# jcasal-homer/HomerHEVC

Hardware: AMD Instinct MI355X
Metric: encoded frames/sec, 1080p & 2160p YUV420 fixed-QP IPPP, 1/2/4/8 MI355X (higher is better)
Workload: dtype int16; 1 GPU; cfg2-1080p-encode; sequences_per_gpu=256, width=1920, height=1080, wfpp_num_threads=17, qp=32, gop=IPPP intra_period=100

## Files before the change

### homerhevc_amd/csrc/k_encode.hip

```cpp
#define HENC_TU_OPERANDS_IN_LDS 1
#include <stddef.h>
#include <stdlib.h>
#include <algorithm>
#include <chrono>
#include <mutex>
#include <condition_variable>
#include <new>
#include <string>
#include <thread>
#include <vector>

#include <type_traits>
#include "common.h"
#include "enc/enc_sched.h"
#include "enc/enc_host.h"
#include "enc/enc_post.h"
#include "picture_io.h"

using namespace henc;

int hmr_subpel_plane_on(hipStream_t stream, int comp, const int16_t *pic, int stride, int rows, uint8_t *out);
int hmr_subpel_planes_on(hipStream_t stream, const int16_t *pic_y, const int16_t *pic_u, const int16_t *pic_v, int stride_y, int rows_y, int stride_c, int rows_c, uint8_t *out_y,
			 uint8_t *out_u, uint8_t *out_v);

struct EncDev {
	const Seq *seq;
	const FrameCtx *frame;
	const DevTables *tables;
	const Geo *geo;
	CtuInfo *ctus, *ctus_start;
	WorkSlow *work_slow;
	int16_t *coeff;
	int *progress;
	uint32_t *prefix;
	unsigned long long *prof;
	uint8_t *guess, *truth, *outtok;
	uint8_t *chain_start, *chain_end;
	int *valid, *dirty;
	unsigned long long *hash;
	uint32_t *intra_before, *used_intra, *used_parts;
	uint8_t *rowstate;
	int *thread_seen;
	int *row0_checked;
	int *counters;
	int threads;
	int dep, dep_full;
	int after, raster;
	FrameCtx *next_frame;
	double *fin;
	RcFrame *rc_dyn;
	const int *rd_src;
	const uint8_t *rd_init, *rd_ring;
	PostPic post;
};

__device__ __forceinline__ void wave_copy_words(void *dst, const void *src, int bytes, int tid)
{
	uint32_t *d = (uint32_t *)dst;
	const uint32_t *s = (const uint32_t *)src;
	for (int i = tid; i < bytes / 4; i += 64) d[i] = s[i];
}
__device__ __forceinline__ void wave_copy_quads(void *dst, const void *src, int bytes, int tid)
{
	uint4 *d = (uint4 *)dst;
	const uint4 *s = (const uint4 *)src;
#pragma unroll 4
	for (int i = tid; i < bytes / 16; i += 64) d[i] = s[i];
}
constexpr int PRED_STATE_BYTES = (64 * 64 + 2 * 32 * 32) * (int)sizeof(pred_t), ROW_STATE_BYTES = MODE_STATE_BYTES + PRED_STATE_BYTES;
static_assert(offsetof(Work, pred_c) == offsetof(Work, pred_y) + 64 * 64 * sizeof(pred_t) && sizeof(((Work *)nullptr)->pred_c) == 2 * 32 * 32 * sizeof(pred_t), "the prediction windows are one block of Work");
static_assert(MODE_STATE_BYTES % 16 == 0 && offsetof(Work, pred_y) % 16 == 0, "wave_copy_quads alignment");

constexpr size_t LDS_WORK = (sizeof(Work) + 15) & ~(size_t)15, LDS_NODES = (sizeof(Node) * NODE_SLOTS + 15) & ~(size_t)15,
		 LDS_GEO = NHELP * HSCRATCH_ELEMS * 2;
namespace henc { __constant__ Geo henc_geo_table[NNODES]; }
constexpr bool LDS_KEEPS_CTU_RECORD = false, LDS_KEEPS_TU_TABLES = false;
static_assert(LDS_KEEPS_TU_TABLES == (HENC_TU_TABLES_IN_LDS != 0), "enc_platform.h: HENC_FT");
constexpr size_t LDS_SEQ = (sizeof(Seq) + sizeof(FrameCtx) + 31) & ~(size_t)15, LDS_CTU = LDS_KEEPS_CTU_RECORD ? (sizeof(CtuPublic) + 15) & ~(size_t)15 : 0,
		 LDS_FT = LDS_KEEPS_TU_TABLES ? (sizeof(FastTables) + 15) & ~(size_t)15 : 0;
#if defined(HENC_PROFILE)
constexpr size_t LDS_BOX = LDS_BOX_BYTES + (1 + NHELP) * LDS_ENC_BYTES, LDS_HSCRATCH = 0, LDS_RD = (sizeof(WorkRd) + 15) & ~(size_t)15;
constexpr size_t LDS_BYTES = HENC_LDS_PROF_OFFSET + 2 * PP_COUNT * 8;
constexpr size_t LDS_FT_OFFSET = LDS_WORK + LDS_NODES + LDS_GEO + LDS_SEQ + LDS_CTU + LDS_BOX + LDS_HSCRATCH;
static_assert(LDS_WORK + LDS_NODES + LDS_GEO + LDS_SEQ + LDS_CTU + LDS_BOX + LDS_HSCRATCH + LDS_FT + LDS_RD <= HENC_LDS_PROF_OFFSET, "profile table overlaps the worker state");
#else
constexpr size_t LDS_BOX = LDS_BOX_BYTES + (1 + NHELP) * LDS_ENC_BYTES, LDS_HSCRATCH = 0, LDS_RD = (sizeof(WorkRd) + 15) & ~(size_t)15;
constexpr size_t LDS_BYTES = LDS_WORK + LDS_NODES + LDS_GEO + LDS_SEQ + LDS_CTU + LDS_BOX + LDS_HSCRATCH + LDS_FT + LDS_RD;
constexpr size_t LDS_FT_OFFSET = LDS_WORK + LDS_NODES + LDS_GEO + LDS_SEQ + LDS_CTU + LDS_BOX + LDS_HSCRATCH;
#endif
static_assert(sizeof(SubpelScratch) <= LDS_WORK + LDS_NODES + LDS_GEO, "task S works where the post stage does");
static_assert(sizeof(PostScratch) <= LDS_WORK + LDS_NODES + LDS_GEO, "the post stage works in what is idle between two CTUs: the worker's Work area, the CTU's partition nodes, the helpers' scratch");
#if !defined(HENC_PROFILE)
static_assert(LDS_OFF_RD == (int)(LDS_BYTES - LDS_RD), "the RD_FULL arrays are the tail of a worker's LDS");
#endif
static_assert(LDS_OFF_ENC == (int)(LDS_WORK + LDS_NODES + LDS_GEO + LDS_SEQ + LDS_CTU + LDS_BOX_BYTES) || LDS_FT != 0 || LDS_CTU != 0, "the RD_FULL arrays are the tail of a worker's LDS: launches without RD_FULL pictures leave them out");
static_assert(LDS_OFF_NODES == (int)LDS_WORK && LDS_OFF_SEQ == (int)(LDS_WORK + LDS_NODES + LDS_GEO) && LDS_OFF_BOX == (int)(LDS_WORK + LDS_NODES + LDS_GEO + LDS_SEQ + LDS_CTU),
	      "enc_common.h: the fixed places of Enc's LDS members");
#if !defined(HENC_WAVES_PER_EU)
#define HENC_WAVES_PER_EU 2
#endif
constexpr int ENC_THREADS = 64 * (1 + NHELP);
static_assert(LDS_BYTES <= 160 * 1024, "a workgroup has 160 KiB of LDS on gfx950");
constexpr int workers_per_cu(size_t lds_bytes)
{
	const int by_lds = (int)((160 * 1024) / ((lds_bytes + 1279) / 1280 * 1280)), by_waves = 4 * HENC_WAVES_PER_EU / (1 + NHELP);
	return by_lds < by_waves ? by_lds : by_waves;
}
constexpr int WORKERS_PER_CU = workers_per_cu(LDS_BYTES - LDS_RD);
#if !defined(HENC_PROFILE) && HENC_WAVES_PER_EU == 2 && HENC_NHELP == 1
static_assert(WORKERS_PER_CU == 4, "a worker's LDS (without the RD_FULL arrays) has to stay within a quarter of the CU's: 32 granules of 1280 bytes");
#endif
#if defined(HENC_PRINT_LDS)
static_assert(LDS_BYTES - LDS_RD == 0 && LDS_WORK == 0 && LDS_NODES == 0 && LDS_BOX == 0 && sizeof(PostScratch) == 0 && WORKERS_PER_CU == 0, "sizes");
#endif

__device__ __forceinline__ bool helper_serve(HelperBox *box, int h, int16_t *scratch, const WaveGrp g, int seq)
{
	extern __shared__ __align__(16) uint8_t lds[];
	Enc &e = *(Enc *)(lds + LDS_OFF_ENC + (1 + h) * LDS_ENC_BYTES);
	HENC_ENC_IN_LDS(e);
	const Enc &worker = *(const Enc *)(lds + LDS_OFF_ENC);
	{
		const int job = box->job[h];
		if (job == HJOB_QUIT) return false;
		if (job == HJOB_NEW_CTU) {
			wave_copy_words(&e, &worker, (int)sizeof(Enc), g.tid);
			g.sync();
			e.box = nullptr;
			e.on_helper = 1 + h;
			e.scratch_a = scratch;
			e.scratch_b = scratch + 1024;
			e.adi_c = scratch + 2048;
			e.prof = nullptr;
		}
		const int *a = box->a[h];
		uint32_t r0 = 0, r1 = 0, r2 = 0, r3 = 0, r4 = 0, r5 = 0;
		switch (job) {
		case HJOB_INTER_TU: {
			int sum = 0;
			uint32_t raw = 0;
			if (NHELP == 1 && a[1] == COMP_UV && e.geo[a[0]].size_chroma <= 8) {
				const PairGrp pg{g.tid & 31, g.tid >> 5};
				const uint32_t d = encode_inter_tu(pg, e, a[0], COMP_U + pg.half, a[2], a[3], &sum, &raw, pg.half * 512);
				r0 = (uint32_t)__builtin_amdgcn_readlane((int)d, 0); r1 = (uint32_t)__builtin_amdgcn_readlane(sum, 0); r2 = (uint32_t)__builtin_amdgcn_readlane((int)raw, 0);
				r3 = (uint32_t)__builtin_amdgcn_readlane((int)d, 32); r4 = (uint32_t)__builtin_amdgcn_readlane(sum, 32); r5 = (uint32_t)__builtin_amdgcn_readlane((int)raw, 32);
				break;
			}
			r0 = encode_inter_tu(g, e, a[0], a[1] == COMP_UV ? COMP_U : a[1], a[2], a[3], &sum, &raw);
			r1 = (uint32_t)sum;
			r2 = raw;
			if (a[1] == COMP_UV) {
				r3 = encode_inter_tu(g, e, a[0], COMP_V, a[2], a[3], &sum, &raw);
				r4 = (uint32_t)sum;
				r5 = raw;
			}
			break;
		}
		case HJOB_SYNC_CU:
			if (a[1] == COMP_UV) sync_cu_chroma_both(g, e, a[0], a[2], a[3], a[4], a[5]);
			else sync_cu_comp(g, e, a[0], a[2], a[3], a[4], a[5], a[1]);
			break;
		case HJOB_SSD: {
			const Geo &q = e.geo[a[0]];
			if (a[1] == COMP_UV) {
				const int n = q.size_chroma, l = ilog2i(n);
				uint32_t acc[2] = {0, 0};
				for (int i = g.tid * 4; i < n * n; i += 64 * 4) {
					const int o = q.yc * 32 + q.xc + (i >> l) * 32 + (i & (n - 1));
#pragma unroll
					for (int c = 0; c < 2; c++) {
						const S4 va = ld4(e.w->curr_c[c] + o), vb = ld4(e.w->pred_c[c] + o);
#pragma unroll
						for (int k = 0; k < 4; k++) { const int32_t dd = (int16_t)(va.v[k] - vb.v[k]); acc[c] += (uint32_t)(dd * dd); }
					}
				}
				r0 = g.sum(acc[0]);
				r1 = g.sum(acc[1]);
			} else {
				const int c = a[1] - 1;
				r0 = blk_ssd(g, e.w->curr_c[c] + q.yc * 32 + q.xc, 32, e.w->pred_c[c] + q.yc * 32 + q.xc, 32, q.size_chroma);
			}
			break;
		}
		case HJOB_CHROMA_SEARCH: {
			const int cand[5] = {a[2] & 255, (a[2] >> 8) & 255, (a[2] >> 16) & 255, (a[2] >> 24) & 255, a[3]};
			uint32_t sads[5];
			chroma_search_comp(g, e, a[0], a[1], cand, sads);
			g.sync();
			if (g.tid == 0)
				for (int k = 0; k < 5; k++) box->r[h][k] = sads[k];
			break;
		}
		case HJOB_CHROMA_TU: {
			int cs = 0;
			r0 = (uint32_t)chroma_tu_comp(g, e, a[0], a[1], a[2], a[3], a[4], a[5] & 255, a[5] >> 8, &cs);
			r1 = (uint32_t)cs;
			break;
		}
#if defined(HENC_QUAD)
		case HJOB_QUAD_C:
			quad_chroma_job(g, e, a[0], a[1]);
			break;
#endif
		case HJOB_INTRA_SAD: {
			const Geo &q = e.geo[a[0]];
			r0 = intra_predict_sad(g, (pred_t *)nullptr, 0, e.w->curr_y + q.y * CTU_STRIDE_Y + q.x, CTU_STRIDE_Y, a[3] ? e.w->adi_f : e.w->adi, a[1], a[2], 1);
			break;
		}
		default: break;
		}
		g.sync();
		if (g.tid == 0) {
			if (job != HJOB_CHROMA_SEARCH) { box->r[h][0] = r0; box->r[h][1] = r1; box->r[h][2] = r2; box->r[h][3] = r3; box->r[h][4] = r4; box->r[h][5] = r5; }
			__hip_atomic_store(&box->done[h], seq, __ATOMIC_RELEASE, __HIP_MEMORY_SCOPE_WORKGROUP);
		}
	}
	return true;
}

__device__ __attribute__((noinline)) bool helper_serve_out(HelperBox *box, int h, int16_t *scratch, const WaveGrp g, int seq) { return helper_serve(box, h, scratch, g, seq); }

__device__ __attribute__((noinline)) bool helper_bg_search(HelperBox *box, int h, int16_t *scratch, const WaveGrp g, int &seq, int bgseq)
{
	extern __shared__ __align__(16) uint8_t lds[];
	Enc &e = *(Enc *)(lds + LDS_OFF_ENC + (1 + h) * LDS_ENC_BYTES);
	HENC_ENC_IN_LDS(e);
	const int ni = uni(box->bg_ni), depth = uni(box->bg_depth);
	const Geo &q = e.geo[ni];
	const int n = q.size, curr_depth = q.depth, inv_depth = CFG_MAX_CU_SHIFT - curr_depth;
	bool quit = false;
	int best_mode = 0, bits = -1;
	double best_cost = 0;
	if (__hip_atomic_load(&box->bg_cancel, __ATOMIC_ACQUIRE, __HIP_MEMORY_SCOPE_WORKGROUP) != bgseq) {
		node_fill_refs(g, e, ni, depth + 1, COMP_Y, 1);
		int preds[3], dirs[2];
		uint16_t src[2];
		intra_neighbour_dirs(e, ni, curr_depth, dirs, src);
		mpm_from_dirs(dirs[0], dirs[1], preds);
		const int rd_fast = e.seq->rd_mode == RDM_FAST ? 1 : 0;
		const src_t *orig = e.w->curr_y + q.y * CTU_STRIDE_Y + q.x;
		bits = intra_search_walk(preds, rd_fast, e.f->sqrt_lambda, [&](int mode) -> int64_t {
			if (__hip_atomic_load(&box->cmd[h], __ATOMIC_ACQUIRE, __HIP_MEMORY_SCOPE_WORKGROUP) == seq) {
				if (!helper_serve_out(box, h, scratch, g, seq)) { quit = true; return -1; }
				seq++;
			}
			if (__hip_atomic_load(&box->bg_cancel, __ATOMIC_ACQUIRE, __HIP_MEMORY_SCOPE_WORKGROUP) == bgseq) return -1;
			return (int64_t)intra_predict_sad(g, (pred_t *)nullptr, 0, orig, CTU_STRIDE_Y, intra_is_filtered(mode, inv_depth) ? e.w->adi_f : e.w->adi, n, mode, 1);
		}, &best_mode, &best_cost);
	}
	g.sync();
	if (g.tid == 0) {
		box->bg_mode = best_mode;
		box->bg_bits = bits;
		__hip_atomic_store(&box->bg_done, bgseq, __ATOMIC_RELEASE, __HIP_MEMORY_SCOPE_WORKGROUP);
	}
	return !quit;
}

template <bool LAT>
__device__ __attribute__((noinline)) void helper_loop(HelperBox *box, int h, int16_t *scratch)
{
	WaveGrp g{(int)(threadIdx.x & 63)};
	if constexpr (!LAT) {
		for (int seq = 1;; seq++) {
			while (__hip_atomic_load(&box->cmd[h], __ATOMIC_ACQUIRE, __HIP_MEMORY_SCOPE_WORKGROUP) != seq) __builtin_amdgcn_s_sleep(1);
			if (!helper_serve(box, h, scratch, g, seq)) return;
		}
	}
	int seq = 1, bgseq = 1;
	for (;;) {
		if (__hip_atomic_load(&box->cmd[h], __ATOMIC_ACQUIRE, __HIP_MEMORY_SCOPE_WORKGROUP) == seq) {
			if (!helper_serve_out(box, h, scratch, g, seq)) return;
			seq++;
			continue;
		}
		if (NHELP == 1 && __hip_atomic_load(&box->bg_cmd, __ATOMIC_ACQUIRE, __HIP_MEMORY_SCOPE_WORKGROUP) == bgseq) {
			if (!helper_bg_search(box, h, scratch, g, seq, bgseq)) return;
			bgseq++;
			continue;
		}
		__builtin_amdgcn_s_sleep(1);
	}
}

template <bool LAT = false>
__device__ __forceinline__ bool rows_enter(unsigned lds_bytes)
{
	extern __shared__ __align__(16) uint8_t lds[];
	HelperBox *box = (HelperBox *)(lds + LDS_WORK + LDS_NODES + LDS_GEO + LDS_SEQ + LDS_CTU);
	const int wave = (int)(threadIdx.x >> 6);
	for (int i = (int)threadIdx.x; i < (int)(lds_bytes / 4); i += ENC_THREADS) ((uint32_t *)lds)[i] = 0;
	__syncthreads();
	if (wave > 0) {
		helper_loop<LAT>(box, wave - 1, (int16_t *)(lds + LDS_WORK + LDS_NODES) + (wave - 1) * HSCRATCH_ELEMS);
		return false;
	}
	return true;
}
__device__ __forceinline__ void release_helpers(int *hseq)
{
	extern __shared__ __align__(16) uint8_t lds[];
	HelperBox *box = (HelperBox *)(lds + LDS_WORK + LDS_NODES + LDS_GEO + LDS_SEQ + LDS_CTU);
	if ((threadIdx.x & 63) == 0)
		for (int h = 0; h < NHELP; h++) {
			box->job[h] = HJOB_QUIT;
			__hip_atomic_store(&box->cmd[h], ++hseq[h], __ATOMIC_RELEASE, __HIP_MEMORY_SCOPE_WORKGROUP);
		}
}
__device__ __forceinline__ void encode_row(const EncDev &d, int pass, int row, int *hseq)
{
	extern __shared__ __align__(16) uint8_t lds[];
	const Seq &S = *d.seq;
	const int W = S.wctu, H = S.hctu;
	WaveGrp g{(int)(threadIdx.x & 63)};
	Work *lw = (Work *)lds;
	HelperBox *box = (HelperBox *)(lds + LDS_WORK + LDS_NODES + LDS_GEO + LDS_SEQ + LDS_CTU);
	for (int i = g.tid; i < (int)(LDS_WORK / 4); i += 64) ((uint32_t *)lds)[i] = 0;
	g.sync();
	Seq *lseq = (Seq *)(lds + LDS_WORK + LDS_NODES + LDS_GEO);
	FrameCtx *lframe = (FrameCtx *)((uint8_t *)lseq + ((sizeof(Seq) + 15) & ~(size_t)15));
	for (int i = g.tid; i < (int)(sizeof(Seq) / 4); i += 64) ((uint32_t *)lseq)[i] = ((const uint32_t *)d.seq)[i];
	for (int i = g.tid; i < (int)(sizeof(FrameCtx) / 4); i += 64) ((uint32_t *)lframe)[i] = ((const uint32_t *)d.frame)[i];
	if (g.tid == 0) lw->slow = (HENC_GLOBAL_PTR(WorkSlow))(d.work_slow + row);
// ... 542 lines not shown
```

### homerhevc_amd/csrc/k_encode_batch.inc

```
namespace {
__global__ __launch_bounds__(256) void k_pack_streams(const EncDev *devs, uint8_t *out, const size_t *offs)
{
	__shared__ uint32_t start[POST_MAX_ROWS + 1];
	const EncDev &d = devs[blockIdx.x];
	const int rows = d.seq->wpp ? d.seq->hctu : 1;
	if (threadIdx.x == 0) {
		uint32_t o = 0;
		for (int r = 0; r < rows; r++) { start[r] = o; o += (uint32_t)d.post.ent[r].bytecnt; }
		start[rows] = o;
	}
	__syncthreads();
	uint8_t *dst = out + offs[blockIdx.x];
	for (int r = 0; r < rows; r++) {
		const uint8_t *src = d.post.bs + (size_t)r * d.post.row_cap;
		const uint32_t n = start[r + 1] - start[r];
		for (uint32_t i = threadIdx.x; i < n; i += blockDim.x) dst[start[r] + i] = src[i];
	}
}

__global__ void k_batch_stage(const EncDev *h_devs, const FrameCtx *h_frames, EncDev *d_devs, FrameCtx *d_frames)
{
	const int i = blockIdx.x, t = threadIdx.x;
	for (int k = t; k < (int)(sizeof(EncDev) / 4); k += blockDim.x) ((uint32_t *)(d_devs + i))[k] = ((const uint32_t *)(h_devs + i))[k];
	for (int k = t; k < (int)(sizeof(FrameCtx) / 4); k += blockDim.x) ((uint32_t *)(d_frames + i))[k] = ((const uint32_t *)(h_frames + i))[k];
	const EncDev d = h_devs[i];
	const int H = d.seq->hctu, W = d.seq->wctu;
	if (t < 3) d.counters[t] = t == 2 ? -1 : 0;
	if (t == 3) *d.row0_checked = 0;
	if (t >= 4 && t < 8) d.post.errors[t - 4] = 0;
	for (int k = t; k < H * (int)(sizeof(PostRow) / 4); k += blockDim.x) ((int *)d.post.rows)[k] = 0;
	for (int k = t; k < H; k += blockDim.x) d.progress[k] = 0;
	for (int k = t; k < H * (W + 1); k += blockDim.x) d.prefix[k] = 0;
}

struct BatchTimes {
	std::chrono::steady_clock::time_point t[8];
	double ms(int a, int b) const { return std::chrono::duration<double, std::milli>(t[b] - t[a]).count(); }
};

template <class F>
void parallel_for(int n, int threads, F fn)
{
	const int T = n < threads ? n : threads;
	std::vector<std::thread> th;
	for (int t = 0; t < T; t++)
		th.emplace_back([=]() {
			for (int i = t; i < n; i += T) fn(i);
		});
	for (auto &x : th) x.join();
}
constexpr int QUEUE_THREADS = 16;
constexpr int CODING_THREADS = 32;

int batch_check(hmr_gpu_enc **encs, int n, const int *slots, uint8_t **streams, const long *caps, long *stream_bytes)
{
	if (!encs || n <= 0 || n > BATCH_MAX || !streams || !caps || !stream_bytes) return HMR_GPU_ERR_ARG;
	for (int i = 0; i < n; i++) {
		hmr_gpu_enc *e = encs[i];
		if (!e || !e->lockstep || e->ctx->device != encs[0]->ctx->device || (slots && (slots[i] < 0 || slots[i] >= (int)e->src.size())) || !streams[i]) {
			hmr_set_error("hmr_gpu_enc_encode_batch: encoder %d: needs the row-per-thread schedule (wfpp_num_threads > 1), the batch's device and a loaded picture slot", i);
			return HMR_GPU_ERR_ARG;
		}
		for (int j = 0; j < i; j++)
			if (encs[j] == e) return HMR_GPU_ERR_ARG;
	}
	return HMR_GPU_OK;
}

int batch_launch(hmr_gpu_enc **encs, int n, const int *slots, const int *image_types, int *pitch_out)
{
	hmr_gpu_enc *lead = encs[0];
	hipStream_t bst = lead->ctx->stream;
	int rc, rows_total = 0, max_ctus = 0;
	bool needs_rd = false;
	if (!lead->d_frames) {
		HIP_TRY(hipMalloc((void **)&lead->d_frames, BATCH_MAX * sizeof(FrameCtx)));
		HIP_TRY(hipHostMalloc((void **)&lead->h_frames, BATCH_MAX * sizeof(FrameCtx), hipHostMallocDefault));
		HIP_TRY(hipHostMalloc((void **)&lead->h_devs, BATCH_MAX * sizeof(EncDev), hipHostMallocDefault));
	}
	for (int i = 0; i < n; i++) {
		hmr_gpu_enc *e = encs[i];
		if ((rc = set_frame(e, slots[i], image_types ? image_types[i] : 0, -1.0, false))) return rc;
		e->pic_stream = bst;
		HIP_TRY(hipEventRecord(e->ev_ready, e->ctx->stream));
		if (i) HIP_TRY(hipStreamWaitEvent(bst, e->ev_ready, 0));
		lead->h_frames[i] = e->f;
		lead->h_devs[i] = e->d;
		lead->h_devs[i].frame = lead->d_frames + i;
		rows_total += pool_inflight(e->seq, e->raster);
		needs_rd = needs_rd || e->seq.rd_mode == RDM_FULL;
		if (e->seq.nctu > max_ctus) max_ctus = e->seq.nctu;
	}
	if (!lead->plane_stream[0]) {
		for (int k = 0; k < 2; k++) {
			HIP_TRY(hipStreamCreateWithFlags(&lead->plane_stream[k], hipStreamNonBlocking));
			HIP_TRY(hipEventCreateWithFlags(&lead->ev_plane[k], hipEventDisableTiming));
		}
		HIP_TRY(hipEventCreateWithFlags(&lead->ev_plane[2], hipEventDisableTiming));
	}
	HIP_TRY(hipEventRecord(lead->ev_plane[2], bst));
	for (int k = 0; k < 2; k++) HIP_TRY(hipStreamWaitEvent(lead->plane_stream[k], lead->ev_plane[2], 0));
	for (int i = 0; i < n; i++) {
		hmr_gpu_enc *e = encs[i];
		const Seq &s = e->seq;
		if (e->f.slice_type == SLICE_I) continue;
		if ((rc = hmr_subpel_plane_on(bst, 0, e->d_pic[e->cur ^ 1][0], s.stride_y, s.height + 2 * s.margin_y, e->planes.y))) return rc;
		for (int k = 0; k < 2; k++)
			if ((rc = hmr_subpel_plane_on(lead->plane_stream[k], 1 + k, e->d_pic[e->cur ^ 1][1 + k], s.stride_c, s.height / 2 + 2 * s.margin_c, e->planes.c[k]))) return rc;
	}
	for (int k = 0; k < 2; k++) {
		HIP_TRY(hipEventRecord(lead->ev_plane[k], lead->plane_stream[k]));
		HIP_TRY(hipStreamWaitEvent(bst, lead->ev_plane[k], 0));
	}
	if (!lead->d_batch) {
		HIP_TRY(hipMalloc((void **)&lead->d_batch, BATCH_MAX * sizeof(EncDev)));
		HIP_TRY(hipDeviceGetAttribute(&lead->n_cus, hipDeviceAttributeMultiprocessorCount, lead->ctx->device));
	}
	const int pitch = GATHER_HEAD + max_ctus + POST_MAX_ROWS;
	if ((size_t)pitch * n > lead->gather_words) {
		if (lead->d_gather) (void)hipFree(lead->d_gather);
		if (lead->h_gather) (void)hipHostFree(lead->h_gather);
		lead->d_gather = lead->h_gather = nullptr;
		lead->gather_words = 0;
		HIP_TRY(hipMalloc((void **)&lead->d_gather, (size_t)pitch * BATCH_MAX * 4));
		HIP_TRY(hipHostMalloc((void **)&lead->h_gather, (size_t)pitch * BATCH_MAX * 4, hipHostMallocDefault));
		lead->gather_words = (size_t)pitch * BATCH_MAX;
	}
	hipLaunchKernelGGL(k_batch_stage, dim3(n), dim3(256), 0, bst, (const EncDev *)lead->h_devs, (const FrameCtx *)lead->h_frames, (EncDev *)lead->d_batch, lead->d_frames);
	HIP_TRY(hipGetLastError());
	HIP_TRY(hipEventRecord(lead->ev_batch0, bst));
	if ((rc = launch_pool(lead, n, rows_total, needs_rd, bst))) return rc;
	(void)hipEventRecord(lead->ev_batch1, bst);
	hipLaunchKernelGGL(k_gather_results, dim3(n), dim3(256), 0, bst, (const EncDev *)lead->d_batch, lead->d_gather, pitch, (const int *)(lead->d_pool_state + BATCH_MAX * POOL_STRIDE));
	HIP_TRY(hipGetLastError());
	HIP_TRY(hipMemcpyAsync(lead->h_gather, lead->d_gather, (size_t)pitch * n * 4, hipMemcpyDeviceToHost, bst));
	*pitch_out = pitch;
	return HMR_GPU_OK;
}

int batch_finish(hmr_gpu_enc **encs, int n, const int *slots, int pitch, BatchTimes &bt)
{
	(void)slots;
	hmr_gpu_enc *lead = encs[0];
	hipStream_t bst = lead->ctx->stream;
	const hipError_t waited = hipStreamSynchronize(bst);
	if (waited != hipSuccess) {
		hmr_set_error("k_encode_pool: %s", hipGetErrorString(waited));
		return HMR_GPU_ERR_HIP;
	}
	bt.t[2] = std::chrono::steady_clock::now();
	float ms = 0;
	HIP_TRY(hipEventElapsedTime(&ms, lead->ev_batch0, lead->ev_batch1));
	if (!lead->h_offs) HIP_TRY(hipHostMalloc((void **)&lead->h_offs, BATCH_MAX * sizeof(size_t), hipHostMallocDefault));
	lead->pend_off.resize(n);
	lead->pend_rows.assign(n, std::vector<uint32_t>());
	size_t total = 0;
	for (int i = 0; i < n; i++) {
		hmr_gpu_enc *e = encs[i];
		const uint32_t *g = lead->h_gather + (size_t)i * pitch;
		if (g[3] & 2) {
			hmr_set_error("k_encode_pool: the launch was abandoned by its watchdog (a worker found nothing to do for too long: HENC_WATCHDOG_S)");
			return HMR_GPU_ERR_HIP;
		}
		if (g[3] & 1) {
			hmr_set_error("hmr_gpu_enc_encode_batch: sequence %d: a CTU row's sub-stream outgrew its buffer (%d bytes)", i, e->row_cap);
			return HMR_GPU_ERR_HIP;
		}
		e->note_stale_predictions(g[3] >> 8);
		const int rows = e->seq.wpp ? e->seq.hctu : 1;
		lead->pend_off[i] = total;
		lead->h_offs[i] = total;
		lead->pend_rows[i].assign(g + pitch - POST_MAX_ROWS, g + pitch - POST_MAX_ROWS + rows);
		for (int r = 0; r < rows; r++) total += lead->pend_rows[i][r];
		total = (total + 255) & ~(size_t)255;
		e->last_ms = e->last_total_ms = ms;
		e->last_encodes = (int)g[1];
		e->f.scene_cut_ctu = (int)g[2];
		e->last_passes = 1;
		release_planes(e);
		e->f_pending = e->f;
		e->awaiting_delivery = true;
		FrameRcOut ro;
		ro.sum_qp = (int)g[4]; ro.consumed_bits = (double)g[5];
		memcpy(&ro.target_pict_size, &g[6], 8);
		end_frame(e->seq, e->st, e->f, frame_acc_dist(e->seq, e->cfg.wfpp_num_threads, [&](int c) { return g[GATHER_HEAD + c]; }), &ro);
	}
	if (total > lead->stage_bytes) {
		if (lead->d_stage) (void)hipFree(lead->d_stage);
		if (lead->h_stage) (void)hipHostFree(lead->h_stage);
		lead->d_stage = lead->h_stage = nullptr;
		lead->stage_bytes = 0;
		const size_t want = total * 2 + (1 << 20);
		HIP_TRY(hipMalloc((void **)&lead->d_stage, want));
		HIP_TRY(hipHostMalloc((void **)&lead->h_stage, want, hipHostMallocDefault));
		lead->stage_bytes = want;
	}
	if (!lead->copy_stream) HIP_TRY(hipStreamCreateWithFlags(&lead->copy_stream, hipStreamNonBlocking));
	hipLaunchKernelGGL(k_pack_streams, dim3(n), dim3(256), 0, bst, (const EncDev *)lead->d_batch, lead->d_stage, (const size_t *)lead->h_offs);
	HIP_TRY(hipGetLastError());
	HIP_TRY(hipEventRecord(lead->ev_decided, bst));
	HIP_TRY(hipStreamWaitEvent(lead->copy_stream, lead->ev_decided, 0));
	if (total) HIP_TRY(hipMemcpyAsync(lead->h_stage, lead->d_stage, total, hipMemcpyDeviceToHost, lead->copy_stream));
	bt.t[3] = std::chrono::steady_clock::now();
	lead->pend_encs.assign(encs, encs + n);
	lead->pend_total = total;
	lead->pending = true;
	return HMR_GPU_OK;
}

int batch_deliver(hmr_gpu_enc *lead, uint8_t **streams, const long *caps, long *stream_bytes, BatchTimes &bt)
{
	const int n = (int)lead->pend_encs.size();
	bt.t[4] = std::chrono::steady_clock::now();
	lead->pending = false;
	for (int i = 0; i < n; i++) lead->pend_encs[i]->awaiting_delivery = false;
	HIP_TRY(hipStreamSynchronize(lead->copy_stream));
	bt.t[5] = std::chrono::steady_clock::now();
	std::vector<int> rcs(n, 0);
	std::vector<std::string> errs(n);
	parallel_for(n, CODING_THREADS, [&](int i) {
		hmr_gpu_enc *e = lead->pend_encs[i];
		rcs[i] = frame_assemble(e, e->f_pending, lead->h_stage + lead->pend_off[i], lead->pend_rows[i].data(), streams[i], caps[i], &stream_bytes[i]);
		if (rcs[i] < 0) errs[i] = hmr_gpu_last_error();
	});
	bt.t[6] = std::chrono::steady_clock::now();
	for (int i = 0; i < n; i++)
		if (rcs[i] < 0) { hmr_set_error("hmr_gpu_enc_encode_batch: sequence %d: %s", i, errs[i].c_str()); return rcs[i]; }
	return HMR_GPU_OK;
}

void batch_report(const BatchTimes &bt, hmr_gpu_enc *lead, bool pipelined)
{
	if (!getenv("HENC_BATCH_TIMING")) return;
	static std::chrono::steady_clock::time_point last_end;
	const auto now = std::chrono::steady_clock::now();
	fprintf(stderr, "batch step%s: launch %.1f ms, wait for the pool %.1f, queue device parts %.1f, download wait %.1f (%.0f MB), entropy coding %.1f; the call %.1f, since the last call %.1f\n",
		pipelined ? " (pipelined)" : "", bt.ms(0, 1), pipelined ? bt.ms(6, 2) : bt.ms(1, 2), bt.ms(2, 3), bt.ms(4, 5), lead->pend_total / 1e6, bt.ms(5, 6),
		std::chrono::duration<double, std::milli>(now - bt.t[0]).count(), std::chrono::duration<double, std::milli>(bt.t[0] - last_end).count());
	last_end = now;
}
}

extern "C" int hmr_gpu_enc_encode_batch(hmr_gpu_enc **encs, int n, const int *slots, const int *image_types, uint8_t **streams, const long *caps, long *stream_bytes)
{
	int rc = batch_check(encs, n, slots, streams, caps, stream_bytes);
	if (rc) return rc;
	if (!slots) return HMR_GPU_ERR_ARG;
	for (int i = 0; i < n; i++)
		if (encs[i]->awaiting_delivery || encs[i]->pending) {
			hmr_set_error("hmr_gpu_enc_encode_batch: encoder %d has an access unit outstanding from a pipelined call: flush first", i);
			return HMR_GPU_ERR_ARG;
		}
	hmr_gpu_enc *lead = encs[0];
	HIP_TRY(hipSetDevice(lead->ctx->device));
	BatchTimes bt;
	int pitch = 0;
	bt.t[0] = std::chrono::steady_clock::now();
	if ((rc = batch_launch(encs, n, slots, image_types, &pitch))) return rc;
	bt.t[1] = std::chrono::steady_clock::now();
	if ((rc = batch_finish(encs, n, slots, pitch, bt))) return rc;
	if ((rc = batch_deliver(lead, streams, caps, stream_bytes, bt))) return rc;
	batch_report(bt, lead, false);
	return HMR_GPU_OK;
}

extern "C" int hmr_gpu_enc_encode_batch_pipelined(hmr_gpu_enc **encs, int n, const int *slots, const int *image_types, uint8_t **streams, const long *caps, long *stream_bytes)
{
	int rc = batch_check(encs, n, slots, streams, caps, stream_bytes);
	if (rc) return rc;
	hmr_gpu_enc *lead = encs[0];
	HIP_TRY(hipSetDevice(lead->ctx->device));
	if (lead->pending) {
		if ((int)lead->pend_encs.size() != n || memcmp(lead->pend_encs.data(), encs, n * sizeof(hmr_gpu_enc *))) {
			hmr_set_error("hmr_gpu_enc_encode_batch_pipelined: the encoder list changed while access units are outstanding: flush (slots = NULL) with the previous list first");
			return HMR_GPU_ERR_ARG;
		}
	} else {
		for (int i = 0; i < n; i++)
			if (encs[i]->awaiting_delivery) {
				hmr_set_error("hmr_gpu_enc_encode_batch_pipelined: encoder %d has an access unit outstanding in another batch", i);
				return HMR_GPU_ERR_ARG;
			}
	}
	BatchTimes bt;
	for (auto &t : bt.t) t = std::chrono::steady_clock::now();
	int pitch = 0;
	if (slots && (rc = batch_launch(encs, n, slots, image_types, &pitch))) return rc;
	bt.t[1] = std::chrono::steady_clock::now();
	if (lead->pending) {
		if ((rc = batch_deliver(lead, streams, caps, stream_bytes, bt))) return rc;
	} else {
		for (int i = 0; i < n; i++) stream_bytes[i] = 0;
		bt.t[6] = bt.t[1];
	}
	if (slots && (rc = batch_finish(encs, n, slots, pitch, bt))) return rc;
	if (slots) batch_report(bt, lead, true);
	return HMR_GPU_OK;
}

extern "C" int hmr_gpu_enc_encode_chain(hmr_gpu_enc **encs, int n, hmr_gpu_enc *prev, const int *slots, const int *image_types, uint8_t **streams, const long *caps, long *stream_bytes)
{
	if (!encs || n <= 0 || n > CHAIN_MAX_FRAMES || !slots || !streams || !caps || !stream_bytes) return HMR_GPU_ERR_ARG;
	for (int j = 0; j < n; j++) {
		hmr_gpu_enc *e = encs[j];
		if (!e || !e->lockstep || e->ctx->device != encs[0]->ctx->device || slots[j] < 0 || slots[j] >= (int)e->src.size() || !streams[j] || e->awaiting_delivery || e->engine_index < 0 ||
		    e->seq.width != encs[0]->seq.width || e->seq.height != encs[0]->seq.height) {
			hmr_set_error("hmr_gpu_enc_encode_chain: frame %d: needs an engine object (hmr_gpu_enc_create_engine) of the chain's sequence on the chain's device with a loaded picture slot", j);
			return HMR_GPU_ERR_ARG;
		}
		if (n > 1 && (e->seq.bitrate_mode != 0 || e->seq.rd_mode == RDM_FULL)) {
			hmr_set_error("hmr_gpu_enc_encode_chain: frame %d: rate control and RD_FULL need the frames one at a time (a chain of %d frames starts them from a predicted state)", j, n);
			return HMR_GPU_ERR_ARG;
		}
		if (j >= e->st.engines && e->d_ctus_eng[0] != encs[j - e->st.engines]->d_ctus_eng[0]) {
			hmr_set_error("hmr_gpu_enc_encode_chain: frame %d: the object has to be a twin (hmr_gpu_enc_create_engine_twin) of the one that encodes frame %d, the engine's frame before it", j, j - e->st.engines);
			return HMR_GPU_ERR_ARG;
		}
		for (int i = 0; i < j; i++)
			if (encs[i] == e) return HMR_GPU_ERR_ARG;
	}
	hmr_gpu_enc *lead = encs[0];
	hipStream_t bst = lead->ctx->stream;
	HIP_TRY(hipSetDevice(lead->ctx->device));
	int rc, rows_total = 0;
	bool needs_rd = false;
	if (!lead->d_frames) {
		HIP_TRY(hipMalloc((void **)&lead->d_frames, BATCH_MAX * sizeof(FrameCtx)));
		HIP_TRY(hipHostMalloc((void **)&lead->h_frames, BATCH_MAX * sizeof(FrameCtx), hipHostMallocDefault));
		HIP_TRY(hipHostMalloc((void **)&lead->h_devs, BATCH_MAX * sizeof(EncDev), hipHostMallocDefault));
	}
	if (!lead->d_batch) HIP_TRY(hipMalloc((void **)&lead->d_batch, BATCH_MAX * sizeof(EncDev)));
	HostState st = prev ? prev->st : lead->st;
	const HostState start_state = st;
	struct Undo { hmr_gpu_enc *e; int cur; HostState st; FrameCtx f; PlaneSet planes, planes2; EncDev d; bool has_picture; hipStream_t pic_stream; };
	std::vector<Undo> undo;
	auto refuse = [&](int code) {
		for (size_t k = undo.size(); k-- > 0;) {
			Undo &u = undo[k];
			u.e->cur = u.cur; u.e->st = u.st; u.e->f = u.f; u.e->chain_planes = u.planes; u.e->chain_planes2 = u.planes2; u.e->d = u.d;
			u.e->has_picture = u.has_picture; u.e->pic_stream = u.pic_stream;
		}
		return code;
	};
	for (int j = 0; j < n; j++) {
		hmr_gpu_enc *e = encs[j];
		const Seq &s = e->seq;
		if (st.num_encoded_frames % e->st.engines != e->engine_index) {
			hmr_set_error("hmr_gpu_enc_encode_chain: frame %d of the sequence belongs to engine %d, not %d", st.num_encoded_frames, st.num_encoded_frames % e->st.engines, e->engine_index);
			return refuse(HMR_GPU_ERR_ARG);
		}
		for (int k = 0; k < 2; k++) {
			PlaneSet &ps = k ? e->chain_planes2 : e->chain_planes;
			if (ps.y) continue;
			PlaneSet p;
			p.device = e->ctx->device; p.bytes_y = (size_t)16 * s.plane_elems_y; p.bytes_c = (size_t)64 * s.plane_elems_c;
			HIP_TRY(hipMalloc((void **)&p.y, p.bytes_y));
			HIP_TRY(hipMalloc((void **)&p.c[0], p.bytes_c));
			HIP_TRY(hipMalloc((void **)&p.c[1], p.bytes_c));
			ps = p;
		}
		undo.push_back(Undo{e, e->cur, e->st, e->f, e->chain_planes, e->chain_planes2, e->d, e->has_picture, e->pic_stream});
		e->st = st;
		const hmr_gpu_enc *r = j ? encs[j - 1] : prev;
		const int16_t *ref_planes[3] = {nullptr, nullptr, nullptr};
		PlaneSet ref_set;
		if (r) {
			for (int c = 0; c < 3; c++) ref_planes[c] = plane0(const_cast<hmr_gpu_enc *>(r), r->cur, c);
			ref_set = r->chain_planes;
		}
		std::swap(e->chain_planes, e->chain_planes2);
		if (j == 0 && e == prev) ref_set = e->chain_planes2;
		if ((rc = set_frame(e, slots[j], image_types ? image_types[j] : 0, -1.0, false, true))) return refuse(rc);
		e->pic_stream = bst;
		st = e->st;
		st.num_encoded_frames++;
		if (e->f.slice_type != SLICE_I) {
			if (!r || !ref_set.y) {
				hmr_set_error("hmr_gpu_enc_encode_chain: frame %d is a P frame and there is no object that holds the picture before it with its phase planes", j);
				return refuse(HMR_GPU_ERR_ARG);
			}
			for (int c = 0; c < 3; c++) e->f.ref[c] = ref_planes[c];
			e->f.sub_y = ref_set.y + (size_t)s.margin_y * 16 * s.stride_y + s.margin_y;
			e->f.sub_c[0] = ref_set.c[0] + (size_t)s.margin_c * 64 * s.stride_c + s.margin_c;
			e->f.sub_c[1] = ref_set.c[1] + (size_t)s.margin_c * 64 * s.stride_c + s.margin_c;
			e->d.dep = j ? j - 1 : -1;
			e->d.dep_full = getenv("HENC_CHAIN_SERIAL") ? 1 : 0;
		}
		if (j >= e->st.engines) {
			const hmr_gpu_enc *b = encs[j - e->st.engines];
			if (b->f.slice_type == SLICE_I && b->f.num_encoded_frames != 0 && s.intra_period != 1) {
				hmr_set_error("hmr_gpu_enc_encode_chain: frame %d is an I frame inside the sequence and the same engine's next frame is in the chain: end the chain before frame %d", j - e->st.engines, j);
				return refuse(HMR_GPU_ERR_ARG);
			}
			e->d.after = j - e->st.engines;
			e->f.avg_dist = 0.0;
			lead->h_devs[j - e->st.engines].next_frame = lead->d_frames + j;
		}
		e->d.post.planes[0] = e->chain_planes.y; e->d.post.planes[1] = e->chain_planes.c[0]; e->d.post.planes[2] = e->chain_planes.c[1];
		HIP_TRY(hipEventRecord(e->ev_ready, e->ctx->stream));
		if (j) HIP_TRY(hipStreamWaitEvent(bst, e->ev_ready, 0));
		lead->h_frames[j] = e->f;
		lead->h_devs[j] = e->d;
		lead->h_devs[j].frame = lead->d_frames + j;
		rows_total += s.hctu;
		needs_rd = needs_rd || s.rd_mode == RDM_FULL;
	}
	const int nctu = lead->seq.nctu, pitch = GATHER_HEAD + nctu + POST_MAX_ROWS;
	if ((size_t)pitch * n > lead->gather_words) {
		if (lead->d_gather) (void)hipFree(lead->d_gather);
		if (lead->h_gather) (void)hipHostFree(lead->h_gather);
		lead->d_gather = lead->h_gather = nullptr;
		lead->gather_words = 0;
		HIP_TRY(hipMalloc((void **)&lead->d_gather, (size_t)pitch * BATCH_MAX * 4));
		HIP_TRY(hipHostMalloc((void **)&lead->h_gather, (size_t)pitch * BATCH_MAX * 4, hipHostMallocDefault));
		lead->gather_words = (size_t)pitch * BATCH_MAX;
	}
	hipLaunchKernelGGL(k_batch_stage, dim3(n), dim3(256), 0, bst, (const EncDev *)lead->h_devs, (const FrameCtx *)lead->h_frames, (EncDev *)lead->d_batch, lead->d_frames);
	HIP_TRY(hipGetLastError());
	HIP_TRY(hipEventRecord(lead->ev_batch0, bst));
	if ((rc = launch_pool(lead, n, rows_total, needs_rd, bst))) return rc;
	(void)hipEventRecord(lead->ev_batch1, bst);
	hipLaunchKernelGGL(k_gather_results, dim3(n), dim3(256), 0, bst, (const EncDev *)lead->d_batch, lead->d_gather, pitch, (const int *)(lead->d_pool_state + BATCH_MAX * POOL_STRIDE));
	HIP_TRY(hipGetLastError());
	HIP_TRY(hipMemcpyAsync(lead->h_gather, lead->d_gather, (size_t)pitch * n * 4, hipMemcpyDeviceToHost, bst));
	{
		const hipError_t waited = hipStreamSynchronize(bst);
		if (waited != hipSuccess) { hmr_set_error("k_encode_pool: %s", hipGetErrorString(waited)); return HMR_GPU_ERR_HIP; }
	}
	float ms = 0;
	HIP_TRY(hipEventElapsedTime(&ms, lead->ev_batch0, lead->ev_batch1));
	HostState seq_state = start_state;
	bool cut_before = false;
	for (int j = 0; j < n; j++) {
		hmr_gpu_enc *e = encs[j];
		const Seq &s = e->seq;
		const uint32_t *g = lead->h_gather + (size_t)j * pitch;
		if (g[3] & 2) { hmr_set_error("k_encode_pool: the launch was abandoned by its watchdog (HENC_WATCHDOG_S)"); return HMR_GPU_ERR_HIP; }
		if (g[3] & 1) { hmr_set_error("hmr_gpu_enc_encode_chain: frame %d: a CTU row's sub-stream outgrew its buffer (%d bytes)", j, e->row_cap); return HMR_GPU_ERR_HIP; }
		e->note_stale_predictions(g[3] >> 8);
		e->last_ms = e->last_total_ms = ms;
		e->last_encodes = (int)g[1];
		e->f.scene_cut_ctu = (int)g[2];
		e->last_passes = 1;
		const bool fired = (int)g[2] >= 0;
		if (fired && cut_before) {
			hmr_set_error("hmr_gpu_enc_encode_chain: two frames of the chain detected a scene change: in the sequential order the first one switches the detection off for the second; repeat the chain frame by frame");
			return HMR_GPU_ERR_ARG;
		}
		cut_before = cut_before || fired;
		FrameCtx replay;
		e->st = seq_state;
		begin_frame(s, e->st, image_types ? image_types[j] : 0, replay);
		double acc_dist;
		memcpy(&acc_dist, &g[8], 8);
		memcpy(&e->f.avg_dist, &g[10], 8);
		if (replay.slice_type != e->f.slice_type || replay.poc != e->f.poc || replay.avg_dist != e->f.avg_dist) {
			hmr_set_error("hmr_gpu_enc_encode_chain: frame %d started from a state the frames before it changed", j);
			return HMR_GPU_ERR_ARG;
		}
		FrameRcOut ro;
		ro.sum_qp = (int)g[4]; ro.consumed_bits = (double)g[5];
		memcpy(&ro.target_pict_size, &g[6], 8);
		end_frame(s, e->st, e->f, acc_dist, &ro);
		seq_state = e->st;
		const int rows = s.wpp ? s.hctu : 1;
		std::vector<uint32_t> row_bytes(g + pitch - POST_MAX_ROWS, g + pitch - POST_MAX_ROWS + rows);
		size_t total = 0;
		for (int r = 0; r < rows; r++) total += row_bytes[r];
		if (e->h_bs.size() < total) e->h_bs.resize(total);
		total = 0;
		for (int r = 0; r < rows; r++) {
			HIP_TRY(hipMemcpyAsync(e->h_bs.data() + total, e->d_bs + (size_t)r * e->row_cap, row_bytes[r], hipMemcpyDeviceToHost, bst));
			total += row_bytes[r];
		}
		HIP_TRY(hipStreamSynchronize(bst));
		if ((rc = frame_assemble(e, e->f, e->h_bs.data(), row_bytes.data(), streams[j], caps[j], &stream_bytes[j])) < 0) return rc;
	}
	return HMR_GPU_OK;
}

extern "C" int hmr_gpu_enc_encode(hmr_gpu_enc *e, const uint8_t *y, const uint8_t *u, const uint8_t *v, int image_type, uint8_t *stream, long cap, long *stream_bytes,
				  uint8_t *recon)
{
	const int rc = hmr_gpu_enc_load_source(e, 0, y, u, v);
	if (rc) return rc;
	return hmr_gpu_enc_encode_source(e, 0, image_type, stream, cap, stream_bytes, recon);
}
```

### homerhevc_amd/csrc/k_encode_object.inc

```
template <class T>
struct PinnedAlloc {
	typedef T value_type;
	PinnedAlloc() = default;
	template <class U> PinnedAlloc(const PinnedAlloc<U> &) {}
	T *allocate(size_t n)
	{
		void *p = nullptr;
		if (hipHostMalloc(&p, n * sizeof(T), hipHostMallocDefault) != hipSuccess) throw std::bad_alloc();
		return (T *)p;
	}
	void deallocate(T *p, size_t) { (void)hipHostFree(p); }
	template <class U> bool operator==(const PinnedAlloc<U> &) const { return true; }
	template <class U> bool operator!=(const PinnedAlloc<U> &) const { return false; }
};

struct PlaneSet { uint8_t *y = nullptr, *c[2] = {nullptr, nullptr}; size_t bytes_y = 0, bytes_c = 0; int device = 0; };
struct PlanePool {
	std::mutex m;
	std::vector<PlaneSet> free_sets;
	int acquire(int device, size_t by, size_t bc, PlaneSet *out)
	{
		{
			std::lock_guard<std::mutex> lk(m);
			for (size_t i = 0; i < free_sets.size(); i++)
				if (free_sets[i].device == device && free_sets[i].bytes_y == by && free_sets[i].bytes_c == bc) {
					*out = free_sets[i];
					free_sets.erase(free_sets.begin() + (long)i);
					return HMR_GPU_OK;
				}
		}
		PlaneSet p;
		p.device = device; p.bytes_y = by; p.bytes_c = bc;
		if (hipMalloc((void **)&p.y, by) != hipSuccess || hipMalloc((void **)&p.c[0], bc) != hipSuccess || hipMalloc((void **)&p.c[1], bc) != hipSuccess) {
			(void)hipGetLastError();
			if (p.y) (void)hipFree(p.y);
			if (p.c[0]) (void)hipFree(p.c[0]);
			if (p.c[1]) (void)hipFree(p.c[1]);
			hmr_set_error("phase planes: out of device memory (%zu bytes per picture)", by + 2 * bc);
			return HMR_GPU_ERR_HIP;
		}
		*out = p;
		return HMR_GPU_OK;
	}
	void release(const PlaneSet &p)
	{
		std::lock_guard<std::mutex> lk(m);
		free_sets.push_back(p);
	}
	int live = 0;
	void encoder_created() { std::lock_guard<std::mutex> lk(m); live++; }
	void encoder_destroyed()
	{
		std::lock_guard<std::mutex> lk(m);
		if (--live > 0) return;
		for (PlaneSet &p : free_sets) {
			(void)hipSetDevice(p.device);
			(void)hipFree(p.y); (void)hipFree(p.c[0]); (void)hipFree(p.c[1]);
		}
		free_sets.clear();
	}
};
PlanePool g_plane_pool;
struct hmr_gpu_enc {
	hmr_gpu_ctx *ctx;
	HostCfg cfg;
	long stale_last = -1, stale_total = 0;
	void note_stale_predictions(uint32_t n) { stale_last = (long)n; stale_total += (long)n; }
	Seq seq;
	HostState st;
	FrameCtx f;
	EncDev d;
	Seq *d_seq;
	FrameCtx *d_frame;
	Geo *d_geo;
	std::vector<Geo> geo;
	std::vector<SrcSlot> src;
	int16_t *d_pic[2][3], *d_pre[3], *d_rec[3];
	PostRow *d_rows = nullptr;
	RowEnt *d_ent = nullptr;
	uint8_t *d_bs = nullptr;
	uint32_t *d_cumbits = nullptr;
	double *d_sao_tab = nullptr;
	int *d_post_err = nullptr;
	RdCtxSim rdsim[MAX_ENGINES];
	uint8_t *d_ctx_ring = nullptr, *d_rd_init = nullptr;
	int *d_rd_src = nullptr;
	uint8_t h_rd_init[(1 + RD_RING) * RD_CTX_BYTES] = {0};
	uint16_t *d_rc_need = nullptr;
	RcFrame *d_rc_dyn = nullptr;
	int row_cap = 0;
	std::vector<RowEnt> h_ent;
	std::vector<uint8_t, PinnedAlloc<uint8_t>> h_bs;
	PlaneSet chain_planes2;
	PlaneSet chain_planes;
	PlaneSet planes;
	size_t src_elems[3], pic_elems[3];
	uint8_t *d_bytes;
	int units_stride, units_rows;
	int16_t *d_mvx, *d_mvy;
	int8_t *d_ref;
	uint8_t *d_qp, *d_flags;
	uint8_t *d_public;
	std::vector<uint8_t, PinnedAlloc<uint8_t>> h_public;
	std::vector<int16_t, PinnedAlloc<int16_t>> h_coeff;
	std::vector<int32_t> h_stats, h_params;
	std::vector<double> h_lambdas;
	hipEvent_t ev_frame = nullptr, ev_ready = nullptr, ev_batch0 = nullptr, ev_batch1 = nullptr;
	int n_cus = 0;
	uint8_t *d_stage = nullptr, *h_stage = nullptr;
	size_t stage_bytes = 0;
	void *d_batch = nullptr;
	bool pending = false, download_queued = false;
	std::vector<hmr_gpu_enc *> pend_encs;
	std::vector<size_t> pend_off;
	std::vector<std::vector<uint32_t>> pend_rows;
	size_t *h_offs = nullptr;
	size_t pend_total = 0;
	hipStream_t copy_stream = nullptr;
	uint32_t *d_gather = nullptr, *h_gather = nullptr;
	size_t gather_words = 0;
	bool awaiting_delivery = false;
	FrameCtx f_pending;
	double acc_pending = 0;
	hipEvent_t ev_packed = nullptr;
	hipEvent_t ev_decided = nullptr;
	FrameCtx *d_frames = nullptr, *h_frames = nullptr;
	EncDev *h_devs = nullptr;
	hipStream_t plane_stream[2] = {nullptr, nullptr};
	hipEvent_t ev_plane[3] = {nullptr, nullptr, nullptr};
	int *d_pool_state = nullptr;
	WorkSlow *d_pool_slow = nullptr;
	int pool_workers = 0;
	JobRing<IngestJob> ingest;
	JobRing<RgbIngestJob> ingest_rgb;
	JobRing<ScaleJob> scale;
	JobRing<EgressJob> egress;
	JobRing<SsimJob> ssim;
	bool has_picture = false;
	hipStream_t pic_stream = nullptr;
	hipEvent_t ev_pic_done = nullptr, ev_own_done = nullptr;
	EntropyState es;
	CtuInfo *d_ctus_eng[MAX_ENGINES] = {nullptr};
	uint8_t *d_rowstate_eng[MAX_ENGINES] = {nullptr};
	int *d_seen_eng[MAX_ENGINES] = {nullptr};
	hmr_gpu_enc *twin_of = nullptr;
	int local_engines = 1, engine_index = -1;
	int cur, lockstep;
	int raster = 0;
	float last_ms, last_total_ms;
	int last_passes, last_encodes;
};

namespace {
void release_planes(hmr_gpu_enc *e);
constexpr int REC_BYTES = 32 + 3 * 256 + 2 * 256 + 9 * 256 + 256 + 256 + 2048 + 2048 + 6144 * 2 + 6144 * 2 + 2 * 5 * 256;

int16_t *plane0(hmr_gpu_enc *e, int which, int comp)
{
	const Seq &s = e->seq;
	const int st = comp ? s.stride_c : s.stride_y, m = comp ? s.margin_c : s.margin_y;
	return e->d_pic[which][comp] + (size_t)m * st + m;
}

template <class T>
int dev_alloc(T **p, size_t n, hipStream_t st)
{
	HIP_TRY(hipMalloc((void **)p, n * sizeof(T)));
	HIP_TRY(hipMemsetAsync(*p, 0, n * sizeof(T), st));
	HIP_TRY(hipStreamSynchronize(st));
	return HMR_GPU_OK;
}
#define DEV_ALLOC(p, n)                           \
	do {                                      \
		const int rc_ = dev_alloc(&(p), (n), e->ctx->stream); \
		if (rc_) return rc_;              \
	} while (0)

IngestJob ingest_job(const hmr_gpu_enc *e, const hmr_gpu_picture &pic, int16_t *const dst[3], int stride_y, int stride_c)
{
	IngestJob j;
	for (int c = 0; c < 3; c++) {
		j.src[c] = pic.plane[c];
		j.pitch[c] = pic.pitch[c];
		j.dst[c] = dst[c];
	}
	j.stride_y = stride_y; j.stride_c = stride_c;
	j.width = e->seq.width; j.height = e->seq.height;
	j.format = pic.format; j.reserved = 0;
	return j;
}
EgressJob egress_job(hmr_gpu_enc *e, const hmr_gpu_picture *pic, int16_t *const src[3], uint64_t *ssd)
{
	const Seq &s = e->seq;
	EgressJob j;
	for (int c = 0; c < 3; c++) {
		j.rec[c] = plane0(e, e->cur, c);
		j.src[c] = src ? src[c] : nullptr;
		j.dst[c] = pic ? const_cast<uint8_t *>(pic->plane[c]) : nullptr;
		j.pitch[c] = pic ? pic->pitch[c] : 0;
	}
	j.ssd = ssd;
	j.stride_y = s.stride_y; j.stride_c = s.stride_c;
	j.src_stride_y = s.src_stride_y; j.src_stride_c = s.src_stride_c;
	j.width = s.width; j.height = s.height;
	j.format = pic ? pic->format : HMR_GPU_PIC_I420; j.reserved = 0;
	return j;
}
hmr_gpu_picture packed_picture(const hmr_gpu_enc *e, const uint8_t *bytes)
{
	const int64_t w = e->seq.width, h = e->seq.height;
	return hmr_gpu_picture{HMR_GPU_PIC_I420, 0, {bytes, bytes + w * h, bytes + w * h + (w / 2) * (h / 2)}, {w, w / 2, w / 2}};
}
int widen_packed(hmr_gpu_enc *e, const uint8_t *bytes, int16_t *const dst[3], int stride_y, int stride_c)
{
	const IngestJob j = ingest_job(e, packed_picture(e, bytes), dst, stride_y, stride_c);
	return run_jobs(e->ingest, hmr_ingest_launch, e->ctx->stream, &j, 1, e->ctx->stream);
}
int narrow_packed(hmr_gpu_enc *e, uint8_t *bytes)
{
	const hmr_gpu_picture pic = packed_picture(e, bytes);
	const EgressJob j = egress_job(e, &pic, nullptr, nullptr);
	return run_jobs(e->egress, hmr_egress_launch, e->ctx->stream, &j, 1, e->ctx->stream);
}

int load_planes(hmr_gpu_enc *e, const uint8_t *y, const uint8_t *u, const uint8_t *v, int16_t *const dst[3], int stride_y, int stride_c)
{
	hipStream_t st = e->ctx->stream;
	const hmr_gpu_picture staged = packed_picture(e, e->d_bytes);
	const uint8_t *in[3] = {y, u, v};
	for (int c = 0; c < 3; c++)
		HIP_TRY(hipMemcpyAsync(const_cast<uint8_t *>(staged.plane[c]), in[c], (size_t)staged.pitch[c] * (c ? e->seq.height / 2 : e->seq.height), hipMemcpyHostToDevice, st));
	const int rc = widen_packed(e, e->d_bytes, dst, stride_y, stride_c);
	if (rc) return rc;
	HIP_TRY(hipStreamSynchronize(st));
	return HMR_GPU_OK;
}


int reference_planes(hmr_gpu_enc *e, hipStream_t st)
{
	const Seq &s = e->seq;
	if (e->f.slice_type == SLICE_I) return HMR_GPU_OK;
	return hmr_subpel_planes_on(st, e->d_pic[e->cur ^ 1][0], e->d_pic[e->cur ^ 1][1], e->d_pic[e->cur ^ 1][2], s.stride_y, s.height + 2 * s.margin_y, s.stride_c,
				    s.height / 2 + 2 * s.margin_c, e->planes.y, e->planes.c[0], e->planes.c[1]);
}
int ctu_stage_prepare(hmr_gpu_enc *e, bool planes_elsewhere = false)
{
	const Seq &s = e->seq;
	hipStream_t st = e->ctx->stream;
	if (!e->lockstep)
		HIP_TRY(hipMemcpyAsync(e->d.ctus_start, e->d.ctus, sizeof(CtuInfo) * s.nctu, hipMemcpyDeviceToDevice, st));
	if (!planes_elsewhere) {
		const int rc = reference_planes(e, st);
		if (rc) return rc;
	}
	{
		static const int zero_counters[3] = {0, 0, -1};
		HIP_TRY(hipMemcpyAsync(e->d.counters, zero_counters, sizeof zero_counters, hipMemcpyHostToDevice, st));
	}
	if (e->lockstep) {
		HIP_TRY(hipMemsetAsync(e->d.progress, 0, sizeof(int) * s.hctu, st));
		HIP_TRY(hipMemsetAsync(e->d.row0_checked, 0, sizeof(int), st));
		HIP_TRY(hipMemsetAsync(e->d.prefix, 0, sizeof(uint32_t) * s.hctu * (s.wctu + 1), st));
	}
	HIP_TRY(hipMemsetAsync(e->d_rows, 0, sizeof(PostRow) * s.hctu, st));
	HIP_TRY(hipMemsetAsync(e->d_post_err, 0, sizeof(int) * 4, st));
	return HMR_GPU_OK;
}
int lockstep_collect(hmr_gpu_enc *e)
{
	hipStream_t st = e->ctx->stream;
	int counters[3], aborted = 0;
	HIP_TRY(hipMemcpyAsync(counters, e->d.counters, sizeof counters, hipMemcpyDeviceToHost, st));
	HIP_TRY(hipMemcpyAsync(&aborted, e->d_pool_state + BATCH_MAX * POOL_STRIDE + 1, sizeof(int), hipMemcpyDeviceToHost, st));
	HIP_TRY(hipStreamSynchronize(st));
	e->last_encodes = counters[1];
	e->f.scene_cut_ctu = counters[2];
	e->last_passes = 1;
	release_planes(e);
	if (aborted) {
		hmr_set_error("k_encode_pool: the launch was abandoned by its watchdog (a worker found nothing to do for too long: HENC_WATCHDOG_S)");
		return HMR_GPU_ERR_HIP;
	}
	return HMR_GPU_OK;
}

static int pool_inflight(const Seq &s, int raster = 0)
{
	if (raster) return 3;
	const int by_step = s.hctu < (s.wctu + 1) / 2 ? s.hctu : (s.wctu + 1) / 2;
	return s.bitrate_mode != 0 ? (by_step + 1) / 2 : by_step;
}
int launch_pool(hmr_gpu_enc *lead, int n, int rows_total, bool needs_rd, hipStream_t st)
{
	if (!lead->n_cus) HIP_TRY(hipDeviceGetAttribute(&lead->n_cus, hipDeviceAttributeMultiprocessorCount, lead->ctx->device));
#if defined(HENC_PROFILE)
	const size_t lds_default = LDS_BYTES + (needs_rd ? 0 : 0);
#else
	const size_t lds_default = needs_rd ? LDS_BYTES : LDS_BYTES - LDS_RD;
#endif
	const size_t lds_bytes = getenv("HENC_LDS_BYTES") && (size_t)atoi(getenv("HENC_LDS_BYTES")) > lds_default ? (size_t)atoi(getenv("HENC_LDS_BYTES")) : lds_default;
	if (lds_bytes > 160 * 1024) {
		hmr_set_error("k_encode_pool: a worker's LDS request of %zu bytes (HENC_LDS_BYTES) is more than a CU has", lds_bytes);
		return HMR_GPU_ERR_ARG;
	}
	const int cap = lead->n_cus * workers_per_cu(lds_bytes);
	int workers = rows_total < cap ? rows_total : cap;
	if (workers < 1) workers = 1;
	if (getenv("HENC_POOL_WORKERS") && atoi(getenv("HENC_POOL_WORKERS")) > 0 && atoi(getenv("HENC_POOL_WORKERS")) < workers) workers = atoi(getenv("HENC_POOL_WORKERS"));
	if (!lead->d_pool_state) HIP_TRY(hipMalloc((void **)&lead->d_pool_state, sizeof(int) * (BATCH_MAX * POOL_STRIDE + 4)));
	if (lead->pool_workers < workers) {
		if (lead->d_pool_slow) (void)hipFree(lead->d_pool_slow);
		lead->d_pool_slow = nullptr;
		lead->pool_workers = 0;
		HIP_TRY(hipMalloc((void **)&lead->d_pool_slow, sizeof(WorkSlow) * workers));
		HIP_TRY(hipMemsetAsync(lead->d_pool_slow, 0, sizeof(WorkSlow) * workers, st));
		lead->pool_workers = workers;
	}
	HIP_TRY(hipMemsetAsync(lead->d_pool_state, 0, sizeof(int) * (BATCH_MAX * POOL_STRIDE + 4), st));
	double watchdog_s = getenv("HENC_WATCHDOG_S") ? atof(getenv("HENC_WATCHDOG_S")) : 120.0;
	if (!(watchdog_s > 0)) watchdog_s = 120.0;
	const unsigned long long watchdog = (unsigned long long)(watchdog_s * 1e8);
	if (workers <= 256) hipLaunchKernelGGL(k_encode_pool_lat, dim3(workers), dim3(ENC_THREADS), lds_bytes, st, (const EncDev *)lead->d_batch, n, lead->d_pool_state, lead->d_pool_state + BATCH_MAX * POOL_STRIDE,
			   lead->d_pool_slow, watchdog, (unsigned)lds_default);
	else hipLaunchKernelGGL(k_encode_pool, dim3(workers), dim3(ENC_THREADS), lds_bytes, st, (const EncDev *)lead->d_batch, n, lead->d_pool_state, lead->d_pool_state + BATCH_MAX * POOL_STRIDE,
			   lead->d_pool_slow, watchdog, (unsigned)lds_default);
	const hipError_t launched = hipGetLastError();
	if (launched != hipSuccess) {
		hmr_set_error("k_encode_pool: %s", hipGetErrorString(launched));
		return HMR_GPU_ERR_HIP;
	}
	return HMR_GPU_OK;
}

int run_ctu_passes(hmr_gpu_enc *e)
{
	const Seq &s = e->seq;
	hipStream_t st = e->ctx->stream;
	int rc = ctu_stage_prepare(e);
	if (rc) return rc;
	HIP_TRY(hipEventRecord(e->ctx->ev0, st));
	if (e->lockstep) {
		if (!e->d_batch) HIP_TRY(hipMalloc((void **)&e->d_batch, BATCH_MAX * sizeof(EncDev)));
		HIP_TRY(hipMemcpyAsync(e->d_batch, &e->d, sizeof(EncDev), hipMemcpyHostToDevice, st));
		if ((rc = launch_pool(e, 1, e->raster ? pool_inflight(s, 1) : s.hctu, s.rd_mode == RDM_FULL, st))) return rc;
		HIP_TRY(hipEventRecord(e->ctx->ev1, st));
		if ((rc = lockstep_collect(e))) return rc;
		HIP_TRY(hipEventElapsedTime(&e->last_ms, e->ctx->ev0, e->ctx->ev1));
		return HMR_GPU_OK;
	}
	int pass = 0;
	for (;; pass++) {
		HIP_TRY(hipMemsetAsync(e->d.progress, 0, sizeof(int) * s.hctu, st));
		{
			EncDev dd = e->d;
			int pp = pass;
			void *args[] = {&dd, &pp};
			const hipError_t launched = hipLaunchCooperativeKernel((const void *)k_encode_ctus, dim3(s.hctu), dim3(ENC_THREADS), args, (unsigned)LDS_BYTES, st);
			if (launched != hipSuccess) {
				hmr_set_error("k_encode_ctus (%d row workers, cooperative): %s", s.hctu, hipGetErrorString(launched));
				return HMR_GPU_ERR_HIP;
			}
		}
		hipLaunchKernelGGL(k_sched_scan, dim3(1), dim3(320), 0, st, e->d);
		hipLaunchKernelGGL(k_sched_check, dim3(s.nctu), dim3(64), 0, st, e->d);
		HIP_TRY(hipGetLastError());
		int counters[3];
		HIP_TRY(hipMemcpyAsync(counters, e->d.counters, sizeof counters, hipMemcpyDeviceToHost, st));
		HIP_TRY(hipStreamSynchronize(st));
		e->last_encodes = counters[1];
		e->f.scene_cut_ctu = counters[2];
		if (counters[0] == 0) break;
		if (pass > s.nctu + 2) {
			hmr_set_error("hmr_gpu_enc: the CTU schedule did not converge");
			return HMR_GPU_ERR_HIP;
		}
	}
	hipLaunchKernelGGL(k_sched_finish, dim3(s.nctu), dim3(64), 0, st, e->d);
	HIP_TRY(hipMemcpyAsync(e->d.chain_start, e->d.chain_end, MODE_STATE_BYTES, hipMemcpyDeviceToDevice, st));
	HIP_TRY(hipMemcpyAsync(e->d_frame, &e->f, sizeof(FrameCtx), hipMemcpyHostToDevice, st));
	HIP_TRY(hipFuncSetAttribute((const void *)k_post_frame, hipFuncAttributeMaxDynamicSharedMemorySize, (int)sizeof(PostScratch)));
	hipLaunchKernelGGL(k_post_frame, dim3(s.hctu < 32 ? s.hctu : 32), dim3(64), sizeof(PostScratch), st, e->d);
	HIP_TRY(hipGetLastError());
	HIP_TRY(hipEventRecord(e->ctx->ev1, st));
	HIP_TRY(hipStreamSynchronize(st));
	HIP_TRY(hipEventElapsedTime(&e->last_ms, e->ctx->ev0, e->ctx->ev1));
	e->last_passes = pass + 1;
	release_planes(e);
	return HMR_GPU_OK;
}

int set_frame(hmr_gpu_enc *e, int slot, int image_type, double avg_dist, bool upload = true, bool chain = false)
{
	const Seq &s = e->seq;
	e->cur ^= 1;
	e->has_picture = true;
	e->pic_stream = e->ctx->stream;
	{
		const int k = e->local_engines > 1 ? e->st.num_encoded_frames % e->local_engines : 0;
		e->d.ctus = e->d_ctus_eng[k];
		e->d.rowstate = e->d_rowstate_eng[k];
		e->d.thread_seen = e->d_seen_eng[k];
	}
	begin_frame(s, e->st, image_type, e->f);
	if (avg_dist >= 0) e->f.avg_dist = avg_dist;
	e->f.lockstep = e->lockstep && !e->raster;
	for (int c = 0; c < 3; c++) {
		e->f.src[c] = e->src[slot].p[c];
		e->f.ref[c] = plane0(e, e->cur ^ 1, c);
		e->f.rec[c] = e->d_rec[c] + (size_t)(c ? s.margin_c : s.margin_y) * (c ? s.stride_c : s.stride_y) + (c ? s.margin_c : s.margin_y);
		e->d.post.fin[c] = plane0(e, e->cur, c);
	}
	e->d.post.sao_lambda = e->d_sao_tab + (e->f.slice_type == SLICE_I ? 104 : 0);
	e->d.post.ctx_after = nullptr;
	if (s.rd_mode == RDM_FULL) {
		std::vector<RdCtxVersion> src;
		e->rdsim[e->local_engines > 1 ? e->f.num_encoded_frames % e->local_engines : 0].frame(e->f.num_encoded_frames, src, e->raster != 0);
		std::vector<int> codes(s.nctu);
		for (int n = 0; n < s.nctu; n++) {
			const RdCtxVersion v = src[n];
			if (v.frame > e->f.num_encoded_frames || (v.frame >= 0 && v.frame <= e->f.num_encoded_frames - RD_RING)) {
				hmr_set_error("RD_FULL: CTU %d copies coder states of frame %d in frame %d (the states of %d frames are kept)", n, v.frame, e->f.num_encoded_frames, RD_RING);
				return HMR_GPU_ERR_ARG;
			}
			const int slot = v.frame < 0 ? 0 : v.frame % RD_RING;
			codes[n] = v.frame < 0 ? 0 : (v.k == 0 ? (1 << 28) | (slot << 24) : (3 << 28) | (slot << 24) | (v.row * s.wctu + v.k - 1));
		}
		const int slot_now = e->f.num_encoded_frames % RD_RING;
		for (int i = 0; i < CTX_TOTAL; i++) e->h_rd_init[(1 + slot_now) * RD_CTX_BYTES + i] = Cabac::init_state(e->f.slice_type, e->f.qp, i);
		HIP_TRY(hipMemcpyAsync(e->d_rd_src, codes.data(), sizeof(int) * s.nctu, hipMemcpyHostToDevice, e->ctx->stream));
		HIP_TRY(hipMemcpyAsync(e->d_rd_init, e->h_rd_init, sizeof e->h_rd_init, hipMemcpyHostToDevice, e->ctx->stream));
		e->d.post.ctx_after = e->d_ctx_ring + (size_t)slot_now * s.nctu * RD_CTX_BYTES;
		e->d.rd_src = e->d_rd_src;
		e->d.rd_init = e->d_rd_init;
		e->d.rd_ring = e->d_ctx_ring;
	}
	e->d.dep = -1;
	e->d.dep_full = 0;
	e->d.after = -1;
	e->d.next_frame = nullptr;
// ... 51 lines not shown

extern "C" int hmr_gpu_enc_record_bytes(void) { return REC_BYTES; }

static thread_local int g_serial_pool = 0;
static int enc_create(hmr_gpu_ctx *ctx, const hmr_gpu_enc_cfg *cfg, int engine_index, hmr_gpu_enc **out)
{
	if (!ctx || !cfg || !out) return HMR_GPU_ERR_ARG;
	static_assert(sizeof(hmr_gpu_enc_cfg) == sizeof(HostCfg), "configuration layouts must match");
	static_assert(offsetof(CtuInfo, n_spec_reads) % 4 == 0 && sizeof(Node) % 4 == 0 && sizeof(Geo) % 2 == 0 && sizeof(Seq) % 4 == 0 && sizeof(FrameCtx) % 4 == 0 && sizeof(CtuPublic) % 4 == 0 && MODE_STATE_BYTES % 4 == 0, "word copies");
	hmr_gpu_enc *e = new hmr_gpu_enc();
	e->ctx = ctx;
	memcpy(&e->cfg, cfg, sizeof(HostCfg));
	const char *why = "";
	if (!make_seq(e->cfg, e->seq, &why)) {
		hmr_set_error("hmr_gpu_enc_create: configuration outside the built rows: %s", why);
		delete e;
		return HMR_GPU_ERR_ARG;
	}
	e->st.engines = clampi(e->cfg.num_enc_engines, 1, MAX_ENGINES);
	e->engine_index = engine_index;
	e->local_engines = engine_index >= 0 ? 1 : e->st.engines;
	if (e->st.engines > 1 && e->cfg.wfpp_num_threads < 2 && engine_index >= 0) {
		hmr_set_error("hmr_gpu_enc_create: configuration outside the built rows: num_enc_engines > 1 needs the row-per-thread schedule (wfpp_num_threads > 1)");
		delete e;
		return HMR_GPU_ERR_ARG;
	}
	if (engine_index >= e->st.engines) { delete e; return HMR_GPU_ERR_ARG; }
	if (e->cfg.bitrate_mode != 0) host_rc_init(e->cfg, e->seq, e->st);
	g_plane_pool.encoder_created();
	struct Guard {
		hmr_gpu_enc *e;
		bool ok = false;
		~Guard() { if (!ok) hmr_gpu_enc_destroy(e); }
	} guard{e};
	e->seq.wide_min_n = 0;
	e->raster = e->cfg.wfpp_num_threads <= 1 && (e->cfg.bitrate_mode != 0 || e->seq.rd_mode == RDM_FULL || g_serial_pool || e->st.engines > 1);
	e->lockstep = e->cfg.wfpp_num_threads > 1 || e->raster;
	const Seq &s = e->seq;
	HIP_TRY(hipSetDevice(ctx->device));
	e->geo.resize(NNODES);
	make_geo(e->geo.data());
	DEV_ALLOC(e->d_seq, 1);
	HIP_TRY(hipMemcpy(e->d_seq, &s, sizeof(Seq), hipMemcpyHostToDevice));
	DEV_ALLOC(e->d_frame, 1);
	DEV_ALLOC(e->d_geo, NNODES);
	HIP_TRY(hipMemcpy(e->d_geo, e->geo.data(), sizeof(Geo) * NNODES, hipMemcpyHostToDevice));
	HIP_TRY(hipMemcpyToSymbol(HIP_SYMBOL(henc_geo_table), e->geo.data(), sizeof(Geo) * NNODES));
	DEV_ALLOC(e->d.ctus, s.nctu);
	if (e->cfg.wfpp_num_threads <= 1) DEV_ALLOC(e->d.ctus_start, s.nctu);
	{
		std::vector<CtuInfo> init(s.nctu);
		memset((void *)init.data(), 0, sizeof(CtuInfo) * s.nctu);
		for (auto &c : init) memset(c.mv_ref_idx, -1, sizeof c.mv_ref_idx);
		HIP_TRY(hipMemcpy(e->d.ctus, init.data(), sizeof(CtuInfo) * s.nctu, hipMemcpyHostToDevice));
		e->d_ctus_eng[0] = e->d.ctus;
		for (int k = 1; k < e->local_engines; k++) {
			DEV_ALLOC(e->d_ctus_eng[k], s.nctu);
			HIP_TRY(hipMemcpy(e->d_ctus_eng[k], init.data(), sizeof(CtuInfo) * s.nctu, hipMemcpyHostToDevice));
		}
	}
	if (e->cfg.wfpp_num_threads <= 1) DEV_ALLOC(e->d.work_slow, s.hctu);
	HIP_TRY(hipFuncSetAttribute((const void *)k_encode_ctus, hipFuncAttributeMaxDynamicSharedMemorySize, (int)LDS_BYTES));
	HIP_TRY(hipFuncSetAttribute((const void *)k_encode_pool, hipFuncAttributeMaxDynamicSharedMemorySize, 160 * 1024));
	HIP_TRY(hipFuncSetAttribute((const void *)k_encode_pool_lat, hipFuncAttributeMaxDynamicSharedMemorySize, 160 * 1024));
	HIP_TRY(hipEventCreate(&e->ev_frame));
	HIP_TRY(hipEventCreate(&e->ev_ready));
	HIP_TRY(hipEventCreate(&e->ev_batch0));
	HIP_TRY(hipEventCreate(&e->ev_batch1));
	HIP_TRY(hipEventCreateWithFlags(&e->ev_packed, hipEventDisableTiming));
	HIP_TRY(hipEventCreateWithFlags(&e->ev_decided, hipEventDisableTiming));
	DEV_ALLOC(e->d.coeff, (size_t)6144 * s.nctu);
	DEV_ALLOC(e->d.progress, s.hctu);
	DEV_ALLOC(e->d.prefix, (size_t)s.hctu * (s.wctu + 1));
	DEV_ALLOC(e->d.prof, (size_t)s.hctu * PF_COUNT + (size_t)s.nctu * 4);
	DEV_ALLOC(e->d.guess, (size_t)s.nctu * MODE_STATE_BYTES);
	DEV_ALLOC(e->d.truth, (size_t)s.nctu * MODE_STATE_BYTES);
	DEV_ALLOC(e->d.outtok, (size_t)s.nctu * MODE_STATE_BYTES);
	DEV_ALLOC(e->d.chain_start, MODE_STATE_BYTES);
	DEV_ALLOC(e->d.chain_end, MODE_STATE_BYTES);
	DEV_ALLOC(e->d.valid, s.nctu);
	DEV_ALLOC(e->d.dirty, s.nctu);
	DEV_ALLOC(e->d.hash, s.nctu);
	DEV_ALLOC(e->d.intra_before, s.nctu);
	DEV_ALLOC(e->d.used_intra, s.nctu);
	DEV_ALLOC(e->d.used_parts, s.nctu);
	DEV_ALLOC(e->d.counters, 4);
	DEV_ALLOC(e->d.rowstate, (size_t)s.hctu * ROW_STATE_BYTES);
	DEV_ALLOC(e->d.thread_seen, 64);
	e->d_rowstate_eng[0] = e->d.rowstate;
	e->d_seen_eng[0] = e->d.thread_seen;
	for (int k = 1; k < e->local_engines; k++) {
		DEV_ALLOC(e->d_rowstate_eng[k], (size_t)s.hctu * ROW_STATE_BYTES);
		DEV_ALLOC(e->d_seen_eng[k], 64);
	}
	DEV_ALLOC(e->d.row0_checked, 1);
	for (int c = 0; c < 3; c++) {
		e->src_elems[c] = (size_t)(c ? s.src_stride_c : s.src_stride_y) * (c ? s.height / 2 : s.height);
		e->pic_elems[c] = (size_t)(c ? s.stride_c : s.stride_y) * ((c ? s.height / 2 : s.height) + 2 * (c ? s.margin_c : s.margin_y));
		for (int k = 0; k < 2; k++) DEV_ALLOC(e->d_pic[k][c], e->pic_elems[c]);
		DEV_ALLOC(e->d_pre[c], e->pic_elems[c]);
		DEV_ALLOC(e->d_rec[c], e->pic_elems[c]);
	}
	{
		e->row_cap = s.wctu * CTU_STREAM_BOUND;
		DEV_ALLOC(e->d_rows, s.hctu);
		DEV_ALLOC(e->d_ent, s.hctu);
		DEV_ALLOC(e->d_bs, (size_t)e->row_cap * s.hctu);
		DEV_ALLOC(e->d_cumbits, s.nctu);
		DEV_ALLOC(e->d_sao_tab, 2 * 52 * 2);
		DEV_ALLOC(e->d_post_err, 4 + 2 * 16 + 4);
		double tab[2][104];
		sao_lambda_table(s, SLICE_P, tab[0]);
		sao_lambda_table(s, SLICE_I, tab[1]);
		HIP_TRY(hipMemcpy(e->d_sao_tab, tab, sizeof tab, hipMemcpyHostToDevice));
		e->h_ent.resize(s.hctu);
		DEV_ALLOC(e->d_rc_dyn, 1);
		if (s.rd_mode == RDM_FULL) {
			for (auto &sim : e->rdsim) sim.init(e->cfg.wfpp_num_threads > 1 ? e->cfg.wfpp_num_threads : 1, s.wctu, s.hctu, s.sao);
			DEV_ALLOC(e->d_ctx_ring, (size_t)RD_RING * s.nctu * RD_CTX_BYTES);
			HIP_TRY(hipMemset(e->d_ctx_ring, 0, (size_t)RD_RING * s.nctu * RD_CTX_BYTES));
			DEV_ALLOC(e->d_rd_init, (1 + RD_RING) * RD_CTX_BYTES);
			DEV_ALLOC(e->d_rd_src, s.nctu);
		}
		if (e->cfg.bitrate_mode != 0 || s.rd_mode == RDM_FULL) {
			std::vector<uint16_t> need;
			if (!rc_need_table(s.wctu, s.hctu, s.sao, e->cfg.wfpp_num_threads > 1, need)) {
				hmr_set_error("hmr_gpu_enc_create: rate control: the reference's entropy-coding lag is not row-monotone on a %d x %d CTU grid", s.wctu, s.hctu);
				return HMR_GPU_ERR_ARG;
			}
			DEV_ALLOC(e->d_rc_need, need.size());
			HIP_TRY(hipMemcpy(e->d_rc_need, need.data(), need.size() * sizeof(uint16_t), hipMemcpyHostToDevice));
		}
	}
	DEV_ALLOC(e->d_bytes, (size_t)s.width * s.height * 3 / 2);
	e->units_stride = s.wctu * 16;
	e->units_rows = s.hctu * 16;
	const size_t nu = (size_t)e->units_stride * e->units_rows;
	DEV_ALLOC(e->d_mvx, nu); DEV_ALLOC(e->d_mvy, nu); DEV_ALLOC(e->d_ref, nu); DEV_ALLOC(e->d_qp, nu);
	DEV_ALLOC(e->d_flags, nu);
	DEV_ALLOC(e->d_public, sizeof(CtuPublic) * s.nctu);
	e->h_public.resize(sizeof(CtuPublic) * s.nctu);
	e->h_coeff.resize((size_t)6144 * s.nctu);
	e->h_stats.resize((size_t)s.nctu * 3 * 5 * 2 * 32);
	e->h_params.resize((size_t)s.nctu * 3 * 34);
	e->d.seq = e->d_seq;
	e->d.frame = e->d_frame;
	e->d.tables = ctx->tables;
	e->d.geo = e->d_geo;
	e->d.rc_dyn = e->d_rc_dyn;
	{
		const size_t oy = (size_t)s.margin_y * s.stride_y + s.margin_y, oc = (size_t)s.margin_c * s.stride_c + s.margin_c;
		PostPic &P = e->d.post;
		memset(&P, 0, sizeof P);
		P.dbk[0] = e->d_pre[0] + oy; P.dbk[1] = e->d_pre[1] + oc; P.dbk[2] = e->d_pre[2] + oc;
		P.units_stride = e->units_stride;
		P.mvx = e->d_mvx; P.mvy = e->d_mvy; P.ref = e->d_ref; P.uqp = e->d_qp; P.flags = e->d_flags;
		P.rows = e->d_rows; P.ent = e->d_ent; P.bs = e->d_bs; P.row_cap = e->row_cap; P.cumbits = e->d_cumbits;
		P.sao_lambda = e->d_sao_tab; P.errors = e->d_post_err; P.rc_need = e->d_rc_need;
		P.prof = (unsigned long long *)(e->d_post_err + 4);
		e->d.fin = (double *)(e->d_post_err + 4 + 2 * 16);
	}
	e->cur = 0;
	e->d.raster = e->raster;
	e->d.threads = e->cfg.wfpp_num_threads > 1 ? e->cfg.wfpp_num_threads : 1;
	e->last_ms = e->last_total_ms = 0;
	e->last_passes = e->last_encodes = 0;
	HIP_TRY(hipStreamSynchronize(ctx->stream));
	guard.ok = true;
	*out = e;
	return HMR_GPU_OK;
}

extern "C" int hmr_gpu_enc_create(hmr_gpu_ctx *ctx, const hmr_gpu_enc_cfg *cfg, hmr_gpu_enc **out) { return enc_create(ctx, cfg, -1, out); }
extern "C" int hmr_gpu_enc_create_serial_pool(hmr_gpu_ctx *ctx, const hmr_gpu_enc_cfg *cfg, hmr_gpu_enc **out)
{
	if (!cfg || cfg->wfpp_num_threads > 1 || cfg->num_enc_engines > 1) {
		hmr_set_error("hmr_gpu_enc_create_serial_pool: wfpp_num_threads and num_enc_engines must be 1");
		return HMR_GPU_ERR_ARG;
	}
	g_serial_pool = 1;
	const int rc = enc_create(ctx, cfg, -1, out);
	g_serial_pool = 0;
	return rc;
}
extern "C" int hmr_gpu_enc_create_engine(hmr_gpu_ctx *ctx, const hmr_gpu_enc_cfg *cfg, int engine_index, hmr_gpu_enc **out)
{
	if (engine_index < 0) return HMR_GPU_ERR_ARG;
	return enc_create(ctx, cfg, engine_index, out);
}
extern "C" int hmr_gpu_enc_create_engine_twin(hmr_gpu_ctx *ctx, hmr_gpu_enc *of, hmr_gpu_enc **out)
{
	if (!ctx || !of || !out || of->engine_index < 0 || of->twin_of) return HMR_GPU_ERR_ARG;
	hmr_gpu_enc *t = nullptr;
	const int rc = enc_create(ctx, (const hmr_gpu_enc_cfg *)&of->cfg, of->engine_index, &t);
	if (rc) return rc;
	(void)hipFree(t->d_ctus_eng[0]);
	(void)hipFree(t->d_rowstate_eng[0]);
	(void)hipFree(t->d_seen_eng[0]);
	t->d_ctus_eng[0] = of->d_ctus_eng[0];
	t->d_rowstate_eng[0] = of->d_rowstate_eng[0];
	t->d_seen_eng[0] = of->d_seen_eng[0];
	t->d.ctus = t->d_ctus_eng[0]; t->d.rowstate = t->d_rowstate_eng[0]; t->d.thread_seen = t->d_seen_eng[0];
	t->twin_of = of;
	*out = t;
	return HMR_GPU_OK;
}
extern "C" int hmr_gpu_enc_state_bytes(void) { return (int)sizeof(HostState); }
extern "C" long hmr_gpu_enc_reference_elems(hmr_gpu_enc *e, int comp) { return e && comp >= 0 && comp < 3 ? (long)e->pic_elems[comp] : -1; }

extern "C" int hmr_gpu_enc_export_reference(hmr_gpu_enc *e, int16_t *dy, int16_t *du, int16_t *dv, void *state)
{
	if (!e || !dy || !du || !dv || !state) return HMR_GPU_ERR_ARG;
	hipStream_t st = e->ctx->stream;
	HIP_TRY(hipSetDevice(e->ctx->device));
	int16_t *dst[3] = {dy, du, dv};
	for (int c = 0; c < 3; c++) HIP_TRY(hipMemcpyAsync(dst[c], e->d_pic[e->cur][c], e->pic_elems[c] * 2, hipMemcpyDeviceToDevice, st));
	HIP_TRY(hipStreamSynchronize(st));
	memcpy(state, &e->st, sizeof(HostState));
	return HMR_GPU_OK;
}
extern "C" int hmr_gpu_enc_import_reference(hmr_gpu_enc *e, const int16_t *dy, const int16_t *du, const int16_t *dv, const void *state)
{
	if (!e || !dy || !du || !dv || !state) return HMR_GPU_ERR_ARG;
	HostState in;
	memcpy(&in, state, sizeof in);
	if (in.engines != e->st.engines || (e->engine_index >= 0 && in.num_encoded_frames % e->st.engines != e->engine_index)) {
		hmr_set_error("hmr_gpu_enc_import_reference: state of frame %d does not precede a frame of engine %d of %d", in.num_encoded_frames - 1, e->engine_index, e->st.engines);
		return HMR_GPU_ERR_ARG;
	}
	hipStream_t st = e->ctx->stream;
	HIP_TRY(hipSetDevice(e->ctx->device));
	const int16_t *src[3] = {dy, du, dv};
	for (int c = 0; c < 3; c++) HIP_TRY(hipMemcpyAsync(e->d_pic[e->cur][c], src[c], e->pic_elems[c] * 2, hipMemcpyDeviceToDevice, st));
	HIP_TRY(hipStreamSynchronize(st));
	e->st = in;
	return HMR_GPU_OK;
}

extern "C" long hmr_gpu_enc_reference_bytes(hmr_gpu_enc *e) { return e ? (long)e->seq.width * e->seq.height * 3 / 2 : -1; }
extern "C" int hmr_gpu_enc_export_references8(hmr_gpu_enc **encs, int n, uint8_t *dev_rows, long pitch, void *states)
{
	if (!encs || n <= 0 || !dev_rows || !states) return HMR_GPU_ERR_ARG;
	for (int i = 0; i < n; i++) {
		hmr_gpu_enc *e = encs[i];
		if (!e || pitch < hmr_gpu_enc_reference_bytes(e)) return HMR_GPU_ERR_ARG;
		HIP_TRY(hipSetDevice(e->ctx->device));
		const int rc = narrow_packed(e, dev_rows + (size_t)i * pitch);
		if (rc) return rc;
		memcpy((uint8_t *)states + (size_t)i * sizeof(HostState), &e->st, sizeof(HostState));
	}
	for (int i = 0; i < n; i++) HIP_TRY(hipStreamSynchronize(encs[i]->ctx->stream));
	return HMR_GPU_OK;
}
extern "C" int hmr_gpu_enc_import_references8(hmr_gpu_enc **encs, int n, const uint8_t *dev_rows, long pitch, const void *states)
{
	if (!encs || n <= 0 || !dev_rows || !states) return HMR_GPU_ERR_ARG;
	for (int i = 0; i < n; i++) {
		hmr_gpu_enc *e = encs[i];
		if (!e || pitch < hmr_gpu_enc_reference_bytes(e)) return HMR_GPU_ERR_ARG;
		HostState in;
		memcpy(&in, (const uint8_t *)states + (size_t)i * sizeof(HostState), sizeof in);
		if (in.engines != e->st.engines || (e->engine_index >= 0 && in.num_encoded_frames % e->st.engines != e->engine_index)) {
			hmr_set_error("hmr_gpu_enc_import_references8: engine %d: state of frame %d does not precede a frame of engine %d of %d", i, in.num_encoded_frames - 1, e->engine_index, e->st.engines);
			return HMR_GPU_ERR_ARG;
		}
		const Seq &s = e->seq;
		HIP_TRY(hipSetDevice(e->ctx->device));
		int16_t *dst[3] = {plane0(e, e->cur, 0), plane0(e, e->cur, 1), plane0(e, e->cur, 2)};
		int rc = widen_packed(e, dev_rows + (size_t)i * pitch, dst, s.stride_y, s.stride_c);
		if (rc) return rc;
		hmr_gpu_frame fr = {s.width, s.height, dst[0], dst[1], dst[2], s.stride_y, s.stride_c};
		rc = hmr_gpu_pad_frame(e->ctx, &fr, s.margin_y, s.margin_y);
		if (rc) return rc;
		e->st = in;
	}
	for (int i = 0; i < n; i++) HIP_TRY(hipStreamSynchronize(encs[i]->ctx->stream));
	return HMR_GPU_OK;
}

extern "C" void hmr_gpu_enc_destroy(hmr_gpu_enc *e)
{
	if (!e) return;
	(void)hipSetDevice(e->ctx->device);
	(void)hipStreamSynchronize(e->ctx->stream);
	release_planes(e);
	for (PlaneSet *ps : {&e->chain_planes, &e->chain_planes2})
		if (ps->y) { (void)hipFree(ps->y); (void)hipFree(ps->c[0]); (void)hipFree(ps->c[1]); }
	e->d.ctus = e->d_ctus_eng[0]; e->d.rowstate = e->d_rowstate_eng[0]; e->d.thread_seen = e->d_seen_eng[0];
	if (e->twin_of) e->d.ctus = nullptr, e->d.rowstate = nullptr, e->d.thread_seen = nullptr;
	for (int k = 1; k < MAX_ENGINES; k++) {
		if (e->d_ctus_eng[k]) (void)hipFree(e->d_ctus_eng[k]);
		if (e->d_rowstate_eng[k]) (void)hipFree(e->d_rowstate_eng[k]);
		if (e->d_seen_eng[k]) (void)hipFree(e->d_seen_eng[k]);
	}
	if (e->ev_frame) (void)hipEventDestroy(e->ev_frame);
	if (e->ev_ready) (void)hipEventDestroy(e->ev_ready);
	if (e->ev_batch0) (void)hipEventDestroy(e->ev_batch0);
	if (e->ev_batch1) (void)hipEventDestroy(e->ev_batch1);
	if (e->ev_packed) (void)hipEventDestroy(e->ev_packed);
	if (e->ev_decided) (void)hipEventDestroy(e->ev_decided);
	if (e->d_frames) (void)hipFree(e->d_frames);
	if (e->h_frames) (void)hipHostFree(e->h_frames);
	if (e->h_devs) (void)hipHostFree(e->h_devs);
	for (int k = 0; k < 2; k++) if (e->plane_stream[k]) { (void)hipStreamSynchronize(e->plane_stream[k]); (void)hipStreamDestroy(e->plane_stream[k]); }
	for (int k = 0; k < 3; k++) if (e->ev_plane[k]) (void)hipEventDestroy(e->ev_plane[k]);
	if (e->copy_stream) { (void)hipStreamSynchronize(e->copy_stream); (void)hipStreamDestroy(e->copy_stream); }
	if (e->d_gather) (void)hipFree(e->d_gather);
	if (e->h_gather) (void)hipHostFree(e->h_gather);
	if (e->h_offs) (void)hipHostFree(e->h_offs);
	e->ingest.release();
	e->ingest_rgb.release();
	e->scale.release();
	e->egress.release();
	e->ssim.release();
	if (e->ev_pic_done) (void)hipEventDestroy(e->ev_pic_done);
	if (e->ev_own_done) (void)hipEventDestroy(e->ev_own_done);
	if (e->d_batch) (void)hipFree(e->d_batch);
	if (e->d_pool_state) (void)hipFree(e->d_pool_state);
	if (e->d_pool_slow) (void)hipFree(e->d_pool_slow);
	if (e->d_stage) (void)hipFree(e->d_stage);
	if (e->h_stage) (void)hipHostFree(e->h_stage);
	void *p[] = {e->d_seq, e->d_frame, e->d_geo, e->d.ctus, e->d.ctus_start, e->d.work_slow, e->d.coeff, e->d.progress, e->d.prefix, e->d.prof, e->d.guess, e->d.truth, e->d.outtok,
		     e->d.chain_start, e->d.chain_end, e->d.valid, e->d.dirty, e->d.hash, e->d.intra_before, e->d.used_intra, e->d.used_parts, e->d.counters, e->d.rowstate, e->d.thread_seen, e->d.row0_checked, e->d_bytes, e->d_mvx,
		     e->d_mvy, e->d_ref, e->d_qp, e->d_flags, e->d_public};
	for (void *q : p) (void)hipFree(q);
	for (int c = 0; c < 3; c++) {
		(void)hipFree(e->d_pic[0][c]);
		(void)hipFree(e->d_pic[1][c]);
		(void)hipFree(e->d_pre[c]);
		(void)hipFree(e->d_rec[c]);
	}
	{
		void *pp[] = {e->d_rows, e->d_ent, e->d_bs, e->d_cumbits, e->d_sao_tab, e->d_post_err, e->d_rc_need, e->d_rc_dyn, e->d_ctx_ring, e->d_rd_init, e->d_rd_src};
		for (void *q : pp) (void)hipFree(q);
	}
	for (auto &sl : e->src)
		for (int c = 0; c < 3; c++) (void)hipFree(sl.p[c]);
	delete e;
	g_plane_pool.encoder_destroyed();
}

extern "C" int hmr_gpu_enc_post_profile(hmr_gpu_enc *e, unsigned long long *out)
{
	if (!e || !out) return HMR_GPU_ERR_ARG;
	HIP_TRY(hipMemcpy(out, e->d_post_err + 4, 16 * sizeof(unsigned long long), hipMemcpyDeviceToHost));
#if defined(HENC_POST_PROFILE)
	HIP_TRY(hipMemcpyFromSymbol(out + 10, HIP_SYMBOL(g_ent_prof), 6 * sizeof(unsigned long long)));
#endif
	return HMR_GPU_OK;
}

extern "C" float hmr_gpu_enc_last_ctu_ms(hmr_gpu_enc *e) { return e ? e->last_ms : 0.f; }

extern "C" int hmr_gpu_enc_stale_predictions(hmr_gpu_enc *e, long *last_picture, long *all_pictures)
{
	if (!e) return HMR_GPU_ERR_ARG;
	if (last_picture) *last_picture = e->stale_last;
	if (all_pictures) *all_pictures = e->stale_total;
	return HMR_GPU_OK;
}

extern "C" int hmr_gpu_enc_last_stats(hmr_gpu_enc *e, int *passes, int *ctu_encodes, float *ctu_ms, float *frame_ms)
{
	if (!e) return HMR_GPU_ERR_ARG;
	if (passes) *passes = e->last_passes;
	if (ctu_encodes) *ctu_encodes = e->last_encodes;
	if (ctu_ms) *ctu_ms = e->last_ms;
	if (frame_ms) *frame_ms = e->last_total_ms;
	return HMR_GPU_OK;
}

extern "C" int hmr_gpu_enc_timeline(hmr_gpu_enc *e, unsigned long long *out)
{
	if (!e || !out) return HMR_GPU_ERR_ARG;
	HIP_TRY(hipMemcpy(out, e->d.prof + (size_t)e->seq.hctu * PF_COUNT, sizeof(unsigned long long) * e->seq.nctu * 4, hipMemcpyDeviceToHost));
	return HMR_GPU_OK;
}

extern "C" int hmr_gpu_enc_profile(hmr_gpu_enc *e, unsigned long long *out, int reset)
{
	if (!e || !out) return HMR_GPU_ERR_ARG;
	HIP_TRY(hipMemcpy(out, e->d.prof, sizeof(unsigned long long) * e->seq.hctu * PF_COUNT, hipMemcpyDeviceToHost));
	if (reset) {
		HIP_TRY(hipMemsetAsync(e->d.prof, 0, sizeof(unsigned long long) * e->seq.hctu * PF_COUNT, e->ctx->stream));
		HIP_TRY(hipStreamSynchronize(e->ctx->stream));
	}
	return HMR_GPU_OK;
}

extern "C" int hmr_gpu_enc_load_source(hmr_gpu_enc *e, int slot, const uint8_t *y, const uint8_t *u, const uint8_t *v)
{
	if (!e || slot < 0 || slot > 4096 || !y || !u || !v) return HMR_GPU_ERR_ARG;
	HIP_TRY(hipSetDevice(e->ctx->device));
	while ((int)e->src.size() <= slot) {
		SrcSlot sl;
		for (int c = 0; c < 3; c++) DEV_ALLOC(sl.p[c], e->src_elems[c]);
		e->src.push_back(sl);
	}
	return load_planes(e, y, u, v, e->src[slot].p, e->seq.src_stride_y, e->seq.src_stride_c);
}

extern "C" int hmr_gpu_enc_frame_ctus(hmr_gpu_enc *e, const uint8_t *y, const uint8_t *u, const uint8_t *v, int image_type, const uint8_t *ref_y, const uint8_t *ref_u,
				      const uint8_t *ref_v, double avg_dist, uint8_t *records)
{
	if (!e || !y || !u || !v) return HMR_GPU_ERR_ARG;
	const Seq &s = e->seq;
	hipStream_t st = e->ctx->stream;
	HIP_TRY(hipSetDevice(e->ctx->device));
	int rc = hmr_gpu_enc_load_source(e, 0, y, u, v);
	if (rc) return rc;
	rc = set_frame(e, 0, image_type, avg_dist);
	if (rc) return rc;
	if (ref_y && ref_u && ref_v) {
		int16_t *dst[3] = {plane0(e, e->cur ^ 1, 0), plane0(e, e->cur ^ 1, 1), plane0(e, e->cur ^ 1, 2)};
		rc = load_planes(e, ref_y, ref_u, ref_v, dst, s.stride_y, s.stride_c);
		if (rc) return rc;
		hmr_gpu_frame fr = {s.width, s.height, dst[0], dst[1], dst[2], s.stride_y, s.stride_c};
		rc = hmr_gpu_pad_frame(e->ctx, &fr, s.margin_y, s.margin_y);
		if (rc) return rc;
	}
	rc = run_ctu_passes(e);
	if (rc) return rc;
	rc = download_public(e);
	if (rc) return rc;
	HIP_TRY(hipStreamSynchronize(st));
	end_frame(s, e->st, e->f, frame_acc_dist(s, e->cfg.wfpp_num_threads, [&](int n) { return ((const CtuPublic *)(e->h_public.data() + sizeof(CtuPublic) * n))->distortion; }));
	if (records) {
		std::vector<int16_t> rec[3];
		std::vector<uint8_t> truth((size_t)s.nctu * MODE_STATE_BYTES), chain_end(MODE_STATE_BYTES);
		std::vector<uint32_t> node0(3 * s.nctu);
		HIP_TRY(hipMemcpy(e->h_coeff.data(), e->d.coeff, e->h_coeff.size() * 2, hipMemcpyDeviceToHost));
		HIP_TRY(hipMemcpy(truth.data(), e->d.truth, truth.size(), hipMemcpyDeviceToHost));
		HIP_TRY(hipMemcpy(chain_end.data(), e->d.chain_end, MODE_STATE_BYTES, hipMemcpyDeviceToHost));
		for (int n = 0; n < s.nctu; n++) {
			Node nd;
			HIP_TRY(hipMemcpy(&nd, &e->d.ctus[n].nodes[0], sizeof(Node), hipMemcpyDeviceToHost));
			node0[3 * n] = nd.cost; node0[3 * n + 1] = nd.distortion; node0[3 * n + 2] = nd.sum;
		}
		for (int c = 0; c < 3; c++) {
			rec[c].resize(e->pic_elems[c]);
			HIP_TRY(hipMemcpy(rec[c].data(), e->d_rec[c], e->pic_elems[c] * 2, hipMemcpyDeviceToHost));
		}
		memset(records, 0, (size_t)REC_BYTES * s.nctu);
		for (int n = 0; n < s.nctu; n++) {
			uint8_t *o = records + (size_t)n * REC_BYTES;
			const CtuPublic &ci = *(const CtuPublic *)(e->h_public.data() + sizeof(CtuPublic) * n);
			int32_t hdr[8] = {0x43545544, e->f.num_encoded_frames, n, e->f.slice_type, (int32_t)node0[3 * n], (int32_t)node0[3 * n + 1], (int32_t)node0[3 * n + 2],
					  e->f.scene_cut_ctu >= 0 && n >= e->f.scene_cut_ctu};
			memcpy(o, hdr, 32); o += 32;
			for (int k = 0; k < 3; k++) { memcpy(o, ci.cbf[k], 256); o += 256; }
			memcpy(o, ci.intra_mode[0], 256); o += 256;
			memcpy(o, ci.intra_mode[1], 256); o += 256;
			const uint8_t *arrs[9] = {ci.inter_mode, ci.tr_idx, ci.pred_depth, ci.part_size_type, ci.pred_mode, ci.skipped, ci.merge, ci.merge_idx, ci.qp};
			for (int k = 0; k < 9; k++) { memcpy(o, arrs[k], 256); o += 256; }
			memcpy(o, ci.mv_ref_idx, 256); o += 256;
			memcpy(o, ci.mv_diff_ref_idx, 256); o += 256;
			memcpy(o, ci.mv_ref, 2048); o += 2048;
			memcpy(o, ci.mv_diff, 2048); o += 2048;
			memcpy(o, e->h_coeff.data() + (size_t)n * 6144, 12288); o += 12288;
			for (int c = 0; c < 3; c++) {
				const int nn = c ? 32 : 64, px = (ci.x >> (c ? 1 : 0)), py = (ci.y >> (c ? 1 : 0));
				const int pw = c ? s.width / 2 : s.width, ph = c ? s.height / 2 : s.height, rs = c ? s.stride_c : s.stride_y, m = c ? s.margin_c : s.margin_y;
				const int16_t *p = rec[c].data() + (size_t)m * rs + m;
				for (int yy = 0; yy < nn; yy++) {
					if (py + yy < ph) {
						const int ww = px + nn <= pw ? nn : pw - px;
						memcpy(o, p + (size_t)(py + yy) * rs + px, ww * 2);
					}
					o += nn * 2;
				}
			}
			memcpy(o, n + 1 < s.nctu ? truth.data() + (size_t)(n + 1) * MODE_STATE_BYTES : chain_end.data(), MODE_STATE_BYTES);
		}
	}
	return e->f.slice_type;
}

namespace {
constexpr int GATHER_HEAD = 12;
constexpr int CHAIN_MAX_FRAMES = 32;
__global__ void k_gather_results(const EncDev *devs, uint32_t *out, int pitch, const int *pool_flags)
{
	const EncDev &d = devs[blockIdx.x];
	uint32_t *o = out + (size_t)blockIdx.x * pitch;
	const int nctu = d.seq->nctu;
	if (threadIdx.x < 3) o[threadIdx.x] = (uint32_t)d.counters[threadIdx.x];
	__shared__ uint32_t s_qp, s_bits, s_stale;
	if (threadIdx.x == 0) { s_qp = 0; s_bits = 0; s_stale = 0; }
	__syncthreads();
	uint32_t q = 0, b = 0, stale = 0;
	for (int c = threadIdx.x; c < nctu; c += blockDim.x) { q += d.ctus[c].nodes[0].qp; stale += (uint32_t)d.ctus[c].n_stale_pred; }
	for (int r = threadIdx.x; r < d.seq->hctu; r += blockDim.x) b += d.post.cumbits[r * d.seq->wctu + d.seq->wctu - 1];
	atomicAdd(&s_qp, q);
	atomicAdd(&s_bits, b);
	atomicAdd(&s_stale, stale);
	__syncthreads();
	if (threadIdx.x == 0) o[3] = (uint32_t)(d.post.errors[0] != 0) | ((uint32_t)(pool_flags && pool_flags[1] != 0) << 1) | ((s_stale > 0xffffffu ? 0xffffffu : s_stale) << 8);
	if (threadIdx.x == 0) {
		o[4] = s_qp;
		o[5] = s_bits;
		const double tp = d.counters[2] >= 0 ? d.rc_dyn->target_pict_size : d.frame->rc.target_pict_size;
		memcpy(&o[6], &tp, 8);
		const double fin = d.fin[0], avg = d.frame->avg_dist;
		memcpy(&o[8], &fin, 8);
		memcpy(&o[10], &avg, 8);
	}
	for (int c = threadIdx.x; c < nctu; c += blockDim.x) o[GATHER_HEAD + c] = d.ctus[c].distortion;
	for (int r = threadIdx.x; r < d.seq->hctu; r += blockDim.x) o[pitch - POST_MAX_ROWS + r] = (uint32_t)d.post.ent[r].bytecnt;
}

}

namespace {
int frame_assemble(hmr_gpu_enc *e, const FrameCtx &f, const uint8_t *bytes, const uint32_t *row_bytes, uint8_t *stream, long cap, long *stream_bytes)
{
	const Seq &s = e->seq;
	const int rows = s.wpp ? s.hctu : 1;
	std::vector<const uint8_t *> data(rows);
	std::vector<int> nb(rows);
	size_t o = 0;
	for (int r = 0; r < rows; r++) { data[r] = bytes + o; nb[r] = (int)row_bytes[r]; o += row_bytes[r]; }
	std::vector<uint8_t> out;
	assemble_access_unit(e->es, s, f, e->cfg.profile, data.data(), nb.data(), out);
	*stream_bytes = (long)out.size();
	if ((long)out.size() > cap) {
		hmr_set_error("hmr_gpu_enc_encode: the access unit needs %ld bytes, the buffer holds %ld", (long)out.size(), cap);
		return HMR_GPU_ERR_ARG;
	}
	memcpy(stream, out.data(), out.size());
	return f.slice_type;
}
int frame_finish(hmr_gpu_enc *e, int slot, uint8_t *stream, long cap, long *stream_bytes, uint8_t *recon)
{
	(void)slot;
	const Seq &s = e->seq;
	hipStream_t st = e->ctx->stream;
	int rc, err[4];
	HIP_TRY(hipMemcpyAsync(e->h_ent.data(), e->d_ent, sizeof(RowEnt) * s.hctu, hipMemcpyDeviceToHost, st));
	const int pitch = GATHER_HEAD + s.nctu + POST_MAX_ROWS;
	if (e->lockstep) {
		if ((size_t)pitch > e->gather_words) {
			if (e->d_gather) (void)hipFree(e->d_gather);
			if (e->h_gather) (void)hipHostFree(e->h_gather);
			e->d_gather = e->h_gather = nullptr;
			e->gather_words = 0;
			HIP_TRY(hipMalloc((void **)&e->d_gather, (size_t)pitch * 4));
			HIP_TRY(hipHostMalloc((void **)&e->h_gather, (size_t)pitch * 4, hipHostMallocDefault));
			e->gather_words = (size_t)pitch;
		}
		hipLaunchKernelGGL(k_gather_results, dim3(1), dim3(256), 0, st, (const EncDev *)e->d_batch, e->d_gather, pitch, (const int *)nullptr);
		HIP_TRY(hipGetLastError());
		HIP_TRY(hipMemcpyAsync(e->h_gather, e->d_gather, (size_t)pitch * 4, hipMemcpyDeviceToHost, st));
	} else if ((rc = download_public(e))) return rc;
	HIP_TRY(hipMemcpyAsync(err, e->d_post_err, sizeof err, hipMemcpyDeviceToHost, st));
	HIP_TRY(hipStreamSynchronize(st));
	if (getenv("HENC_DEBUG_POST")) {
		std::vector<PostRow> rows(s.hctu);
		HIP_TRY(hipMemcpy(rows.data(), e->d_rows, sizeof(PostRow) * s.hctu, hipMemcpyDeviceToHost));
		for (int r = 0; r < s.hctu; r++)
			fprintf(stderr, "post row %d: dec %d D %d/%d P %d/%d F %d/%d\n", r, rows[r].dec, rows[r].d_claim, rows[r].d_done, rows[r].p_claim, rows[r].p_done, rows[r].f_claim, rows[r].f_done);
		fprintf(stderr, "post errors %d %d %d %d, sao %d\n", err[0], err[1], err[2], err[3], s.sao);
	}
	if (err[0]) {
		hmr_set_error("hmr_gpu_enc_encode: a CTU row's sub-stream outgrew its buffer (%d bytes)", e->row_cap);
		return HMR_GPU_ERR_HIP;
	}
	if (err[2]) {
		hmr_set_error("hmr_gpu_enc_encode: the post-decision stage was abandoned by its watchdog");
		return HMR_GPU_ERR_HIP;
	}
	const int rows = s.wpp ? s.hctu : 1;
	std::vector<uint32_t> row_bytes(rows);
	size_t total = 0;
	for (int r = 0; r < rows; r++) total += row_bytes[r] = (uint32_t)e->h_ent[r].bytecnt;
	if (e->h_bs.size() < total) e->h_bs.resize(total);
	total = 0;
	for (int r = 0; r < rows; r++) {
		HIP_TRY(hipMemcpyAsync(e->h_bs.data() + total, e->d_bs + (size_t)r * e->row_cap, row_bytes[r], hipMemcpyDeviceToHost, st));
		total += row_bytes[r];
	}
	if (recon) {
		if ((rc = narrow_packed(e, e->d_bytes))) return rc;
		HIP_TRY(hipMemcpyAsync(recon, e->d_bytes, (size_t)s.width * s.height * 3 / 2, hipMemcpyDeviceToHost, st));
	}
	HIP_TRY(hipStreamSynchronize(st));
	const uint32_t *gr = e->h_gather;
	e->note_stale_predictions(e->lockstep ? gr[3] >> 8 : (uint32_t)err[3]);
	const double acc = e->lockstep ? frame_acc_dist(s, e->cfg.wfpp_num_threads, [&](int n) { return gr[GATHER_HEAD + n]; })
				       : frame_acc_dist(s, e->cfg.wfpp_num_threads, [&](int n) { return ((const CtuPublic *)(e->h_public.data() + sizeof(CtuPublic) * n))->distortion; });
	rc = frame_assemble(e, e->f, e->h_bs.data(), row_bytes.data(), stream, cap, stream_bytes);
	if (rc < 0) return rc;
	FrameRcOut ro = {0, 0.0, 0.0};
	if (e->lockstep) {
		ro.sum_qp = (int)gr[4]; ro.consumed_bits = (double)gr[5];
		memcpy(&ro.target_pict_size, &gr[6], 8);
	}
	end_frame(s, e->st, e->f, acc, &ro);
	HIP_TRY(hipEventRecord(e->ctx->ev1, st));
	HIP_TRY(hipStreamSynchronize(st));
	HIP_TRY(hipEventElapsedTime(&e->last_total_ms, e->ev_frame, e->ctx->ev1));
	return e->f.slice_type;
}
}

extern "C" int hmr_gpu_enc_encode_source(hmr_gpu_enc *e, int slot, int image_type, uint8_t *stream, long cap, long *stream_bytes, uint8_t *recon)
{
	if (!e || slot < 0 || slot >= (int)e->src.size() || !stream || !stream_bytes) return HMR_GPU_ERR_ARG;
	if (e->awaiting_delivery) {
		hmr_set_error("hmr_gpu_enc_encode_source: the encoder has an access unit outstanding from a pipelined batch call: flush first");
		return HMR_GPU_ERR_ARG;
	}
	hipStream_t st = e->ctx->stream;
	HIP_TRY(hipSetDevice(e->ctx->device));
	HIP_TRY(hipEventRecord(e->ev_frame, st));
	int rc = set_frame(e, slot, image_type, -1.0);
	if (rc) return rc;
	rc = run_ctu_passes(e);
// ... 4 lines not shown
```

### homerhevc_amd/csrc/k_subpel.hip

```cpp
#include "common.h"

namespace {

constexpr int TW = 64, TH = 16;

__device__ __forceinline__ uint32_t clip255(int v)
{
	v = v < 0 ? 0 : (v > 255 ? 255 : v);
	asm volatile("" : "+v"(v));
	return (uint32_t)v & 255u;
}

__device__ __forceinline__ int xcd_contiguous(unsigned block, unsigned blocks)
{
	const unsigned per_xcd = blocks / 8, tile = (block % 8) * per_xcd + block / 8;
	return (int)tile;
}

typedef short short2_t __attribute__((ext_vector_type(2)));
__device__ __forceinline__ uint32_t pack4_clip(int r0, int r1, int r2, int r3)
{
	const short2_t lo = {0, 0}, hi = {255, 255};
	uint32_t a = __builtin_amdgcn_perm((uint32_t)r1, (uint32_t)r0, 0x05040100u), b = __builtin_amdgcn_perm((uint32_t)r3, (uint32_t)r2, 0x05040100u);
	short2_t va, vb;
	__builtin_memcpy(&va, &a, 4);
	__builtin_memcpy(&vb, &b, 4);
	va = __builtin_elementwise_min(__builtin_elementwise_max(va, lo), hi);
	vb = __builtin_elementwise_min(__builtin_elementwise_max(vb, lo), hi);
	__builtin_memcpy(&a, &va, 4);
	__builtin_memcpy(&b, &vb, 4);
	return __builtin_amdgcn_perm(b, a, 0x06040200u);
}

typedef short short4_t __attribute__((ext_vector_type(4)));
__device__ __forceinline__ short4_t lds4(const int16_t *p) { return *(const short4_t *)p; }


__global__ __launch_bounds__(256) void k_subpel_luma(const int16_t *__restrict__ pic, int stride, int rows, uint8_t *__restrict__ out)
{
	__shared__ __attribute__((aligned(16))) int16_t in[TH + 7][TW + 8];
	__shared__ __attribute__((aligned(16))) int16_t hs[3][TH + 7][TW];
	const int tiles_x = (stride + TW - 1) / TW;
	const int tile = xcd_contiguous(blockIdx.x, gridDim.x);
	const int x0 = (tile % tiles_x) * TW, y0 = (tile / tiles_x) * TH;
	if (y0 >= rows) return;
	const long elems = (long)stride * rows;
	const int t = (int)threadIdx.x;
	for (int i = t; i < (TH + 7) * (TW + 8); i += 256) {
		const int r = i / (TW + 8), c = i - r * (TW + 8);
		const long li = (long)(y0 - 3 + r) * stride + (x0 - 4 + c);
		in[r][c] = (li >= 0 && li < elems) ? pic[li] : (int16_t)0;
	}
	__syncthreads();
	const int c1[8] = {-1, 4, -10, 58, 17, -5, 1, 0}, c2[8] = {-1, 4, -11, 40, 40, -11, 4, -1}, c3[8] = {0, 1, -5, 17, 58, -10, 4, -1};
	for (int i = t; i < (TH + 7) * (TW / 4); i += 256) {
		const int r = i / (TW / 4), c = (i - r * (TW / 4)) << 2;
		const short4_t a = lds4(&in[r][c]), b = lds4(&in[r][c + 4]), d = lds4(&in[r][c + 8]);
		const int sm[12] = {a.x, a.y, a.z, a.w, b.x, b.y, b.z, b.w, d.x, d.y, d.z, d.w};
		short4_t o1, o2, o3;
#pragma unroll
		for (int j = 0; j < 4; j++) {
			int s1 = 0, s2 = 0, s3 = 0;
#pragma unroll
			for (int k = 0; k < 8; k++) {
				const int v = sm[j + 1 + k];
				s1 += v * c1[k]; s2 += v * c2[k]; s3 += v * c3[k];
			}
			o1[j] = (short)(s1 - 8192); o2[j] = (short)(s2 - 8192); o3[j] = (short)(s3 - 8192);
		}
		*(short4_t *)&hs[0][r][c] = o1; *(short4_t *)&hs[1][r][c] = o2; *(short4_t *)&hs[2][r][c] = o3;
	}
	__syncthreads();
	const int ty = t >> 4, tx = (t & 15) << 2;
	const int y = y0 + ty, x = x0 + tx;
	if (y >= rows || x >= stride) return;
	uint32_t pk[16];
	short4_t v0[8], v1[8], v2[8], v3[8];
#pragma unroll
	for (int k = 0; k < 8; k++) { v0[k] = lds4(&in[ty + k][tx + 4]); v1[k] = lds4(&hs[0][ty + k][tx]); v2[k] = lds4(&hs[1][ty + k][tx]); v3[k] = lds4(&hs[2][ty + k][tx]); }
	pk[0] = pack4_clip(v0[3][0], v0[3][1], v0[3][2], v0[3][3]);
	pk[1] = pack4_clip((v1[3][0] + 8192 + 32) >> 6, (v1[3][1] + 8192 + 32) >> 6, (v1[3][2] + 8192 + 32) >> 6, (v1[3][3] + 8192 + 32) >> 6);
	pk[2] = pack4_clip((v2[3][0] + 8192 + 32) >> 6, (v2[3][1] + 8192 + 32) >> 6, (v2[3][2] + 8192 + 32) >> 6, (v2[3][3] + 8192 + 32) >> 6);
	pk[3] = pack4_clip((v3[3][0] + 8192 + 32) >> 6, (v3[3][1] + 8192 + 32) >> 6, (v3[3][2] + 8192 + 32) >> 6, (v3[3][3] + 8192 + 32) >> 6);
#pragma unroll
	for (int fy = 1; fy < 4; fy++) {
		const int *cf = fy == 1 ? c1 : (fy == 2 ? c2 : c3);
		int r[4][4];
#pragma unroll
		for (int j = 0; j < 4; j++) {
			int s0 = 0, s1 = 0, s2 = 0, s3 = 0;
#pragma unroll
			for (int k = 0; k < 8; k++) { s0 += v0[k][j] * cf[k]; s1 += v1[k][j] * cf[k]; s2 += v2[k][j] * cf[k]; s3 += v3[k][j] * cf[k]; }
			r[0][j] = (s0 + 32) >> 6;
			r[1][j] = (s1 + 2048 + (8192 << 6)) >> 12;
			r[2][j] = (s2 + 2048 + (8192 << 6)) >> 12;
			r[3][j] = (s3 + 2048 + (8192 << 6)) >> 12;
		}
#pragma unroll
		for (int fx = 0; fx < 4; fx++) pk[fy * 4 + fx] = pack4_clip(r[fx][0], r[fx][1], r[fx][2], r[fx][3]);
	}
	uint8_t *o = out + ((size_t)y * 16 * stride + x);
#pragma unroll
	for (int f = 0; f < 16; f++) *(uint32_t *)(o + (size_t)f * stride) = pk[f];
}

__global__ __launch_bounds__(256) void k_subpel_chroma(const int16_t *__restrict__ pic, int stride, int rows, uint8_t *__restrict__ out)
{
	__shared__ __attribute__((aligned(16))) int16_t in[TH + 3][TW + 8];
	__shared__ __attribute__((aligned(16))) int16_t hs[7][TH + 3][TW];
	const int tiles_x = (stride + TW - 1) / TW;
	const int tile = xcd_contiguous(blockIdx.x, gridDim.x);
	const int x0 = (tile % tiles_x) * TW, y0 = (tile / tiles_x) * TH;
	if (y0 >= rows) return;
	const long elems = (long)stride * rows;
	const int t = (int)threadIdx.x;
	for (int i = t; i < (TH + 3) * (TW + 8); i += 256) {
		const int r = i / (TW + 8), c = i - r * (TW + 8);
		const long li = (long)(y0 - 1 + r) * stride + (x0 - 4 + c);
		in[r][c] = (li >= 0 && li < elems) ? pic[li] : (int16_t)0;
	}
	__syncthreads();
	const int cf[8][4] = {{0, 64, 0, 0}, {-2, 58, 10, -2}, {-4, 54, 16, -2}, {-6, 46, 28, -4}, {-4, 36, 36, -4}, {-4, 28, 46, -6}, {-2, 16, 54, -4}, {-2, 10, 58, -2}};
	for (int i = t; i < (TH + 3) * (TW / 4); i += 256) {
		const int r = i / (TW / 4), c = (i - r * (TW / 4)) << 2;
		const short4_t a = lds4(&in[r][c]), b = lds4(&in[r][c + 4]), d = lds4(&in[r][c + 8]);
		const int sm[12] = {a.x, a.y, a.z, a.w, b.x, b.y, b.z, b.w, d.x, d.y, d.z, d.w};
#pragma unroll
		for (int fx = 1; fx < 8; fx++) {
			short4_t o;
#pragma unroll
			for (int j = 0; j < 4; j++) o[j] = (short)(sm[j + 3] * cf[fx][0] + sm[j + 4] * cf[fx][1] + sm[j + 5] * cf[fx][2] + sm[j + 6] * cf[fx][3] - 8192);
			*(short4_t *)&hs[fx - 1][r][c] = o;
		}
	}
	__syncthreads();
	const int ty = t >> 4, tx = (t & 15) << 2;
	const int y = y0 + ty, x = x0 + tx;
	if (y >= rows || x >= stride) return;
	uint8_t *o = out + ((size_t)y * 64 * stride + x);
	short4_t in4[4];
#pragma unroll
	for (int k = 0; k < 4; k++) in4[k] = lds4(&in[ty + k][tx + 4]);
	{
		uint32_t pk[8];
#pragma unroll
		for (int fx = 1; fx < 8; fx++) {
			const short4_t h = lds4(&hs[fx - 1][ty + 1][tx]);
			pk[fx] = pack4_clip((h[0] + 8192 + 32) >> 6, (h[1] + 8192 + 32) >> 6, (h[2] + 8192 + 32) >> 6, (h[3] + 8192 + 32) >> 6);
		}
		pk[0] = pack4_clip(in4[1][0], in4[1][1], in4[1][2], in4[1][3]);
#pragma unroll
		for (int f = 0; f < 8; f++) *(uint32_t *)(o + (size_t)f * stride) = pk[f];
	}
	for (int fx = 0; fx < 8; fx++) {
		short4_t h[4];
#pragma unroll
		for (int k = 0; k < 4; k++) h[k] = fx ? lds4(&hs[fx - 1][ty + k][tx]) : in4[k];
#pragma unroll
		for (int fy = 1; fy < 8; fy++) {
			int r[4];
#pragma unroll
			for (int j = 0; j < 4; j++) {
				const int sum = h[0][j] * cf[fy][0] + h[1][j] * cf[fy][1] + h[2][j] * cf[fy][2] + h[3][j] * cf[fy][3];
				r[j] = fx ? (sum + 2048 + (8192 << 6)) >> 12 : (sum + 32) >> 6;
			}
			*(uint32_t *)(o + (size_t)(fy * 8 + fx) * stride) = pack4_clip(r[0], r[1], r[2], r[3]);
		}
	}
}

}

int hmr_subpel_planes_on(hipStream_t stream, const int16_t *pic_y, const int16_t *pic_u, const int16_t *pic_v, int stride_y, int rows_y, int stride_c, int rows_c, uint8_t *out_y,
			 uint8_t *out_u, uint8_t *out_v)
{
	if (!pic_y || !out_y || (stride_y & 3) || (stride_c & 3) || stride_y <= 0 || rows_y <= 0) return HMR_GPU_ERR_ARG;
	const int gy = (((stride_y + TW - 1) / TW) * ((rows_y + TH - 1) / TH) + 7) / 8 * 8;
	hipLaunchKernelGGL(k_subpel_luma, dim3(gy), dim3(256), 0, stream, pic_y, stride_y, rows_y, out_y);
	if (pic_u && pic_v && out_u && out_v) {
		const int gc = (((stride_c + TW - 1) / TW) * ((rows_c + TH - 1) / TH) + 7) / 8 * 8;
		hipLaunchKernelGGL(k_subpel_chroma, dim3(gc), dim3(256), 0, stream, pic_u, stride_c, rows_c, out_u);
		hipLaunchKernelGGL(k_subpel_chroma, dim3(gc), dim3(256), 0, stream, pic_v, stride_c, rows_c, out_v);
	}
	HIP_TRY(hipGetLastError());
	return HMR_GPU_OK;
}
int hmr_subpel_plane_on(hipStream_t stream, int comp, const int16_t *pic, int stride, int rows, uint8_t *out)
{
	if (!pic || !out || (stride & 3) || stride <= 0 || rows <= 0) return HMR_GPU_ERR_ARG;
	const int grid = (((stride + TW - 1) / TW) * ((rows + TH - 1) / TH) + 7) / 8 * 8;
	if (comp == 0) hipLaunchKernelGGL(k_subpel_luma, dim3(grid), dim3(256), 0, stream, pic, stride, rows, out);
	else hipLaunchKernelGGL(k_subpel_chroma, dim3(grid), dim3(256), 0, stream, pic, stride, rows, out);
	HIP_TRY(hipGetLastError());
	return HMR_GPU_OK;
}
extern "C" int hmr_gpu_subpel_planes(hmr_gpu_ctx *ctx, const int16_t *pic_y, const int16_t *pic_u, const int16_t *pic_v, int stride_y, int rows_y, int stride_c, int rows_c,
				     uint8_t *out_y, uint8_t *out_u, uint8_t *out_v)
{
	if (!ctx) return HMR_GPU_ERR_ARG;
	return hmr_subpel_planes_on(ctx->stream, pic_y, pic_u, pic_v, stride_y, rows_y, stride_c, rows_c, out_y, out_u, out_v);
}
```

### include/homer_gpu.h

```cpp
#ifndef HOMER_GPU_H
#define HOMER_GPU_H

#include <stddef.h>
#include <stdint.h>

#ifdef __cplusplus
extern "C" {
#endif

typedef struct hmr_gpu_ctx hmr_gpu_ctx;

enum hmr_gpu_status {
	HMR_GPU_OK = 0,
	HMR_GPU_ERR_NO_DEVICE = -1,
	HMR_GPU_ERR_HIP = -2,
	HMR_GPU_ERR_ARG = -3,
	HMR_GPU_ERR_NOMEM = -4
};


int hmr_gpu_create(hmr_gpu_ctx **out, int device, void *stream);
void hmr_gpu_destroy(hmr_gpu_ctx *ctx);
const char *hmr_gpu_last_error(void);
int hmr_gpu_sync(hmr_gpu_ctx *ctx);
// ... 110 lines not shown
			  int beta_offset_div2, int tc_offset_div2, uint8_t *bs_ver, uint8_t *bs_hor);
int hmr_gpu_deblock_ctu(hmr_gpu_ctx *ctx, const hmr_gpu_frame *frame, const hmr_gpu_units *info, const uint8_t *pred_depth, const uint8_t *tr_idx,
			int cb_qp_offset, int cr_qp_offset, int beta_offset_div2, int tc_offset_div2, int ctu_x, int ctu_y, int ctu_size, int dir);
int hmr_gpu_sao_stats_frame(hmr_gpu_ctx *ctx, const hmr_gpu_frame *orig, const hmr_gpu_frame *recon, int32_t *stats);
int hmr_gpu_sao_stats_ctu(hmr_gpu_ctx *ctx, const hmr_gpu_frame *orig, const hmr_gpu_frame *recon, int ctu_index, int32_t *stats);
int hmr_gpu_sao_apply_frame(hmr_gpu_ctx *ctx, const hmr_gpu_frame *src, const hmr_gpu_frame *dst, const int32_t *params);
int hmr_gpu_sao_apply_ctu(hmr_gpu_ctx *ctx, const hmr_gpu_frame *src, const hmr_gpu_frame *dst, int ctu_index, const int32_t *params);
int hmr_gpu_pad_frame(hmr_gpu_ctx *ctx, const hmr_gpu_frame *frame, int pad_x, int pad_y);


typedef struct hmr_gpu_me_job {
	double corr;
	uint32_t orig_off, orig_stride;
	uint32_t ref_off, ref_stride;
	int16_t gx, gy;
	int16_t init_x, init_y;
	int16_t n_amvp, n_search;
	int16_t amvp[2][2];
	int16_t search[5][2];
	uint32_t action;
	uint32_t reserved;
} hmr_gpu_me_job;
typedef struct hmr_gpu_me_result {
	int32_t mvx, mvy;
	int32_t subx, suby;
	uint32_t sad;
} hmr_gpu_me_result;
int hmr_gpu_motion_estimation_batch(hmr_gpu_ctx *ctx, const hmr_gpu_me_job *jobs, int njobs, int size, const int16_t *orig_base, const int16_t *ref_base,
				    int range_x, int range_y, int frame_w, int frame_h, hmr_gpu_me_result *out);
int hmr_gpu_mc_batch(hmr_gpu_ctx *ctx, const hmr_gpu_job *jobs, int njobs, int flags, int is_bi_predict, const int16_t *a_base, int16_t *c_base);
uint32_t hmr_gpu_motion_estimation(int16_t *orig, int orig_stride, int16_t *ref, int ref_stride, int gx, int gy, int init_x, int init_y, int size,
				   int range_x, int range_y, int frame_w, int frame_h, const int32_t *amvp, int n_amvp, const int32_t *search, int n_search,
				   double corr, int action, int32_t *out_mv4);
void hmr_gpu_mc_luma(int16_t *ref, int ref_stride, int16_t *pred, int pred_stride, int width, int height, int mvx, int mvy, int is_bi);
void hmr_gpu_mc_chroma(int16_t *ref, int ref_stride, int16_t *pred, int pred_stride, int size, int mvx, int mvy, int is_bi);


enum hmr_gpu_op {
	HMR_GPU_OP_SAD = 1, HMR_GPU_OP_SSD16B, HMR_GPU_OP_PREDICT, HMR_GPU_OP_RECONST, HMR_GPU_OP_COPY, HMR_GPU_OP_VARIANCE, HMR_GPU_OP_INTRA_PRED,
	HMR_GPU_OP_INTRA_REFS, HMR_GPU_OP_INTERPOLATE, HMR_GPU_OP_WAVG, HMR_GPU_OP_TRANSFORM, HMR_GPU_OP_ITRANSFORM, HMR_GPU_OP_QUANT,
	HMR_GPU_OP_INV_QUANT, HMR_GPU_OP_MC, HMR_GPU_OP_ME, HMR_GPU_OP_EDGE_FLAGS, HMR_GPU_OP_DEBLOCK, HMR_GPU_OP_SAO_STATS, HMR_GPU_OP_SAO_APPLY, HMR_GPU_OP_PAD,
	HMR_GPU_OP_TU_CHAIN,
	HMR_GPU_OP_INTRA_SEARCH,
	HMR_GPU_OP_INTER_TU_CHAIN = 25,
	HMR_GPU_OP_SAO_OFFSETS = 30,
	HMR_GPU_OP_CHROMA_SEARCH = 29,
	HMR_GPU_OP_TU_MULTI = 28,
	HMR_GPU_OP_PIXEL_MULTI = 27,
	HMR_GPU_OP_TREE_DECIDE = 26,
	HMR_GPU_OP_INTRA_TU_CHAIN = 24
};
typedef struct hmr_gpu_cmd {
	int op, njobs, size;
	int p[4];
	const void *jobs, *a, *b;
	void *c, *out;
	void *p64[3];
	int branch;
} hmr_gpu_cmd;
#define HMR_GPU_MAX_BRANCHES 64
#define HMR_GPU_MAX_SEGMENTS 8
typedef struct hmr_gpu_segment {
	const hmr_gpu_job *jobs;
	void *out;
	int njobs, size;
} hmr_gpu_segment;
int hmr_gpu_pixel_multi(hmr_gpu_ctx *ctx, int op, const hmr_gpu_segment *segs, int nseg, const int16_t *a, const int16_t *b, int16_t *c);
struct hmr_gpu_intra_result;
typedef struct hmr_gpu_tu_segment {
	const void *jobs;
	uint32_t *ssd;
	int32_t *ac_sum;
	const struct hmr_gpu_intra_result *modes;
	int njobs, size, kind, rounds;
} hmr_gpu_tu_segment;
int hmr_gpu_tu_chain_multi(hmr_gpu_ctx *ctx, const hmr_gpu_tu_segment *segs, int nseg, const int16_t *orig_base, const int16_t *decoded_base, int16_t *pred_base,
			   int16_t *level_base, int16_t *recon_base);
typedef struct hmr_gpu_cmdlist hmr_gpu_cmdlist;
int hmr_gpu_cmdlist_create(hmr_gpu_ctx *ctx, const hmr_gpu_cmd *cmds, int n, hmr_gpu_cmdlist **out);
int hmr_gpu_cmdlist_run(hmr_gpu_ctx *ctx, hmr_gpu_cmdlist *list, void **event_pairs);
int hmr_gpu_cmdlist_capture(hmr_gpu_ctx *ctx, hmr_gpu_cmdlist *list);
int hmr_gpu_cmdlist_replay(hmr_gpu_ctx *ctx, hmr_gpu_cmdlist *list);
void hmr_gpu_cmdlist_destroy(hmr_gpu_cmdlist *list);


typedef struct hmr_gpu_tu_job {
	uint32_t orig_off, orig_stride;
	uint32_t pred_off, pred_stride;
	uint32_t rec_off, rec_stride;
	uint32_t lev_off;
	uint32_t p0;
	uint32_t p1;
} hmr_gpu_tu_job;
int hmr_gpu_tu_chain_batch(hmr_gpu_ctx *ctx, const hmr_gpu_tu_job *jobs, int njobs, int size, const int16_t *orig_base, const int16_t *pred_base,
			   int16_t *level_base, int16_t *recon_base, uint32_t *ssd, int32_t *ac_sum);
uint32_t hmr_gpu_tu_chain(int16_t *orig, int orig_stride, int16_t *pred, int pred_stride, int16_t *levels, int16_t *recon, int recon_stride, int size,
			  int is_dst, int scan_mode, int comp, int is_intra, int slice_is_intra, int sign_hiding, int per, int rem, int *ac_sum);

typedef struct hmr_gpu_itu_job {
	uint32_t orig_off, orig_stride;
	uint32_t pred_off, pred_stride;
	uint32_t rec_off, rec_stride;
	uint32_t lev_off;
	uint32_t p0, p1;
	uint32_t dec_off, dec_stride;
	uint32_t flags;
	uint32_t sizes;
	uint32_t mode;
} hmr_gpu_itu_job;
int hmr_gpu_intra_tu_chain_batch(hmr_gpu_ctx *ctx, const hmr_gpu_itu_job *jobs, int njobs, int size, const int16_t *orig_base, const int16_t *decoded_base,
				 int16_t *pred_base, int16_t *level_base, int16_t *recon_base, uint32_t *ssd, int32_t *ac_sum);
uint32_t hmr_gpu_intra_tu_chain(int16_t *orig, int orig_stride, int16_t *decoded_corner, int decoded_stride, int left, int top, int bottom_left, int top_right,
				int bl_size, int tr_size, int strong_enabled, int is_filtered, int mode, int is_luma, int16_t *pred, int pred_stride, int16_t *levels,
				int16_t *recon, int recon_stride, int size, int is_dst, int scan_mode, int comp, int slice_is_intra, int sign_hiding, int per, int rem,
				int *ac_sum);
#define HMR_GPU_ITU_MODE_FROM_SEARCH 0x100u
struct hmr_gpu_intra_result;
int hmr_gpu_intra_tu_chain_modes_batch(hmr_gpu_ctx *ctx, const hmr_gpu_itu_job *jobs, int njobs, int size, const int16_t *orig_base, const int16_t *decoded_base,
				       int16_t *pred_base, int16_t *level_base, int16_t *recon_base, uint32_t *ssd, int32_t *ac_sum,
				       const struct hmr_gpu_intra_result *modes);
int hmr_gpu_intra_tu_chain_rounds_batch(hmr_gpu_ctx *ctx, const hmr_gpu_itu_job *jobs, int njobs, int rounds, int size, const int16_t *orig_base,
					const int16_t *decoded_base, int16_t *pred_base, int16_t *level_base, int16_t *recon_base, uint32_t *ssd, int32_t *ac_sum,
					const struct hmr_gpu_intra_result *modes);
typedef struct hmr_gpu_inter_tu_job {
	uint32_t orig_off, orig_stride;
	uint32_t pred_off, pred_stride;
	uint32_t rec_off, rec_stride;
	uint32_t lev_off;
	uint32_t p0, p1;
	uint32_t reserved;
	double weight, zero_thr;
} hmr_gpu_inter_tu_job;
#define HMR_GPU_INTER_TU_FROM_SOURCE 1u
int hmr_gpu_inter_tu_chain_batch(hmr_gpu_ctx *ctx, const hmr_gpu_inter_tu_job *jobs, int njobs, int size, const int16_t *residual_base, const int16_t *pred_base,
				 int16_t *level_base, int16_t *recon_base, uint32_t *ssd, int32_t *ac_sum);
uint32_t hmr_gpu_inter_tu_chain(int16_t *residual, int residual_stride, int16_t *pred, int pred_stride, int16_t *levels, int16_t *recon, int recon_stride, int size,
				int scan_mode, int comp, int slice_is_intra, int sign_hiding, int per, int rem, double weight, double zero_thr, int *ac_sum);

typedef struct hmr_gpu_inter_tu_host {
	int16_t *residual; int residual_stride;
	int16_t *pred; int pred_stride;
	int16_t *levels;
	int16_t *recon; int recon_stride;
	int size, scan_mode, comp, slice_is_intra, sign_hiding, per, rem;
	double weight, zero_thr;
	uint32_t ssd;
	int ac_sum;
} hmr_gpu_inter_tu_host;
void hmr_gpu_inter_tu_chain_n(hmr_gpu_inter_tu_host *tus, int n);

typedef struct hmr_gpu_intra_job {
	double sqrt_lambda;
	uint32_t orig_off, orig_stride;
	uint32_t dec_off, dec_stride;
	uint32_t adi_off, adif_off;
	uint32_t pred_off, pred_stride;
	uint32_t flags;
	uint32_t sizes;
	int32_t preds[3];
	uint32_t pred_bits[3];
	uint32_t other_bits;
	uint32_t reserved;
} hmr_gpu_intra_job;
typedef struct hmr_gpu_intra_result {
	int32_t best_mode;
	int32_t bits;
	double cost;
} hmr_gpu_intra_result;
int hmr_gpu_intra_search_batch(hmr_gpu_ctx *ctx, const hmr_gpu_intra_job *jobs, int njobs, int size, const int16_t *orig_base,
			       const int16_t *decoded_base, int16_t *out_base, hmr_gpu_intra_result *out);
void hmr_gpu_intra_search(int16_t *orig, int orig_stride, int16_t *decoded_corner, int decoded_stride, int n, int left, int top, int bottom_left,
			  int top_right, int bl_size, int tr_size, int strong_enabled, const int32_t *preds, const int32_t *pred_bits, int other_bits,
			  double sqrt_lambda, int16_t *adi, int16_t *adi_filtered, int16_t *pred, int pred_stride, int32_t *out, double *best_cost);


#define HMR_GPU_TREE_NO_PARENT 0xffffffffu
typedef struct hmr_gpu_tree_job {
	uint32_t parent;
	uint32_t child[4];
	uint32_t par_rec_off, par_rec_stride;
	uint32_t chl_rec_off, chl_rec_stride;
	uint32_t par_lev_off, chl_lev_off;
	uint32_t size;
	uint32_t rule;
} hmr_gpu_tree_job;
typedef struct hmr_gpu_tree_result {
	uint32_t split;
	uint32_t cost, sum;
	uint8_t cbf[4];
} hmr_gpu_tree_result;
int hmr_gpu_tree_decide_batch(hmr_gpu_ctx *ctx, const hmr_gpu_tree_job *jobs, int njobs, const uint32_t *ssd, const int32_t *ac_sum, int16_t *recon_base,
			      int16_t *level_base, hmr_gpu_tree_result *out);
void hmr_gpu_intra_luma_cu(int16_t *orig, int orig_stride, int16_t *dec_par, int dec_par_stride, int16_t *dec_chl, int dec_chl_stride, const int32_t *nb,
			   int strong_enabled, const int32_t *preds, const int32_t *pred_bits, int other_bits, double sqrt_lambda, int16_t *adi, int16_t *adi_filtered,
			   int16_t *pred, int pred_stride, int16_t *lev_par, int16_t *lev_chl, int size, int slice_is_intra, int sign_hiding, int per, int rem, int rule,
			   int32_t *out, double *best_cost);


typedef struct hmr_gpu_chroma_job {
	double sqrt_lambda;
	uint32_t orig_u_off, orig_v_off, orig_stride;
	uint32_t dec_u_off, dec_v_off, dec_stride;
	uint32_t flags;
	uint32_t sizes;
	uint32_t luma_mode;
	uint32_t reserved;
} hmr_gpu_chroma_job;
int hmr_gpu_chroma_search_batch(hmr_gpu_ctx *ctx, const hmr_gpu_chroma_job *jobs, int njobs, int size, const int16_t *orig_base, const int16_t *decoded_base,
				const hmr_gpu_intra_result *luma_modes, hmr_gpu_intra_result *out);
void hmr_gpu_intra_chroma_cu(int16_t *orig_u, int16_t *orig_v, int orig_stride, int16_t *dec_u, int16_t *dec_v, int dec_stride, const int32_t *nb, int luma_mode,
			     int split, double sqrt_lambda, double weight, int16_t *pred_u, int16_t *pred_v, int pred_stride, int16_t *lev_u, int16_t *lev_v, int size,
			     int slice_is_intra, int sign_hiding, int per, int rem, int32_t *out);


int hmr_gpu_sao_offsets_frame(hmr_gpu_ctx *ctx, const int32_t *stats, int n_ctu, const double *lambdas, int32_t *offsets, int32_t *aux, int64_t *dist);
void hmr_gpu_sao_offsets_ctu(const int32_t *stats, const double *lambdas, int32_t *offsets, int32_t *aux, int64_t *dist);


typedef struct hmr_gpu_enc_cfg {
	int32_t size, profile, width, height;
	float frame_rate;
	int32_t cu_size, max_pred_partition_depth, max_intra_tr_depth, max_inter_tr_depth, intra_period, gop_size, num_b, num_ref_frames;
	int32_t motion_estimation_precision, qp, chroma_qp_offset, num_enc_engines, wfpp_enable, wfpp_num_threads, sign_hiding, sample_adaptive_offset;
	int32_t bitrate_mode, bitrate, vbv_size, vbv_init, reinit_gop_on_scene_change, rd_mode, performance_mode;
} hmr_gpu_enc_cfg;
typedef struct hmr_gpu_enc hmr_gpu_enc;

int hmr_gpu_enc_create(hmr_gpu_ctx *ctx, const hmr_gpu_enc_cfg *cfg, hmr_gpu_enc **out);
int hmr_gpu_enc_create_serial_pool(hmr_gpu_ctx *ctx, const hmr_gpu_enc_cfg *cfg, hmr_gpu_enc **out);
void hmr_gpu_enc_destroy(hmr_gpu_enc *enc);
int hmr_gpu_enc_record_bytes(void);
int hmr_gpu_enc_frame_ctus(hmr_gpu_enc *enc, const uint8_t *y, const uint8_t *u, const uint8_t *v, int image_type, const uint8_t *ref_y, const uint8_t *ref_u,
			   const uint8_t *ref_v, double avg_dist, uint8_t *records);
float hmr_gpu_enc_last_ctu_ms(hmr_gpu_enc *enc);

int hmr_gpu_enc_encode(hmr_gpu_enc *enc, const uint8_t *y, const uint8_t *u, const uint8_t *v, int image_type, uint8_t *stream, long cap, long *stream_bytes,
		       uint8_t *recon);
int hmr_gpu_enc_load_source(hmr_gpu_enc *enc, int slot, const uint8_t *y, const uint8_t *u, const uint8_t *v);
int hmr_gpu_enc_encode_source(hmr_gpu_enc *enc, int slot, int image_type, uint8_t *stream, long cap, long *stream_bytes, uint8_t *recon);
int hmr_gpu_enc_encode_batch(hmr_gpu_enc **encs, int n, const int *slots, const int *image_types, uint8_t **streams, const long *caps, long *stream_bytes);
int hmr_gpu_enc_encode_batch_pipelined(hmr_gpu_enc **encs, int n, const int *slots, const int *image_types, uint8_t **streams, const long *caps, long *stream_bytes);
int hmr_gpu_enc_last_stats(hmr_gpu_enc *enc, int *passes, int *ctu_encodes, float *ctu_ms, float *frame_ms);
int hmr_gpu_enc_stale_predictions(hmr_gpu_enc *enc, long *last_picture, long *all_pictures);
int hmr_gpu_enc_profile(hmr_gpu_enc *enc, unsigned long long *out, int reset);
int hmr_gpu_enc_timeline(hmr_gpu_enc *enc, unsigned long long *out);

int hmr_gpu_enc_create_engine(hmr_gpu_ctx *ctx, const hmr_gpu_enc_cfg *cfg, int engine_index, hmr_gpu_enc **out);
int hmr_gpu_enc_state_bytes(void);
long hmr_gpu_enc_reference_elems(hmr_gpu_enc *enc, int comp);
int hmr_gpu_enc_export_reference(hmr_gpu_enc *enc, int16_t *dev_y, int16_t *dev_u, int16_t *dev_v, void *state);
int hmr_gpu_enc_import_reference(hmr_gpu_enc *enc, const int16_t *dev_y, const int16_t *dev_u, const int16_t *dev_v, const void *state);
long hmr_gpu_enc_reference_bytes(hmr_gpu_enc *enc);
int hmr_gpu_enc_create_engine_twin(hmr_gpu_ctx *ctx, hmr_gpu_enc *of, hmr_gpu_enc **out);
int hmr_gpu_enc_encode_chain(hmr_gpu_enc **encs, int n, hmr_gpu_enc *prev, const int *slots, const int *image_types, uint8_t **streams, const long *caps, long *stream_bytes);
int hmr_gpu_enc_export_references8(hmr_gpu_enc **encs, int n, uint8_t *dev_rows, long pitch, void *states);
int hmr_gpu_enc_import_references8(hmr_gpu_enc **encs, int n, const uint8_t *dev_rows, long pitch, const void *states);

enum { HMR_GPU_PIC_I420 = 0, HMR_GPU_PIC_NV12 = 1 };
typedef struct hmr_gpu_picture {
	int32_t format, reserved;
	const uint8_t *plane[3];
	int64_t pitch[3];
} hmr_gpu_picture;
int hmr_gpu_picture_check(const hmr_gpu_picture *pic, int width, int height);
int hmr_gpu_enc_load_source_device(hmr_gpu_enc *enc, int slot, const hmr_gpu_picture *pic, void *producer_stream);
int hmr_gpu_enc_load_sources_device(hmr_gpu_enc **encs, int n, const int *slots, const hmr_gpu_picture *pics, void *producer_stream);

int hmr_gpu_enc_export_pictures_device(hmr_gpu_enc **encs, int n, const hmr_gpu_picture *pics, const int *slots, uint64_t *dev_ssd, void *consumer_stream);
int hmr_gpu_enc_export_picture_device(hmr_gpu_enc *enc, const hmr_gpu_picture *pic, int slot, uint64_t *dev_ssd, void *consumer_stream);
int hmr_gpu_psnr(const uint64_t ssd[3], int width, int height, double psnr[3]);

enum { HMR_GPU_RGB_PACKED8 = 0, HMR_GPU_RGB_PLANAR8 = 1, HMR_GPU_RGB_PLANAR_F16 = 2, HMR_GPU_RGB_PLANAR_F32 = 3 };
enum { HMR_GPU_MATRIX_BT601 = 0, HMR_GPU_MATRIX_BT709 = 1 };
typedef struct hmr_gpu_rgb_picture {
	int32_t format, matrix, full_range, reserved;
	int32_t pixel_bytes;
	int32_t offset[3];
	const void *plane[3];
	int64_t pitch[3];
} hmr_gpu_rgb_picture;
int hmr_gpu_rgb_picture_check(const hmr_gpu_rgb_picture *pic, int width, int height);
int hmr_gpu_rgb_convert_host(const hmr_gpu_rgb_picture *pic, int width, int height, uint8_t *y, uint8_t *u, uint8_t *v);
int hmr_gpu_enc_load_source_rgb_device(hmr_gpu_enc *enc, int slot, const hmr_gpu_rgb_picture *pic, void *producer_stream);
int hmr_gpu_enc_load_sources_rgb_device(hmr_gpu_enc **encs, int n, const int *slots, const hmr_gpu_rgb_picture *pics, void *producer_stream);
int hmr_gpu_enc_export_source_device(hmr_gpu_enc *enc, int slot, const hmr_gpu_picture *out, void *consumer_stream);
int hmr_gpu_enc_export_sources_device(hmr_gpu_enc **encs, int n, const int *slots, const hmr_gpu_picture *outs, void *consumer_stream);

typedef struct hmr_gpu_scaled_picture {
	hmr_gpu_picture pic;
	int32_t width, height;
} hmr_gpu_scaled_picture;
int hmr_gpu_scale_check(int src_w, int src_h, int dst_w, int dst_h);
int hmr_gpu_enc_load_sources_scaled_device(hmr_gpu_enc **encs, int n, const int *slots, const hmr_gpu_scaled_picture *pics, void *producer_stream);
int hmr_gpu_enc_load_source_scaled_device(hmr_gpu_enc *enc, int slot, const hmr_gpu_scaled_picture *pic, void *producer_stream);
int hmr_gpu_scale_host(const hmr_gpu_scaled_picture *pic, int dst_w, int dst_h, uint8_t *y, uint8_t *u, uint8_t *v);

int hmr_gpu_enc_ssim_device(hmr_gpu_enc **encs, int n, const int *slots, int64_t *dev_ssim, void *consumer_stream);
int hmr_gpu_enc_ssim_one_device(hmr_gpu_enc *enc, int slot, int64_t *dev_ssim, void *consumer_stream);
int hmr_gpu_ssim(const int64_t sums[3], int width, int height, double ssim[3]);
int hmr_gpu_ssim_host(const hmr_gpu_picture *a, const hmr_gpu_picture *b, int width, int height, int64_t sums[3]);

int hmr_gpu_subpel_planes(hmr_gpu_ctx *ctx, const int16_t *pic_y, const int16_t *pic_u, const int16_t *pic_v, int stride_y, int rows_y, int stride_c, int rows_c,
			  uint8_t *out_y, uint8_t *out_u, uint8_t *out_v);

int hmr_gpu_probe_valu_issue(hmr_gpu_ctx *ctx, int waves_per_simd, int dependent, double *wave_instr_per_s, double *ms);
int hmr_gpu_probe_issue(hmr_gpu_ctx *ctx, int op, int waves_per_simd, int dependent, double *wave_instr_per_s, double *ms);

void hmr_gpu_prim_bytes(int on);
uint32_t hmr_gpu_prim_sad(int16_t *src, uint32_t src_stride, int16_t *pred, uint32_t pred_stride, int size);
uint32_t hmr_gpu_prim_ssd16b(int16_t *src, uint32_t src_stride, int16_t *pred, uint32_t pred_stride, int size);
void hmr_gpu_prim_predict(int16_t *orig, int orig_stride, int16_t *pred, int pred_stride, int16_t *residual, int residual_stride, int size);
void hmr_gpu_prim_reconst(int16_t *pred, int pred_stride, int16_t *residual, int residual_stride, int16_t *decoded, int decoded_stride, int size);
uint32_t hmr_gpu_prim_modified_variance(int16_t *p, int size, int stride, int modif);
void hmr_gpu_prim_intra_planar(int16_t *prediction, int pred_stride, int16_t *adi_pred_buff, int adi_size, int cu_size);
void hmr_gpu_prim_intra_angular(int16_t *prediction, int pred_stride, int16_t *adi_pred_buff, int adi_size, int cu_size, int cu_mode, int is_luma);
void hmr_gpu_prim_fill_reference_samples(int16_t *decoded_corner, int stride, int n, int left, int top, int bottom_left, int top_right, int bl_size, int tr_size, int16_t *adi);
void hmr_gpu_prim_adi_filter(int16_t *adi, int16_t *out, int adi_size, int n, int strong_enabled);
void hmr_gpu_prim_transform(int16_t *block, int16_t *coeff, int block_stride, int n, int is_dst);
void hmr_gpu_prim_itransform(int16_t *block, int16_t *coeff, int block_stride, int n, int is_dst);
void hmr_gpu_prim_quant(int16_t *src, int16_t *dst, int16_t *delta_u, int scan_mode, int depth, int comp, int is_intra, int slice_is_intra, int sign_hiding, int *ac_sum,
			int cu_size, int per, int rem);
void hmr_gpu_prim_inv_quant(int16_t *src, int16_t *dst, int depth, int comp, int is_intra, int cu_size, int per, int rem);
int hmr_gpu_prim_multi_sad(int maxc, const uint8_t *src, const uint8_t *plane, size_t plane_bytes, const int64_t *cand_off, int ncalls, int stride, int n, uint32_t *out);

enum hmr_gpu_walk_step { HMR_GPU_WALK_QUAD8_Y = 1, HMR_GPU_WALK_QUAD8_C, HMR_GPU_WALK_QUAD16_Y, HMR_GPU_WALK_QUAD16_C, HMR_GPU_WALK_TU, HMR_GPU_WALK_TU_PAIR };
typedef struct hmr_gpu_walk_case {
	int32_t step, node, comp, one_slot;
	int32_t qp, ctu_x, ctu_y, slice_type;
	int32_t sign_hiding, chroma_qp_offset, stride_y, stride_c;
	int32_t mv[4][2];
	double avg_dist, chroma_weight;
	int64_t sub_y, sub_c[2], curr, pred;
} hmr_gpu_walk_case;
typedef struct hmr_gpu_walk_out {
	uint32_t dist[4][3];
	int32_t sum[4][3];
	uint32_t raw[4][3], cbf[4][3];
	uint32_t stray, reserved[15];
	uint8_t pred[4][256];
	int16_t rec[4][256], lv[4][256];
} hmr_gpu_walk_out;
int hmr_gpu_walk_forms(const hmr_gpu_walk_case *cases, int ncases, const uint8_t *arena, size_t arena_bytes, hmr_gpu_walk_out *out);

#ifdef __cplusplus
}
#endif
#endif
```

Before: 469.5 frames/s.

## Batch sub-pel plane interpolation into job-table kernels with dot2 vertical filtering

Replaces the per-picture, per-plane subpel kernel launches on three streams with a job table. The table is copied to the device, and one luma and one chroma launch cover the whole batch through a 2-D grid. The subpel kernels are also rewritten: wider tiles, vectorised LDS staging, sdot2-based vertical phase filters with a wave per horizontal phase, and vector stores. This aims to cut thousands of launches per batch and raise kernel efficiency. The trade-offs are a ring-buffer dependency for the job table and more register pressure in the templated kernels.

```diff
diff --git a/homerhevc_amd/csrc/k_encode.hip b/homerhevc_amd/csrc/k_encode.hip
--- a/homerhevc_amd/csrc/k_encode.hip
+++ b/homerhevc_amd/csrc/k_encode.hip
@@ -19,6 +19,7 @@
 
 using namespace henc;
 
+#include "subpel_jobs.h"
 int hmr_subpel_plane_on(hipStream_t stream, int comp, const int16_t *pic, int stride, int rows, uint8_t *out);
 int hmr_subpel_planes_on(hipStream_t stream, const int16_t *pic_y, const int16_t *pic_u, const int16_t *pic_v, int stride_y, int rows_y, int stride_c, int rows_c, uint8_t *out_y,
 			 uint8_t *out_u, uint8_t *out_v);
diff --git a/homerhevc_amd/csrc/k_encode_batch.inc b/homerhevc_amd/csrc/k_encode_batch.inc
--- a/homerhevc_amd/csrc/k_encode_batch.inc
+++ b/homerhevc_amd/csrc/k_encode_batch.inc
@@ -67,7 +67,7 @@
 	return HMR_GPU_OK;
 }
 
-int batch_launch(hmr_gpu_enc **encs, int n, const int *slots, const int *image_types, int *pitch_out)
+int batch_launch(hmr_gpu_enc **encs, int n, const int *slots, const int *image_types, int *pitch_out, std::chrono::steady_clock::time_point *setup_done)
 {
 	hmr_gpu_enc *lead = encs[0];
 	hipStream_t bst = lead->ctx->stream;
@@ -91,26 +91,23 @@
 		needs_rd = needs_rd || e->seq.rd_mode == RDM_FULL;
 		if (e->seq.nctu > max_ctus) max_ctus = e->seq.nctu;
 	}
-	if (!lead->plane_stream[0]) {
-		for (int k = 0; k < 2; k++) {
-			HIP_TRY(hipStreamCreateWithFlags(&lead->plane_stream[k], hipStreamNonBlocking));
-			HIP_TRY(hipEventCreateWithFlags(&lead->ev_plane[k], hipEventDisableTiming));
-		}
-		HIP_TRY(hipEventCreateWithFlags(&lead->ev_plane[2], hipEventDisableTiming));
-	}
-	HIP_TRY(hipEventRecord(lead->ev_plane[2], bst));
-	for (int k = 0; k < 2; k++) HIP_TRY(hipStreamWaitEvent(lead->plane_stream[k], lead->ev_plane[2], 0));
-	for (int i = 0; i < n; i++) {
-		hmr_gpu_enc *e = encs[i];
-		const Seq &s = e->seq;
-		if (e->f.slice_type == SLICE_I) continue;
-		if ((rc = hmr_subpel_plane_on(bst, 0, e->d_pic[e->cur ^ 1][0], s.stride_y, s.height + 2 * s.margin_y, e->planes.y))) return rc;
-		for (int k = 0; k < 2; k++)
-			if ((rc = hmr_subpel_plane_on(lead->plane_stream[k], 1 + k, e->d_pic[e->cur ^ 1][1 + k], s.stride_c, s.height / 2 + 2 * s.margin_c, e->planes.c[k]))) return rc;
-	}
-	for (int k = 0; k < 2; k++) {
-		HIP_TRY(hipEventRecord(lead->ev_plane[k], lead->plane_stream[k]));
-		HIP_TRY(hipStreamWaitEvent(bst, lead->ev_plane[k], 0));
+	if (setup_done) *setup_done = std::chrono::steady_clock::now();
+	{
+		SubpelJob *table;
+		hipEvent_t turn;
+		if ((rc = lead->subpel.prepare(n, bst)) || (rc = lead->subpel.next_table(&table, &turn))) return rc;
+		int m = 0;
+		for (int i = 0; i < n; i++) {
+			hmr_gpu_enc *e = encs[i];
+			const Seq &s = e->seq;
+			if (e->f.slice_type == SLICE_I) continue;
+			int16_t *const *ref = e->d_pic[e->cur ^ 1];
+			table[m++] = SubpelJob{{ref[0], ref[1], ref[2]}, {e->planes.y, e->planes.c[0], e->planes.c[1]}, s.stride_y, s.height + 2 * s.margin_y, s.stride_c, s.height / 2 + 2 * s.margin_c};
+		}
+		if (m) {
+			if ((rc = hmr_subpel_jobs_launch(bst, table, lead->subpel.d, m))) return rc;
+			HIP_TRY(hipEventRecord(turn, bst));
+		}
 	}
 	if (!lead->d_batch) {
 		HIP_TRY(hipMalloc((void **)&lead->d_batch, BATCH_MAX * sizeof(EncDev)));
@@ -234,8 +231,8 @@
 	if (!getenv("HENC_BATCH_TIMING")) return;
 	static std::chrono::steady_clock::time_point last_end;
 	const auto now = std::chrono::steady_clock::now();
-	fprintf(stderr, "batch step%s: launch %.1f ms, wait for the pool %.1f, queue device parts %.1f, download wait %.1f (%.0f MB), entropy coding %.1f; the call %.1f, since the last call %.1f\n",
-		pipelined ? " (pipelined)" : "", bt.ms(0, 1), pipelined ? bt.ms(6, 2) : bt.ms(1, 2), bt.ms(2, 3), bt.ms(4, 5), lead->pend_total / 1e6, bt.ms(5, 6),
+	fprintf(stderr, "batch step%s: launch %.1f ms (of which frame set-up %.1f), wait for the pool %.1f, queue device parts %.1f, download wait %.1f (%.0f MB), entropy coding %.1f; the call %.1f, since the last call %.1f\n",
+		pipelined ? " (pipelined)" : "", bt.ms(0, 1), bt.ms(0, 7), pipelined ? bt.ms(6, 2) : bt.ms(1, 2), bt.ms(2, 3), bt.ms(4, 5), lead->pend_total / 1e6, bt.ms(5, 6),
 		std::chrono::duration<double, std::milli>(now - bt.t[0]).count(), std::chrono::duration<double, std::milli>(bt.t[0] - last_end).count());
 	last_end = now;
 }
@@ -256,7 +253,7 @@
 	BatchTimes bt;
 	int pitch = 0;
 	bt.t[0] = std::chrono::steady_clock::now();
-	if ((rc = batch_launch(encs, n, slots, image_types, &pitch))) return rc;
+	if ((rc = batch_launch(encs, n, slots, image_types, &pitch, &bt.t[7]))) return rc;
 	bt.t[1] = std::chrono::steady_clock::now();
 	if ((rc = batch_finish(encs, n, slots, pitch, bt))) return rc;
 	if ((rc = batch_deliver(lead, streams, caps, stream_bytes, bt))) return rc;
@@ -285,7 +282,7 @@
 	BatchTimes bt;
 	for (auto &t : bt.t) t = std::chrono::steady_clock::now();
 	int pitch = 0;
-	if (slots && (rc = batch_launch(encs, n, slots, image_types, &pitch))) return rc;
+	if (slots && (rc = batch_launch(encs, n, slots, image_types, &pitch, &bt.t[7]))) return rc;
 	bt.t[1] = std::chrono::steady_clock::now();
 	if (lead->pending) {
 		if ((rc = batch_deliver(lead, streams, caps, stream_bytes, bt))) return rc;
diff --git a/homerhevc_amd/csrc/k_encode_object.inc b/homerhevc_amd/csrc/k_encode_object.inc
--- a/homerhevc_amd/csrc/k_encode_object.inc
+++ b/homerhevc_amd/csrc/k_encode_object.inc
@@ -126,8 +126,6 @@
 	hipEvent_t ev_decided = nullptr;
 	FrameCtx *d_frames = nullptr, *h_frames = nullptr;
 	EncDev *h_devs = nullptr;
-	hipStream_t plane_stream[2] = {nullptr, nullptr};
-	hipEvent_t ev_plane[3] = {nullptr, nullptr, nullptr};
 	int *d_pool_state = nullptr;
 	WorkSlow *d_pool_slow = nullptr;
 	int pool_workers = 0;
@@ -136,6 +134,7 @@
 	JobRing<ScaleJob> scale;
 	JobRing<EgressJob> egress;
 	JobRing<SsimJob> ssim;
+	JobRing<SubpelJob> subpel;
 	bool has_picture = false;
 	hipStream_t pic_stream = nullptr;
 	hipEvent_t ev_pic_done = nullptr, ev_own_done = nullptr;
@@ -793,8 +792,6 @@
 	if (e->d_frames) (void)hipFree(e->d_frames);
 	if (e->h_frames) (void)hipHostFree(e->h_frames);
 	if (e->h_devs) (void)hipHostFree(e->h_devs);
-	for (int k = 0; k < 2; k++) if (e->plane_stream[k]) { (void)hipStreamSynchronize(e->plane_stream[k]); (void)hipStreamDestroy(e->plane_stream[k]); }
-	for (int k = 0; k < 3; k++) if (e->ev_plane[k]) (void)hipEventDestroy(e->ev_plane[k]);
 	if (e->copy_stream) { (void)hipStreamSynchronize(e->copy_stream); (void)hipStreamDestroy(e->copy_stream); }
 	if (e->d_gather) (void)hipFree(e->d_gather);
 	if (e->h_gather) (void)hipHostFree(e->h_gather);
@@ -804,6 +801,7 @@
 	e->scale.release();
 	e->egress.release();
 	e->ssim.release();
+	e->subpel.release();
 	if (e->ev_pic_done) (void)hipEventDestroy(e->ev_pic_done);
 	if (e->ev_own_done) (void)hipEventDestroy(e->ev_own_done);
 	if (e->d_batch) (void)hipFree(e->d_batch);
diff --git a/homerhevc_amd/csrc/k_subpel.hip b/homerhevc_amd/csrc/k_subpel.hip
--- a/homerhevc_amd/csrc/k_subpel.hip
+++ b/homerhevc_amd/csrc/k_subpel.hip
@@ -1,21 +1,25 @@
+#include <algorithm>
+
 #include "common.h"
+#include "subpel_jobs.h"
 
 namespace {
 
-constexpr int TW = 64, TH = 16;
-
-__device__ __forceinline__ uint32_t clip255(int v)
-{
-	v = v < 0 ? 0 : (v > 255 ? 255 : v);
-	asm volatile("" : "+v"(v));
-	return (uint32_t)v & 255u;
-}
+constexpr int TW = 128, TH = 16, TH_C = 8;
+constexpr int IW = TW + 16;
+constexpr int HW = TW + 8;
 
 __device__ __forceinline__ int xcd_contiguous(unsigned block, unsigned blocks)
 {
 	const unsigned per_xcd = blocks / 8, tile = (block % 8) * per_xcd + block / 8;
 	return (int)tile;
 }
+
+#define GLOBAL_AS __attribute__((address_space(1)))
+typedef const int16_t GLOBAL_AS *pic_ptr;
+typedef uint8_t GLOBAL_AS *out_ptr;
+typedef uint32_t u32x2 __attribute__((ext_vector_type(2)));
+typedef uint32_t u32x4 __attribute__((ext_vector_type(4)));
 
 typedef short short2_t __attribute__((ext_vector_type(2)));
 __device__ __forceinline__ uint32_t pack4_clip(int r0, int r1, int r2, int r3)
@@ -35,27 +39,111 @@
 typedef short short4_t __attribute__((ext_vector_type(4)));
 __device__ __forceinline__ short4_t lds4(const int16_t *p) { return *(const short4_t *)p; }
 
-
-__global__ __launch_bounds__(256) void k_subpel_luma(const int16_t *__restrict__ pic, int stride, int rows, uint8_t *__restrict__ out)
-{
-	__shared__ __attribute__((aligned(16))) int16_t in[TH + 7][TW + 8];
-	__shared__ __attribute__((aligned(16))) int16_t hs[3][TH + 7][TW];
+__device__ __forceinline__ int dot2(uint32_t pair, uint32_t taps, int acc)
+{
+	short2_t p, c;
+	__builtin_memcpy(&p, &pair, 4);
+	__builtin_memcpy(&c, &taps, 4);
+	return __builtin_amdgcn_sdot2(p, c, acc, false);
+}
+constexpr uint32_t taps(int lo, int hi) { return ((uint32_t)lo & 0xffffu) | ((uint32_t)hi << 16); }
+
+template <int VW>
+__device__ __forceinline__ void lds_row(const int16_t *p, uint32_t *d)
+{
+	if constexpr (VW == 4) {
+		const u32x2 v = *(const u32x2 *)p;
+		d[0] = v.x; d[1] = v.y;
+	} else {
+#pragma unroll
+		for (int i = 0; i < VW / 8; i++) {
+			const u32x4 v = *(const u32x4 *)(p + 8 * i);
+			d[4 * i] = v.x; d[4 * i + 1] = v.y; d[4 * i + 2] = v.z; d[4 * i + 3] = v.w;
+		}
+	}
+}
+template <int VW>
+__device__ __forceinline__ void store_row(out_ptr p, const uint32_t *d)
+{
+	if constexpr (VW == 16) *(u32x4 GLOBAL_AS *)p = u32x4{d[0], d[1], d[2], d[3]};
+	else if constexpr (VW == 8) *(u32x2 GLOBAL_AS *)p = u32x2{d[0], d[1]};
+	else *(uint32_t GLOBAL_AS *)p = d[0];
+}
+
+__device__ __forceinline__ void stage_tile(int16_t *in, pic_ptr pic, int stride, long elems, int x0, int ytop, int nr, int t)
+{
+	const bool aligned = ((uintptr_t)pic & 7) == 0;
+	for (int i = t; i < nr * (IW / 4); i += 256) {
+		const int r = i / (IW / 4), c = (i - r * (IW / 4)) << 2;
+		const long li = (long)(ytop + r) * stride + (x0 - 8 + c);
+		short4_t v = {0, 0, 0, 0};
+		if (li >= 0 && li < elems) {
+			if (aligned) v = *(const short4_t GLOBAL_AS *)(pic + li);
+			else { v.x = pic[li]; v.y = pic[li + 1]; v.z = pic[li + 2]; v.w = pic[li + 3]; }
+		}
+		*(short4_t *)&in[r * IW + c] = v;
+	}
+}
+
+template <int VW, int NT, int NFY>
+__device__ __forceinline__ void vertical_phases(const int16_t *src, int sw, bool first, int mid, const uint32_t (&tp)[NFY][NT / 2], out_ptr o, size_t fstep)
+{
+	constexpr int NP = VW / 2;
+	uint32_t R[NT][NP];
+#pragma unroll
+	for (int k = 0; k < NT; k++) lds_row<VW>(src + k * sw, R[k]);
+	const int bias = first ? 32 : 2048 + (8192 << 6), sh = first ? 6 : 12, bias0 = first ? 0 : 8192 + 32, sh0 = first ? 0 : 6;
+	{
+		uint32_t pk[VW / 4];
+#pragma unroll
+		for (int q = 0; q < VW / 4; q++) {
+			const int a = (int)R[mid][2 * q], b = (int)R[mid][2 * q + 1];
+			pk[q] = pack4_clip(((int)(short)a + bias0) >> sh0, ((a >> 16) + bias0) >> sh0, ((int)(short)b + bias0) >> sh0, ((b >> 16) + bias0) >> sh0);
+		}
+		store_row<VW>(o, pk);
+	}
+	uint32_t even[NT / 2][NP], odd[NT / 2][NP];
+#pragma unroll
+	for (int m = 0; m < NT / 2; m++)
+#pragma unroll
+		for (int i = 0; i < NP; i++) {
+			even[m][i] = __builtin_amdgcn_perm(R[2 * m + 1][i], R[2 * m][i], 0x05040100u);
+			odd[m][i] = __builtin_amdgcn_perm(R[2 * m + 1][i], R[2 * m][i], 0x07060302u);
+		}
+#pragma unroll
+	for (int fy = 1; fy < NFY; fy++) {
+		uint32_t pk[VW / 4];
+#pragma unroll
+		for (int q = 0; q < VW / 4; q++) {
+			int s[4] = {bias, bias, bias, bias};
+#pragma unroll
+			for (int m = 0; m < NT / 2; m++) {
+				s[0] = dot2(even[m][2 * q], tp[fy][m], s[0]);
+				s[1] = dot2(odd[m][2 * q], tp[fy][m], s[1]);
+				s[2] = dot2(even[m][2 * q + 1], tp[fy][m], s[2]);
+				s[3] = dot2(odd[m][2 * q + 1], tp[fy][m], s[3]);
+			}
+			pk[q] = pack4_clip(s[0] >> sh, s[1] >> sh, s[2] >> sh, s[3] >> sh);
+		}
+		store_row<VW>(o + fy * fstep, pk);
+	}
+}
+
+template <int VW>
+__device__ __forceinline__ void luma_tile(pic_ptr pic, int stride, int rows, out_ptr out, int tile)
+{
+	__shared__ __attribute__((aligned(16))) int16_t in[(TH + 7) * IW];
+	__shared__ __attribute__((aligned(16))) int16_t hs[3 * (TH + 7) * HW];
 	const int tiles_x = (stride + TW - 1) / TW;
-	const int tile = xcd_contiguous(blockIdx.x, gridDim.x);
 	const int x0 = (tile % tiles_x) * TW, y0 = (tile / tiles_x) * TH;
 	if (y0 >= rows) return;
-	const long elems = (long)stride * rows;
 	const int t = (int)threadIdx.x;
-	for (int i = t; i < (TH + 7) * (TW + 8); i += 256) {
-		const int r = i / (TW + 8), c = i - r * (TW + 8);
-		const long li = (long)(y0 - 3 + r) * stride + (x0 - 4 + c);
-		in[r][c] = (li >= 0 && li < elems) ? pic[li] : (int16_t)0;
-	}
+	stage_tile(in, pic, stride, (long)stride * rows, x0, y0 - 3, TH + 7, t);
 	__syncthreads();
 	const int c1[8] = {-1, 4, -10, 58, 17, -5, 1, 0}, c2[8] = {-1, 4, -11, 40, 40, -11, 4, -1}, c3[8] = {0, 1, -5, 17, 58, -10, 4, -1};
 	for (int i = t; i < (TH + 7) * (TW / 4); i += 256) {
 		const int r = i / (TW / 4), c = (i - r * (TW / 4)) << 2;
-		const short4_t a = lds4(&in[r][c]), b = lds4(&in[r][c + 4]), d = lds4(&in[r][c + 8]);
+		const short4_t a = lds4(&in[r * IW + c + 4]), b = lds4(&in[r * IW + c + 8]), d = lds4(&in[r * IW + c + 12]);
 		const int sm[12] = {a.x, a.y, a.z, a.w, b.x, b.y, b.z, b.w, d.x, d.y, d.z, d.w};
 		short4_t o1, o2, o3;
 #pragma unroll
@@ -68,104 +156,114 @@
 			}
 			o1[j] = (short)(s1 - 8192); o2[j] = (short)(s2 - 8192); o3[j] = (short)(s3 - 8192);
 		}
-		*(short4_t *)&hs[0][r][c] = o1; *(short4_t *)&hs[1][r][c] = o2; *(short4_t *)&hs[2][r][c] = o3;
+		*(short4_t *)&hs[(0 * (TH + 7) + r) * HW + c] = o1; *(short4_t *)&hs[(1 * (TH + 7) + r) * HW + c] = o2; *(short4_t *)&hs[(2 * (TH + 7) + r) * HW + c] = o3;
 	}
 	__syncthreads();
-	const int ty = t >> 4, tx = (t & 15) << 2;
-	const int y = y0 + ty, x = x0 + tx;
-	if (y >= rows || x >= stride) return;
-	uint32_t pk[16];
-	short4_t v0[8], v1[8], v2[8], v3[8];
-#pragma unroll
-	for (int k = 0; k < 8; k++) { v0[k] = lds4(&in[ty + k][tx + 4]); v1[k] = lds4(&hs[0][ty + k][tx]); v2[k] = lds4(&hs[1][ty + k][tx]); v3[k] = lds4(&hs[2][ty + k][tx]); }
-	pk[0] = pack4_clip(v0[3][0], v0[3][1], v0[3][2], v0[3][3]);
-	pk[1] = pack4_clip((v1[3][0] + 8192 + 32) >> 6, (v1[3][1] + 8192 + 32) >> 6, (v1[3][2] + 8192 + 32) >> 6, (v1[3][3] + 8192 + 32) >> 6);
-	pk[2] = pack4_clip((v2[3][0] + 8192 + 32) >> 6, (v2[3][1] + 8192 + 32) >> 6, (v2[3][2] + 8192 + 32) >> 6, (v2[3][3] + 8192 + 32) >> 6);
-	pk[3] = pack4_clip((v3[3][0] + 8192 + 32) >> 6, (v3[3][1] + 8192 + 32) >> 6, (v3[3][2] + 8192 + 32) >> 6, (v3[3][3] + 8192 + 32) >> 6);
-#pragma unroll
-	for (int fy = 1; fy < 4; fy++) {
-		const int *cf = fy == 1 ? c1 : (fy == 2 ? c2 : c3);
-		int r[4][4];
-#pragma unroll
-		for (int j = 0; j < 4; j++) {
-			int s0 = 0, s1 = 0, s2 = 0, s3 = 0;
-#pragma unroll
-			for (int k = 0; k < 8; k++) { s0 += v0[k][j] * cf[k]; s1 += v1[k][j] * cf[k]; s2 += v2[k][j] * cf[k]; s3 += v3[k][j] * cf[k]; }
-			r[0][j] = (s0 + 32) >> 6;
-			r[1][j] = (s1 + 2048 + (8192 << 6)) >> 12;
-			r[2][j] = (s2 + 2048 + (8192 << 6)) >> 12;
-			r[3][j] = (s3 + 2048 + (8192 << 6)) >> 12;
-		}
-#pragma unroll
-		for (int fx = 0; fx < 4; fx++) pk[fy * 4 + fx] = pack4_clip(r[fx][0], r[fx][1], r[fx][2], r[fx][3]);
-	}
-	uint8_t *o = out + ((size_t)y * 16 * stride + x);
-#pragma unroll
-	for (int f = 0; f < 16; f++) *(uint32_t *)(o + (size_t)f * stride) = pk[f];
-}
-
-__global__ __launch_bounds__(256) void k_subpel_chroma(const int16_t *__restrict__ pic, int stride, int rows, uint8_t *__restrict__ out)
-{
-	__shared__ __attribute__((aligned(16))) int16_t in[TH + 3][TW + 8];
-	__shared__ __attribute__((aligned(16))) int16_t hs[7][TH + 3][TW];
+	constexpr int G = TW / VW, RP = 64 / G;
+	constexpr uint32_t tp[4][4] = {{0, 0, 0, 0},
+				       {taps(-1, 4), taps(-10, 58), taps(17, -5), taps(1, 0)},
+				       {taps(-1, 4), taps(-11, 40), taps(40, -11), taps(4, -1)},
+				       {taps(0, 1), taps(-5, 17), taps(58, -10), taps(4, -1)}};
+	const int fx = __builtin_amdgcn_readfirstlane(t >> 6), lane = t & 63;
+	const int16_t *src = fx ? hs + (fx - 1) * (TH + 7) * HW : in + 8;
+	const int sw = fx ? HW : IW;
+	for (int p = 0; p < TH / RP; p++) {
+		const int ty = p * RP + lane / G, tx = (lane % G) * VW;
+		const int y = y0 + ty, x = x0 + tx;
+		if (y >= rows || x >= stride) continue;
+		vertical_phases<VW, 8, 4>(src + ty * sw + tx, sw, fx == 0, 3, tp, out + ((size_t)y * 16 + fx) * stride + x, (size_t)4 * stride);
+	}
+}
+
+template <int VW>
+__device__ __forceinline__ void chroma_tile(pic_ptr pic, int stride, int rows, out_ptr out, int tile)
+{
+	__shared__ __attribute__((aligned(16))) int16_t in[(TH_C + 3) * IW];
+	__shared__ __attribute__((aligned(16))) int16_t hs[7 * (TH_C + 3) * HW];
 	const int tiles_x = (stride + TW - 1) / TW;
-	const int tile = xcd_contiguous(blockIdx.x, gridDim.x);
-	const int x0 = (tile % tiles_x) * TW, y0 = (tile / tiles_x) * TH;
+	const int x0 = (tile % tiles_x) * TW, y0 = (tile / tiles_x) * TH_C;
 	if (y0 >= rows) return;
-	const long elems = (long)stride * rows;
 	const int t = (int)threadIdx.x;
-	for (int i = t; i < (TH + 3) * (TW + 8); i += 256) {
-		const int r = i / (TW + 8), c = i - r * (TW + 8);
-		const long li = (long)(y0 - 1 + r) * stride + (x0 - 4 + c);
-		in[r][c] = (li >= 0 && li < elems) ? pic[li] : (int16_t)0;
-	}
+	stage_tile(in, pic, stride, (long)stride * rows, x0, y0 - 1, TH_C + 3, t);
 	__syncthreads();
 	const int cf[8][4] = {{0, 64, 0, 0}, {-2, 58, 10, -2}, {-4, 54, 16, -2}, {-6, 46, 28, -4}, {-4, 36, 36, -4}, {-4, 28, 46, -6}, {-2, 16, 54, -4}, {-2, 10, 58, -2}};
-	for (int i = t; i < (TH + 3) * (TW / 4); i += 256) {
+	for (int i = t; i < (TH_C + 3) * (TW / 4); i += 256) {
 		const int r = i / (TW / 4), c = (i - r * (TW / 4)) << 2;
-		const short4_t a = lds4(&in[r][c]), b = lds4(&in[r][c + 4]), d = lds4(&in[r][c + 8]);
+		const short4_t a = lds4(&in[r * IW + c + 4]), b = lds4(&in[r * IW + c + 8]), d = lds4(&in[r * IW + c + 12]);
 		const int sm[12] = {a.x, a.y, a.z, a.w, b.x, b.y, b.z, b.w, d.x, d.y, d.z, d.w};
 #pragma unroll
 		for (int fx = 1; fx < 8; fx++) {
 			short4_t o;
 #pragma unroll
 			for (int j = 0; j < 4; j++) o[j] = (short)(sm[j + 3] * cf[fx][0] + sm[j + 4] * cf[fx][1] + sm[j + 5] * cf[fx][2] + sm[j + 6] * cf[fx][3] - 8192);
-			*(short4_t *)&hs[fx - 1][r][c] = o;
+			*(short4_t *)&hs[((fx - 1) * (TH_C + 3) + r) * HW + c] = o;
 		}
 	}
 	__syncthreads();
-	const int ty = t >> 4, tx = (t & 15) << 2;
-	const int y = y0 + ty, x = x0 + tx;
-	if (y >= rows || x >= stride) return;
-	uint8_t *o = out + ((size_t)y * 64 * stride + x);
-	short4_t in4[4];
-#pragma unroll
-	for (int k = 0; k < 4; k++) in4[k] = lds4(&in[ty + k][tx + 4]);
-	{
-		uint32_t pk[8];
-#pragma unroll
-		for (int fx = 1; fx < 8; fx++) {
-			const short4_t h = lds4(&hs[fx - 1][ty + 1][tx]);
-			pk[fx] = pack4_clip((h[0] + 8192 + 32) >> 6, (h[1] + 8192 + 32) >> 6, (h[2] + 8192 + 32) >> 6, (h[3] + 8192 + 32) >> 6);
-		}
-		pk[0] = pack4_clip(in4[1][0], in4[1][1], in4[1][2], in4[1][3]);
-#pragma unroll
-		for (int f = 0; f < 8; f++) *(uint32_t *)(o + (size_t)f * stride) = pk[f];
-	}
-	for (int fx = 0; fx < 8; fx++) {
-		short4_t h[4];
-#pragma unroll
-		for (int k = 0; k < 4; k++) h[k] = fx ? lds4(&hs[fx - 1][ty + k][tx]) : in4[k];
-#pragma unroll
-		for (int fy = 1; fy < 8; fy++) {
-			int r[4];
-#pragma unroll
-			for (int j = 0; j < 4; j++) {
-				const int sum = h[0][j] * cf[fy][0] + h[1][j] * cf[fy][1] + h[2][j] * cf[fy][2] + h[3][j] * cf[fy][3];
-				r[j] = fx ? (sum + 2048 + (8192 << 6)) >> 12 : (sum + 32) >> 6;
-			}
-			*(uint32_t *)(o + (size_t)(fy * 8 + fx) * stride) = pack4_clip(r[0], r[1], r[2], r[3]);
-		}
+	constexpr int G = TW / VW, RP = 64 / G, PASSES = TH_C / RP;
+	constexpr uint32_t tp[8][2] = {{0, 0}, {taps(-2, 58), taps(10, -2)}, {taps(-4, 54), taps(16, -2)}, {taps(-6, 46), taps(28, -4)}, {taps(-4, 36), taps(36, -4)},
+				       {taps(-4, 28), taps(46, -6)}, {taps(-2, 16), taps(54, -4)}, {taps(-2, 10), taps(58, -2)}};
+	const int w = __builtin_amdgcn_readfirstlane(t >> 6), lane = t & 63;
+	for (int item = w; item < 8 * PASSES; item += 4) {
+		const int fx = item & 7, p = item >> 3;
+		const int ty = p * RP + lane / G, tx = (lane % G) * VW;
+		const int y = y0 + ty, x = x0 + tx;
+		if (y >= rows || x >= stride) continue;
+		const int16_t *src = fx ? hs + (fx - 1) * (TH_C + 3) * HW : in + 8;
+		const int sw = fx ? HW : IW;
+		vertical_phases<VW, 4, 8>(src + ty * sw + tx, sw, fx == 0, 1, tp, out + ((size_t)y * 64 + fx) * stride + x, (size_t)8 * stride);
+	}
+}
+
+template <int VW>
+__global__ __launch_bounds__(256) void k_subpel_luma(const int16_t *__restrict__ pic, int stride, int rows, uint8_t *__restrict__ out)
+{
+	luma_tile<VW>((pic_ptr)pic, stride, rows, (out_ptr)out, xcd_contiguous(blockIdx.x, gridDim.x));
+}
+template <int VW>
+__global__ __launch_bounds__(256) void k_subpel_chroma(const int16_t *__restrict__ pic, int stride, int rows, uint8_t *__restrict__ out)
+{
+	chroma_tile<VW>((pic_ptr)pic, stride, rows, (out_ptr)out, xcd_contiguous(blockIdx.x, gridDim.x));
+}
+template <int VW>
+__global__ __launch_bounds__(256) void k_subpel_luma_jobs(const SubpelJob *__restrict__ jobs)
+{
+	const SubpelJob &j = jobs[blockIdx.y];
+	luma_tile<VW>((pic_ptr)j.pic[0], j.stride_y, j.rows_y, (out_ptr)j.out[0], xcd_contiguous(blockIdx.x, gridDim.x));
+}
+template <int VW>
+__global__ __launch_bounds__(256) void k_subpel_chroma_jobs(const SubpelJob *__restrict__ jobs)
+{
+	const SubpelJob &j = jobs[blockIdx.y >> 1];
+	const int comp = 1 + (blockIdx.y & 1);
+	chroma_tile<VW>((pic_ptr)j.pic[comp], j.stride_c, j.rows_c, (out_ptr)j.out[comp], xcd_contiguous(blockIdx.x, gridDim.x));
+}
+__global__ __launch_bounds__(64) void k_subpel_jobs(const uint32_t *h_jobs, uint32_t *d_jobs, int words)
+{
+	for (int k = threadIdx.x; k < words; k += blockDim.x) d_jobs[blockIdx.x * words + k] = h_jobs[blockIdx.x * words + k];
+}
+
+inline int store_width(const uint8_t *out, int stride)
+{
+	const uintptr_t a = (uintptr_t)out | (uintptr_t)stride;
+	return (a & 15) == 0 ? 16 : ((a & 7) == 0 ? 8 : 4);
+}
+inline int grid_of(int stride, int rows, int th) { return (((stride + TW - 1) / TW) * ((rows + th - 1) / th) + 7) / 8 * 8; }
+inline bool plane_ok(const int16_t *pic, const uint8_t *out, int stride, int rows) { return pic && out && !((uintptr_t)out & 3) && !(stride & 3) && stride > 0 && rows > 0; }
+
+void launch_plane(hipStream_t stream, int comp, const int16_t *pic, int stride, int rows, uint8_t *out)
+{
+	const int vw = store_width(out, stride);
+	if (comp == 0) {
+		const dim3 grid(grid_of(stride, rows, TH));
+		if (vw == 16) hipLaunchKernelGGL(k_subpel_luma<16>, grid, dim3(256), 0, stream, pic, stride, rows, out);
+		else if (vw == 8) hipLaunchKernelGGL(k_subpel_luma<8>, grid, dim3(256), 0, stream, pic, stride, rows, out);
+		else hipLaunchKernelGGL(k_subpel_luma<4>, grid, dim3(256), 0, stream, pic, stride, rows, out);
+	} else {
+		const dim3 grid(grid_of(stride, rows, TH_C));
+		if (vw == 16) hipLaunchKernelGGL(k_subpel_chroma<16>, grid, dim3(256), 0, stream, pic, stride, rows, out);
+		else if (vw == 8) hipLaunchKernelGGL(k_subpel_chroma<8>, grid, dim3(256), 0, stream, pic, stride, rows, out);
+		else hipLaunchKernelGGL(k_subpel_chroma<4>, grid, dim3(256), 0, stream, pic, stride, rows, out);
 	}
 }
 
@@ -174,29 +272,69 @@
 int hmr_subpel_planes_on(hipStream_t stream, const int16_t *pic_y, const int16_t *pic_u, const int16_t *pic_v, int stride_y, int rows_y, int stride_c, int rows_c, uint8_t *out_y,
 			 uint8_t *out_u, uint8_t *out_v)
 {
-	if (!pic_y || !out_y || (stride_y & 3) || (stride_c & 3) || stride_y <= 0 || rows_y <= 0) return HMR_GPU_ERR_ARG;
-	const int gy = (((stride_y + TW - 1) / TW) * ((rows_y + TH - 1) / TH) + 7) / 8 * 8;
-	hipLaunchKernelGGL(k_subpel_luma, dim3(gy), dim3(256), 0, stream, pic_y, stride_y, rows_y, out_y);
-	if (pic_u && pic_v && out_u && out_v) {
-		const int gc = (((stride_c + TW - 1) / TW) * ((rows_c + TH - 1) / TH) + 7) / 8 * 8;
-		hipLaunchKernelGGL(k_subpel_chroma, dim3(gc), dim3(256), 0, stream, pic_u, stride_c, rows_c, out_u);
-		hipLaunchKernelGGL(k_subpel_chroma, dim3(gc), dim3(256), 0, stream, pic_v, stride_c, rows_c, out_v);
+	if (!plane_ok(pic_y, out_y, stride_y, rows_y) || (stride_c & 3)) return HMR_GPU_ERR_ARG;
+	const bool chroma = pic_u && pic_v && out_u && out_v;
+	if (chroma && (!plane_ok(pic_u, out_u, stride_c, rows_c) || !plane_ok(pic_v, out_v, stride_c, rows_c))) return HMR_GPU_ERR_ARG;
+	launch_plane(stream, 0, pic_y, stride_y, rows_y, out_y);
+	if (chroma) {
+		launch_plane(stream, 1, pic_u, stride_c, rows_c, out_u);
+		launch_plane(stream, 2, pic_v, stride_c, rows_c, out_v);
 	}
 	HIP_TRY(hipGetLastError());
 	return HMR_GPU_OK;
 }
 int hmr_subpel_plane_on(hipStream_t stream, int comp, const int16_t *pic, int stride, int rows, uint8_t *out)
 {
-	if (!pic || !out || (stride & 3) || stride <= 0 || rows <= 0) return HMR_GPU_ERR_ARG;
-	const int grid = (((stride + TW - 1) / TW) * ((rows + TH - 1) / TH) + 7) / 8 * 8;
-	if (comp == 0) hipLaunchKernelGGL(k_subpel_luma, dim3(grid), dim3(256), 0, stream, pic, stride, rows, out);
-	else hipLaunchKernelGGL(k_subpel_chroma, dim3(grid), dim3(256), 0, stream, pic, stride, rows, out);
+	if (!plane_ok(pic, out, stride, rows)) return HMR_GPU_ERR_ARG;
+	launch_plane(stream, comp, pic, stride, rows, out);
 	HIP_TRY(hipGetLastError());
 	return HMR_GPU_OK;
 }
+int hmr_subpel_jobs_launch(hipStream_t stream, const SubpelJob *h_jobs, SubpelJob *d_jobs, int n)
+{
+	static_assert(sizeof(SubpelJob) % 4 == 0, "word copies");
+	if (!h_jobs || !d_jobs || n < 1 || n > SUBPEL_MAX_JOBS) return HMR_GPU_ERR_ARG;
+	int vw_y = 16, vw_c = 16, gy = 0, gc = 0;
+	for (int i = 0; i < n; i++) {
+		const SubpelJob &j = h_jobs[i];
+		if (!plane_ok(j.pic[0], j.out[0], j.stride_y, j.rows_y) || !plane_ok(j.pic[1], j.out[1], j.stride_c, j.rows_c) || !plane_ok(j.pic[2], j.out[2], j.stride_c, j.rows_c)) {
+			hmr_set_error("phase planes: picture %d of the batch: needs the three padded planes, outputs on 4-byte boundaries and strides that are multiples of 4", i);
+			return HMR_GPU_ERR_ARG;
+		}
+		vw_y = std::min(vw_y, store_width(j.out[0], j.stride_y));
+		vw_c = std::min(vw_c, std::min(store_width(j.out[1], j.stride_c), store_width(j.out[2], j.stride_c)));
+		gy = std::max(gy, grid_of(j.stride_y, j.rows_y, TH));
+		gc = std::max(gc, grid_of(j.stride_c, j.rows_c, TH_C));
+	}
+	hipLaunchKernelGGL(k_subpel_jobs, dim3(n), dim3(64), 0, stream, (const uint32_t *)h_jobs, (uint32_t *)d_jobs, (int)(sizeof(SubpelJob) / 4));
+	const SubpelJob *jobs = d_jobs;
+	if (vw_y == 16) hipLaunchKernelGGL(k_subpel_luma_jobs<16>, dim3(gy, n), dim3(256), 0, stream, jobs);
+	else if (vw_y == 8) hipLaunchKernelGGL(k_subpel_luma_jobs<8>, dim3(gy, n), dim3(256), 0, stream, jobs);
+	else hipLaunchKernelGGL(k_subpel_luma_jobs<4>, dim3(gy, n), dim3(256), 0, stream, jobs);
+	if (vw_c == 16) hipLaunchKernelGGL(k_subpel_chroma_jobs<16>, dim3(gc, 2 * n), dim3(256), 0, stream, jobs);
+	else if (vw_c == 8) hipLaunchKernelGGL(k_subpel_chroma_jobs<8>, dim3(gc, 2 * n), dim3(256), 0, stream, jobs);
+	else hipLaunchKernelGGL(k_subpel_chroma_jobs<4>, dim3(gc, 2 * n), dim3(256), 0, stream, jobs);
+	HIP_TRY(hipGetLastError());
+	return HMR_GPU_OK;
+}
 extern "C" int hmr_gpu_subpel_planes(hmr_gpu_ctx *ctx, const int16_t *pic_y, const int16_t *pic_u, const int16_t *pic_v, int stride_y, int rows_y, int stride_c, int rows_c,
 				     uint8_t *out_y, uint8_t *out_u, uint8_t *out_v)
 {
 	if (!ctx) return HMR_GPU_ERR_ARG;
 	return hmr_subpel_planes_on(ctx->stream, pic_y, pic_u, pic_v, stride_y, rows_y, stride_c, rows_c, out_y, out_u, out_v);
 }
+extern "C" int hmr_gpu_subpel_planes_batch(hmr_gpu_ctx *ctx, const hmr_gpu_subpel_job *jobs, int n)
+{
+	if (!ctx || !jobs || n < 1 || n > SUBPEL_MAX_JOBS) return HMR_GPU_ERR_ARG;
+	int rc = hmr_ctx_need_stage(ctx);
+	if (rc) return rc;
+	HIP_TRY(hipStreamSynchronize(ctx->stream));
+	SubpelJob *h = (SubpelJob *)ctx->h_stage;
+	for (int i = 0; i < n; i++) {
+		const hmr_gpu_subpel_job &s = jobs[i];
+		h[i] = SubpelJob{{s.pic_y, s.pic_u, s.pic_v}, {s.out_y, s.out_u, s.out_v}, s.stride_y, s.rows_y, s.stride_c, s.rows_c};
+	}
+	if ((rc = hmr_subpel_jobs_launch(ctx->stream, h, (SubpelJob *)ctx->d_stage, n))) return rc;
+	HIP_TRY(hipStreamSynchronize(ctx->stream));
+	return HMR_GPU_OK;
+}
diff --git a/homerhevc_amd/csrc/subpel_jobs.h b/homerhevc_amd/csrc/subpel_jobs.h
--- /dev/null
+++ b/homerhevc_amd/csrc/subpel_jobs.h
@@ -0,0 +1,11 @@
+#pragma once
+#include <cstdint>
+
+struct SubpelJob {
+	const int16_t *pic[3];
+	uint8_t *out[3];
+	int32_t stride_y, rows_y, stride_c, rows_c;
+};
+constexpr int SUBPEL_MAX_JOBS = 512;
+
+int hmr_subpel_jobs_launch(hipStream_t stream, const SubpelJob *h_jobs, SubpelJob *d_jobs, int n);
diff --git a/include/homer_gpu.h b/include/homer_gpu.h
--- a/include/homer_gpu.h
+++ b/include/homer_gpu.h
@@ -436,6 +436,12 @@
 
 int hmr_gpu_subpel_planes(hmr_gpu_ctx *ctx, const int16_t *pic_y, const int16_t *pic_u, const int16_t *pic_v, int stride_y, int rows_y, int stride_c, int rows_c,
 			  uint8_t *out_y, uint8_t *out_u, uint8_t *out_v);
+typedef struct hmr_gpu_subpel_job {
+	const int16_t *pic_y, *pic_u, *pic_v;
+	uint8_t *out_y, *out_u, *out_v;
+	int32_t stride_y, rows_y, stride_c, rows_c;
+} hmr_gpu_subpel_job;
+int hmr_gpu_subpel_planes_batch(hmr_gpu_ctx *ctx, const hmr_gpu_subpel_job *jobs, int n);
 
 int hmr_gpu_probe_valu_issue(hmr_gpu_ctx *ctx, int waves_per_simd, int dependent, double *wave_instr_per_s, double *ms);
 int hmr_gpu_probe_issue(hmr_gpu_ctx *ctx, int op, int waves_per_simd, int dependent, double *wave_instr_per_s, double *ms);
```

New measurement: 474.1 frames/s (median of 6 runs). No clear change (+1.0%).
